# groupeLIAMG/ttcr

Measured on AMD Instinct MI355X. Metric: Mnodes/s per sweep-iteration (512^3 fp32 grid, first-order FSM), higher is better.
Workload: dtype f32

## Files before the change

include/ttcr_amd.h:

```cpp
#ifndef TTCR_AMD_H
#define TTCR_AMD_H

#include <stddef.h>
#include <stdint.h>

#ifdef __cplusplus
extern "C" {
#endif

typedef struct ttcr_fsm_grid ttcr_fsm_grid;

enum { TTCR_F32 = 0, TTCR_F64 = 1 };

enum {
    TTCR_OK = 0,
    TTCR_ERR_VALUE = 1,
    TTCR_ERR_RUNTIME = 2,
    TTCR_ERR_DEVICE = 3,
    TTCR_ERR_UNSUPPORTED = 4
};

int ttcr_fsm_device_count(void);

const char* ttcr_fsm_last_error(void);

int ttcr_fsm3d_create(ttcr_fsm_grid** out, int dtype, int cell_slowness, uint32_t ncx, uint32_t ncy,
                      uint32_t ncz, double dx, double xmin, double ymin, double zmin, double eps,
                      int maxit, int weno, int n_slots, int translate_origin, int device);

int ttcr_fsm2d_create(ttcr_fsm_grid** out, int dtype, int cell_slowness, uint32_t ncx, uint32_t ncz,
                      double dx, double dz, double xmin, double zmin, double eps, int maxit, int weno,
                      int rotated_template, int n_slots, int device);

int ttcr_fsm3d_create_multi(ttcr_fsm_grid** out, int dtype, int cell_slowness, uint32_t ncx, uint32_t ncy,
                            uint32_t ncz, double dx, double xmin, double ymin, double zmin, double eps,
                            int maxit, int weno, int n_slots, int translate_origin, const int* devices, int n_devices);
int ttcr_fsm2d_create_multi(ttcr_fsm_grid** out, int dtype, int cell_slowness, uint32_t ncx, uint32_t ncz,
                            double dx, double dz, double xmin, double zmin, double eps, int maxit, int weno,
                            int rotated_template, int n_slots, const int* devices, int n_devices);
int ttcr_fsm_n_devices(const ttcr_fsm_grid* g);

void ttcr_fsm_destroy(ttcr_fsm_grid* g);

int ttcr_fsm_set_slowness(ttcr_fsm_grid* g, const void* s, size_t n);
int ttcr_fsm_set_slowness_device(ttcr_fsm_grid* g, const void* d_s, size_t n);
int ttcr_fsm_set_slowness_c_order(ttcr_fsm_grid* g, const void* s, size_t n);

int ttcr_fsm_get_slowness(ttcr_fsm_grid* g, void* out, size_t n);

int ttcr_fsm_raytrace(ttcr_fsm_grid* g, int slot, int n_tx, const void* tx, const void* t0, int n_rx,
                      const void* rx, void* tt_out);

int ttcr_fsm_raytrace_multi(ttcr_fsm_grid* g, int n_src, const int* tx_off, const void* tx,
                            const void* t0, const int* rx_off, const void* rx, void* tt_out);

int ttcr_fsm_get_tt(ttcr_fsm_grid* g, int slot, void* out, size_t n);
int ttcr_fsm_get_tt_device(ttcr_fsm_grid* g, int slot, void** d_ptr);
int ttcr_fsm_get_tt_device_view(ttcr_fsm_grid* g, int slot, void** d_ptr, size_t* stride);

int ttcr_fsm_interp(ttcr_fsm_grid* g, int slot, int n_pts, const void* pts, void* tt_out);

int ttcr_fsm_compute_slowness(ttcr_fsm_grid* g, int n_pts, const void* pts, int translated, void* out);

int ttcr_fsm_get_niter(ttcr_fsm_grid* g, int slot, int* niter, int* niterw);
int ttcr_fsm_get_changes(ttcr_fsm_grid* g, int slot, double* first_order, int n_first, double* weno, int n_weno);
int ttcr_fsm_get_reference_changes(ttcr_fsm_grid* g, int slot, double* first_order, int n_first, double* weno, int n_weno);

int ttcr_fsm_n_slots(const ttcr_fsm_grid* g);
size_t ttcr_fsm_n_nodes(const ttcr_fsm_grid* g);
size_t ttcr_fsm_n_cells(const ttcr_fsm_grid* g);

int ttcr_fsm_set_option(ttcr_fsm_grid* g, const char* key, double value);

int ttcr_fsm_rays_size(const ttcr_fsm_grid* g, size_t* n_rays, size_t* n_points);
int ttcr_fsm_get_rays(const ttcr_fsm_grid* g, long long* offsets, void* pts);

int ttcr_fsm_raytrace_rays(ttcr_fsm_grid* g, int slot, int n_tx, const void* tx, const void* t0, int n_rx,
                           const void* rx, void* tt_out);
int ttcr_fsm_slot_rays_size(const ttcr_fsm_grid* g, int slot, size_t* n_rays, size_t* n_points);
int ttcr_fsm_get_slot_rays(const ttcr_fsm_grid* g, int slot, long long* offsets, void* pts);

int ttcr_fsm_raytrace_m(ttcr_fsm_grid* g, int slot, int n_tx, const void* tx, const void* t0, int n_rx,
                        const void* rx, void* tt_out);
int ttcr_fsm_raytrace_rm(ttcr_fsm_grid* g, int slot, int n_tx, const void* tx, const void* t0, int n_rx,
                         const void* rx, void* tt_out);
int ttcr_fsm_slot_m_size(const ttcr_fsm_grid* g, int slot, size_t* n_rows, size_t* nnz);
int ttcr_fsm_get_slot_m(const ttcr_fsm_grid* g, int slot, long long* row_off, long long* j, void* v);
int ttcr_fsm_raytrace_multi_m(ttcr_fsm_grid* g, int n_src, const int* tx_off, const void* tx, const void* t0, const int* rx_off,
                              const void* rx, void* tt_out, int with_rays);
int ttcr_fsm_multi_m_size(const ttcr_fsm_grid* g, size_t* n_rows, size_t* nnz);
int ttcr_fsm_get_multi_m(const ttcr_fsm_grid* g, long long* row_off, long long* j, void* v);

typedef struct ttcr_fsm_tape ttcr_fsm_tape;
int ttcr_fsm_raytrace_multi_tape(ttcr_fsm_grid* g, int n_src, const int* tx_off, const void* tx, const void* t0, const int* rx_off,
                                 const void* rx, void* tt_out, ttcr_fsm_tape** tape);
int ttcr_fsm_tape_size(const ttcr_fsm_tape* t, size_t* n_rows, size_t* n_cols, size_t* nnz);
int ttcr_fsm_tape_bytes(const ttcr_fsm_tape* t, size_t* bytes);
int ttcr_fsm_tape_device(const ttcr_fsm_tape* t, int* device);
int ttcr_fsm_tape_get_csr(const ttcr_fsm_tape* t, long long* row_off, long long* j, void* v);
int ttcr_fsm_tape_vjp(const ttcr_fsm_tape* t, const void* w, int w_on_device, void* grad, int grad_on_device);
int ttcr_fsm_tape_free(ttcr_fsm_tape* t);

typedef struct ttcr_fsm_adjoint ttcr_fsm_adjoint;
int ttcr_fsm_raytrace_multi_adjoint(ttcr_fsm_grid* g, int n_src, const int* tx_off, const void* tx, const void* t0, const int* rx_off,
                                    const void* rx, void* tt_out, ttcr_fsm_adjoint** tape);
int ttcr_fsm_raytrace_multi_adjoint_cells(ttcr_fsm_grid* g, int n_src, const int* tx_off, const void* tx, const void* t0, const int* rx_off,
                                          const void* rx, void* tt_out, ttcr_fsm_adjoint** tape);
int ttcr_fsm_adjoint_model(const ttcr_fsm_adjoint* t, int* cells, size_t* n_params, size_t* n_nodes);
int ttcr_fsm_adjoint_size(const ttcr_fsm_adjoint* t, size_t* n_events, size_t* n_rows, size_t* n_nodes);
int ttcr_fsm_adjoint_bytes(const ttcr_fsm_adjoint* t, size_t* bytes);
int ttcr_fsm_adjoint_device(const ttcr_fsm_adjoint* t, int* device);
int ttcr_fsm_adjoint_get_field(const ttcr_fsm_adjoint* t, size_t event, void* out);
int ttcr_fsm_adjoint_vjp(const ttcr_fsm_adjoint* t, const void* w, int w_on_device, const void* field_cot, int fc_on_device, void* grad,
                         int grad_on_device, int schedule, int* passes);
int ttcr_fsm_adjoint_jvp(const ttcr_fsm_adjoint* t, const void* ds, int ds_on_device, void* dtt, int dtt_on_device, void* dfields,
                         int df_on_device, int schedule, int* passes);
int ttcr_fsm_adjoint_gn(const ttcr_fsm_adjoint* t, const void* v, int v_on_device, const void* row_weight, int rw_on_device, void* out,
                        int out_on_device, int schedule, int* passes_jvp, int* passes_vjp);
int ttcr_fsm_adjoint_points(const ttcr_fsm_adjoint* t, size_t* n_points, int* event_of_point);
int ttcr_fsm_adjoint_jvp_source(const ttcr_fsm_adjoint* t, const void* dsrc, int dsrc_on_device, int n_cols, void* dtt, int dtt_on_device,
                                void* dfields, int df_on_device, int schedule, int* passes);
int ttcr_fsm_adjoint_vjp_source(const ttcr_fsm_adjoint* t, const void* w, int w_on_device, const void* field_cot, int fc_on_device, void* grad,
                                int grad_on_device, void* gsrc, int gsrc_on_device, int schedule, int* passes);
int ttcr_fsm_adjoint_hold(ttcr_fsm_adjoint* t, const void* w, int w_on_device, const void* field_cot, int fc_on_device, void* grad,
                          int grad_on_device, int schedule, int* passes);
int ttcr_fsm_adjoint_release(ttcr_fsm_adjoint* t);
int ttcr_fsm_adjoint_hvp(ttcr_fsm_adjoint* t, const void* v, int v_on_device, void* out, int out_on_device, int schedule, int* passes_jvp,
                         int* passes_vjp);
int ttcr_fsm_adjoint_newton(ttcr_fsm_adjoint* t, const void* v, int v_on_device, const void* row_weight, int rw_on_device, void* out,
                            int out_on_device, int schedule, int* passes_jvp, int* passes_vjp);
int ttcr_fsm_adjoint_jvp_block(const ttcr_fsm_adjoint* t, int n_cols, const void* ds, int ds_on_device, void* dtt, int dtt_on_device,
                               void* dfields, int df_on_device, int schedule, int* passes);
int ttcr_fsm_adjoint_vjp_block(const ttcr_fsm_adjoint* t, int n_cols, const void* w, int w_on_device, void* grad, int grad_on_device,
                               int schedule, int* passes);
int ttcr_fsm_adjoint_gn_block(const ttcr_fsm_adjoint* t, int n_cols, const void* v, int v_on_device, const void* row_weight,
                              int rw_cols, int rw_on_device, void* out, int out_on_device, int schedule, int* passes_jvp, int* passes_vjp);
int ttcr_fsm_adjoint_block_release(ttcr_fsm_adjoint* t);
int ttcr_fsm_adjoint_free(ttcr_fsm_adjoint* t);

int ttcr_fsm_raytrace_l(ttcr_fsm_grid* g, int slot, int n_tx, const void* tx, const void* t0, int n_rx,
                        const void* rx, void* tt_out, int with_rays);
int ttcr_fsm_slot_l_size(const ttcr_fsm_grid* g, int slot, size_t* n_rows, size_t* nnz);
int ttcr_fsm_get_slot_l(const ttcr_fsm_grid* g, int slot, long long* row_off, long long* cell, void* v);
int ttcr_fsm_raytrace_multi_l(ttcr_fsm_grid* g, int n_src, const int* tx_off, const void* tx, const void* t0, const int* rx_off,
                              const void* rx, void* tt_out, int with_rays);
int ttcr_fsm_multi_l_size(const ttcr_fsm_grid* g, size_t* n_rows, size_t* nnz);
int ttcr_fsm_get_multi_l(const ttcr_fsm_grid* g, long long* row_off, long long* cell, void* v);

typedef struct {
// ... 20 lines not shown
```

ttcr_amd/_lib.py:

```python
import ctypes as C
import os

HERE = os.path.dirname(os.path.abspath(__file__))
LIB_PATH = os.environ.get("TTCR_AMD_LIB") or os.path.join(HERE, "libttcr_amd.so")

TTCR_F32, TTCR_F64 = 0, 1
OK, ERR_VALUE, ERR_RUNTIME, ERR_DEVICE, ERR_UNSUPPORTED = 0, 1, 2, 3, 4

_P = C.c_void_p
_U32 = C.c_uint32
_D = C.c_double
_I = C.c_int


class Timing(C.Structure):
    _fields_ = [("sweep_ms", C.c_double), ("total_ms", C.c_double), ("kernel_launches", C.c_longlong),
                ("node_updates", C.c_longlong), ("evaluated_updates", C.c_longlong), ("iterations", C.c_int),
                ("n_sources", C.c_int)]


SYMBOLS = {
    "ttcr_fsm_device_count": (_I, []),
    "ttcr_fsm_last_error": (C.c_char_p, []),
    "ttcr_fsm3d_create": (_I, [C.POINTER(_P), _I, _I, _U32, _U32, _U32, _D, _D, _D, _D, _D, _I, _I, _I, _I, _I]),
    "ttcr_fsm2d_create": (_I, [C.POINTER(_P), _I, _I, _U32, _U32, _D, _D, _D, _D, _D, _I, _I, _I, _I, _I]),
    "ttcr_fsm3d_create_multi": (_I, [C.POINTER(_P), _I, _I, _U32, _U32, _U32, _D, _D, _D, _D, _D, _I, _I, _I, _I, C.POINTER(_I), _I]),
    "ttcr_fsm2d_create_multi": (_I, [C.POINTER(_P), _I, _I, _U32, _U32, _D, _D, _D, _D, _D, _I, _I, _I, _I, C.POINTER(_I), _I]),
    "ttcr_fsm_n_devices": (_I, [_P]),
    "ttcr_fsm_destroy": (None, [_P]),
    "ttcr_fsm_set_slowness": (_I, [_P, _P, C.c_size_t]),
    "ttcr_fsm_set_slowness_device": (_I, [_P, _P, C.c_size_t]),
    "ttcr_fsm_set_slowness_c_order": (_I, [_P, _P, C.c_size_t]),
    "ttcr_fsm_get_slowness": (_I, [_P, _P, C.c_size_t]),
    "ttcr_fsm_raytrace": (_I, [_P, _I, _I, _P, _P, _I, _P, _P]),
    "ttcr_fsm_raytrace_multi": (_I, [_P, _I, _P, _P, _P, _P, _P, _P]),
    "ttcr_fsm_get_tt": (_I, [_P, _I, _P, C.c_size_t]),
    "ttcr_fsm_get_tt_device": (_I, [_P, _I, C.POINTER(_P)]),
    "ttcr_fsm_get_tt_device_view": (_I, [_P, _I, C.POINTER(_P), C.POINTER(C.c_size_t)]),
    "ttcr_fsm_interp": (_I, [_P, _I, _I, _P, _P]),
    "ttcr_fsm_compute_slowness": (_I, [_P, _I, _P, _I, _P]),
    "ttcr_fsm_get_niter": (_I, [_P, _I, C.POINTER(_I), C.POINTER(_I)]),
    "ttcr_fsm_get_changes": (_I, [_P, _I, C.POINTER(_D), _I, C.POINTER(_D), _I]),
    "ttcr_fsm_get_reference_changes": (_I, [_P, _I, C.POINTER(_D), _I, C.POINTER(_D), _I]),
    "ttcr_fsm_n_slots": (_I, [_P]),
    "ttcr_fsm_n_nodes": (C.c_size_t, [_P]),
    "ttcr_fsm_n_cells": (C.c_size_t, [_P]),
    "ttcr_fsm_set_option": (_I, [_P, C.c_char_p, _D]),
    "ttcr_fsm_last_timing": (_I, [_P, C.POINTER(Timing)]),
    "ttcr_fsm_last_kernel": (_I, [_P, C.c_char_p, C.c_size_t]),
    "ttcr_fsm_build_id": (C.c_char_p, []),
    "ttcr_fsm_stopping_stats": (_I, [_P, C.POINTER(C.c_longlong), C.POINTER(C.c_longlong), C.POINTER(C.c_longlong)]),
    "ttcr_fsm_prefill_swaps": (_I, [_P, C.POINTER(C.c_longlong)]),
    "ttcr_fsm_reference_change": (_I, [_P, C.c_void_p, C.c_void_p, C.c_int, C.c_void_p]),
    "ttcr_fsm_rays_size": (_I, [_P, C.POINTER(C.c_size_t), C.POINTER(C.c_size_t)]),
    "ttcr_fsm_get_rays": (_I, [_P, _P, _P]),
    "ttcr_fsm_raytrace_rays": (_I, [_P, _I, _I, _P, _P, _I, _P, _P]),
    "ttcr_fsm_slot_rays_size": (_I, [_P, _I, C.POINTER(C.c_size_t), C.POINTER(C.c_size_t)]),
    "ttcr_fsm_get_slot_rays": (_I, [_P, _I, _P, _P]),
    "ttcr_fsm_raytrace_m": (_I, [_P, _I, _I, _P, _P, _I, _P, _P]),
    "ttcr_fsm_raytrace_rm": (_I, [_P, _I, _I, _P, _P, _I, _P, _P]),
    "ttcr_fsm_raytrace_multi_m": (_I, [_P, _I, _P, _P, _P, _P, _P, _P, _I]),
    "ttcr_fsm_multi_m_size": (_I, [_P, C.POINTER(C.c_size_t), C.POINTER(C.c_size_t)]),
    "ttcr_fsm_get_multi_m": (_I, [_P, _P, _P, _P]),
    "ttcr_fsm_raytrace_multi_tape": (_I, [_P, _I, _P, _P, _P, _P, _P, _P, C.POINTER(_P)]),
    "ttcr_fsm_tape_size": (_I, [_P, C.POINTER(C.c_size_t), C.POINTER(C.c_size_t), C.POINTER(C.c_size_t)]),
    "ttcr_fsm_tape_bytes": (_I, [_P, C.POINTER(C.c_size_t)]),
    "ttcr_fsm_tape_device": (_I, [_P, C.POINTER(_I)]),
    "ttcr_fsm_tape_get_csr": (_I, [_P, _P, _P, _P]),
    "ttcr_fsm_tape_vjp": (_I, [_P, _P, _I, _P, _I]),
    "ttcr_fsm_tape_free": (_I, [_P]),
    "ttcr_fsm_raytrace_multi_adjoint": (_I, [_P, _I, _P, _P, _P, _P, _P, _P, C.POINTER(_P)]),
    "ttcr_fsm_raytrace_multi_adjoint_cells": (_I, [_P, _I, _P, _P, _P, _P, _P, _P, C.POINTER(_P)]),
    "ttcr_fsm_adjoint_model": (_I, [_P, C.POINTER(_I), C.POINTER(C.c_size_t), C.POINTER(C.c_size_t)]),
    "ttcr_fsm_adjoint_size": (_I, [_P, C.POINTER(C.c_size_t), C.POINTER(C.c_size_t), C.POINTER(C.c_size_t)]),
    "ttcr_fsm_adjoint_bytes": (_I, [_P, C.POINTER(C.c_size_t)]),
    "ttcr_fsm_adjoint_device": (_I, [_P, C.POINTER(_I)]),
    "ttcr_fsm_adjoint_get_field": (_I, [_P, C.c_size_t, _P]),
    "ttcr_fsm_adjoint_vjp": (_I, [_P, _P, _I, _P, _I, _P, _I, _I, C.POINTER(_I)]),
    "ttcr_fsm_adjoint_jvp": (_I, [_P, _P, _I, _P, _I, _P, _I, _I, C.POINTER(_I)]),
    "ttcr_fsm_adjoint_gn": (_I, [_P, _P, _I, _P, _I, _P, _I, _I, C.POINTER(_I), C.POINTER(_I)]),
    "ttcr_fsm_adjoint_points": (_I, [_P, C.POINTER(C.c_size_t), _P]),
    "ttcr_fsm_adjoint_jvp_source": (_I, [_P, _P, _I, _I, _P, _I, _P, _I, _I, C.POINTER(_I)]),
    "ttcr_fsm_adjoint_vjp_source": (_I, [_P, _P, _I, _P, _I, _P, _I, _P, _I, _I, C.POINTER(_I)]),
    "ttcr_fsm_adjoint_hold": (_I, [_P, _P, _I, _P, _I, _P, _I, _I, C.POINTER(_I)]),
    "ttcr_fsm_adjoint_release": (_I, [_P]),
    "ttcr_fsm_adjoint_hvp": (_I, [_P, _P, _I, _P, _I, _I, C.POINTER(_I), C.POINTER(_I)]),
    "ttcr_fsm_adjoint_newton": (_I, [_P, _P, _I, _P, _I, _P, _I, _I, C.POINTER(_I), C.POINTER(_I)]),
    "ttcr_fsm_adjoint_jvp_block": (_I, [_P, _I, _P, _I, _P, _I, _P, _I, _I, C.POINTER(_I)]),
    "ttcr_fsm_adjoint_vjp_block": (_I, [_P, _I, _P, _I, _P, _I, _I, C.POINTER(_I)]),
    "ttcr_fsm_adjoint_gn_block": (_I, [_P, _I, _P, _I, _P, _I, _I, _P, _I, _I, C.POINTER(_I), C.POINTER(_I)]),
    "ttcr_fsm_adjoint_block_release": (_I, [_P]),
    "ttcr_fsm_adjoint_free": (_I, [_P]),
    "ttcr_fsm_raytrace_multi_l": (_I, [_P, _I, _P, _P, _P, _P, _P, _P, _I]),
    "ttcr_fsm_multi_l_size": (_I, [_P, C.POINTER(C.c_size_t), C.POINTER(C.c_size_t)]),
    "ttcr_fsm_get_multi_l": (_I, [_P, _P, _P, _P]),
    "ttcr_fsm_slot_m_size": (_I, [_P, _I, C.POINTER(C.c_size_t), C.POINTER(C.c_size_t)]),
    "ttcr_fsm_get_slot_m": (_I, [_P, _I, _P, _P, _P]),
    "ttcr_fsm_raytrace_l": (_I, [_P, _I, _I, _P, _P, _I, _P, _P, _I]),
    "ttcr_fsm_slot_l_size": (_I, [_P, _I, C.POINTER(C.c_size_t), C.POINTER(C.c_size_t)]),
    "ttcr_fsm_get_slot_l": (_I, [_P, _I, _P, _P, _P]),
}

_lib = None


def load():
    global _lib
    if _lib is None:
        if not os.path.exists(LIB_PATH):
            raise ImportError(
                f"{LIB_PATH} is missing: build the HIP extension first (python -m ttcr_amd.build). "
                "ttcr_amd has no CPU fallback.")
        lib = C.CDLL(LIB_PATH)
        for name, (res, args) in SYMBOLS.items():
            fn = getattr(lib, name)
            fn.restype = res
            fn.argtypes = args
        if not os.environ.get("TTCR_AMD_LIB"):
            from . import build as _b

            have, want = lib.ttcr_fsm_build_id().decode(), _b.source_hash()
            if have != want:
                raise ImportError(f"{LIB_PATH} was built from other sources (build id {have}, the sources here hash to {want}): "
                                  "rebuild it (python -m ttcr_amd.build)")
        _lib = lib
    return _lib
# ... 30 lines not shown
```

ttcr_amd/csrc/fsm_capi.hip:

```cpp
#include <hip/hip_runtime.h>

#include <algorithm>
#include <atomic>
#include <chrono>
#include <condition_variable>
#include <cmath>
#include <cstdio>
#include <cstdlib>
#include <cstring>
#include <limits>
#include <map>
#include <memory>
#include <mutex>
#include <sstream>
#include <stdexcept>
#include <string>
#include <thread>
#include <vector>

#include "../../include/ttcr_amd.h"
#include "fsm_kernels.h"
#include "fsm_fast_api.h"
#include "fsm_tape_api.h"
#include "fsm_adjoint_api.h"
// ... 60 lines not shown
    virtual ~GridBase() {}
    virtual void set_slowness(const void* s, size_t n, bool on_device, bool c_order = false) = 0;
    virtual void get_slowness(void* out, size_t n) = 0;
    virtual void raytrace_multi(int n_src, const int* tx_off, const void* tx, const void* t0, const int* rx_off,
                                const void* rx, void* tt_out, int forced_slot, const int* explicit_slots = nullptr,
                                bool force_rays = false) = 0;
    virtual void raytrace_rays(int slot, int n_tx, const void* tx, const void* t0, int n_rx, const void* rx, void* tt_out) = 0;
    virtual void slot_rays_size(int slot, size_t* n_rays, size_t* n_points) const = 0;
    virtual void get_slot_rays(int slot, long long* offsets, void* pts) const = 0;
    virtual void raytrace_m(int slot, int n_tx, const void* tx, const void* t0, int n_rx, const void* rx, void* tt_out, bool both) = 0;
    virtual void slot_m_size(int slot, size_t* n_rows, size_t* nnz) const = 0;
    virtual void get_slot_m(int slot, long long* row_off, long long* j, void* v) const = 0;
    virtual void raytrace_multi_m(int n_src, const int* tx_off, const void* tx, const void* t0, const int* rx_off, const void* rx,
                                  void* tt_out, bool both) = 0;
    virtual void multi_m_size(size_t* n_rows, size_t* nnz) const = 0;
    virtual void get_multi_m(long long* row_off, long long* j, void* v) const = 0;
    virtual void raytrace_multi_tape(int n_src, const int* tx_off, const void* tx, const void* t0, const int* rx_off, const void* rx,
                                     void* tt_out, TapeRows& out) = 0;
    virtual void raytrace_multi_adjoint(int n_src, const int* tx_off, const void* tx, const void* t0, const int* rx_off, const void* rx,
                                        void* tt_out, AdjSink& sink) = 0;
    virtual void adjoint_geometry(int* nn3, double* spacing, bool wrt_cells) const = 0;
    AdjSink* adj_sink = nullptr;
    std::vector<int> adj_src, adj_row;
    virtual void raytrace_l(int slot, int n_tx, const void* tx, const void* t0, int n_rx, const void* rx, void* tt_out, bool with_rays) = 0;
    virtual void slot_l_size(int slot, size_t* n_rows, size_t* nnz) const = 0;
    virtual void get_slot_l(int slot, long long* row_off, long long* cell, void* v) const = 0;
    virtual void raytrace_multi_l(int n_src, const int* tx_off, const void* tx, const void* t0, const int* rx_off, const void* rx,
                                  void* tt_out, bool with_rays) = 0;
    virtual void multi_l_size(size_t* n_rows, size_t* nnz) const = 0;
    virtual void get_multi_l(long long* row_off, long long* cell, void* v) const = 0;
    virtual void validate_points(int n_tx, const void* tx, int n_rx, const void* rx) = 0;
    struct Request {
        int slot, n_tx, n_rx;
        const void *tx, *t0, *rx;
        void* tt;
        int status = TTCR_OK;
        std::string err;
        bool done = false;
    };
    std::mutex q_mu;
    std::condition_variable q_cv;
    std::vector<Request*> queue;
    bool leader_active = false;
    bool had_company = false;
    std::atomic<int> combine_window_us{200};
    size_t elem_size = 4;
    virtual void get_tt(int slot, void* out, size_t n) = 0;
    virtual void* tt_device(int slot) = 0;
    virtual void* tt_device_view(int slot, size_t* stride) = 0;
    std::mutex mu;
    virtual void interp(int slot, int n, const void* pts, void* out) = 0;
    virtual void compute_slowness(int n, const void* pts, bool translated, void* out) = 0;
    virtual void rays_size(size_t* n_rays, size_t* n_points) const = 0;
    virtual void get_rays(long long* offsets, void* pts) const = 0;
    int dim = 3, dtype = 0, n_slots = 1, device = 0;
    size_t n_nodes = 0, n_cells = 0;
    std::vector<int> niter, niterw;
    std::vector<int> phys;
    int P(int slot) const { return phys.empty() ? slot : phys[slot]; }
    int stopping_shortcuts = 3;
    int stopping_rule = 1;
    long long reference_sums = 0, reference_sums_missed = 0;
    long long refsum_rounds = 0;
    virtual void stopping_stats(long long* sums, long long* missed, long long* rounds) const {
        if (sums) *sums = reference_sums;
        if (missed) *missed = reference_sums_missed;
        if (rounds) *rounds = refsum_rounds;
    }
    virtual void reference_change_host(const void* times, const void* field, bool parallel, void* out) = 0;
    int pair_by_distance = 1;
    virtual void set_pair_layout(int) {}
    virtual long long prefill_swap_count() const { return 0; }
    int lone_chunk = 16;
    int arith = 0;
    int prefill = -1;
    std::vector<std::vector<double>> change_hist, change_histw;
    std::vector<std::vector<double>> ref_hist, ref_histw;
    virtual void get_reference_changes(int slot, double* first, int n_first, double* wen, int n_weno) const {
        if (slot < 0 || slot >= n_slots) throw ValueError("Thread number is larger than number of threads");
        slot = P(slot);
        for (int q = 0; q < n_first; ++q) first[q] = (!ref_hist.empty() && q < (int)ref_hist[slot].size()) ? ref_hist[slot][q] : std::nan("");
        for (int q = 0; q < n_weno; ++q) wen[q] = (!ref_histw.empty() && q < (int)ref_histw[slot].size()) ? ref_histw[slot][q] : std::nan("");
    }
    virtual void get_changes(int slot, double* first, int n_first, double* wen, int n_weno) const {
        if (slot < 0 || slot >= n_slots) throw ValueError("Thread number is larger than number of threads");
        slot = P(slot);
        for (int q = 0; q < n_first; ++q) first[q] = (!change_hist.empty() && q < (int)change_hist[slot].size()) ? change_hist[slot][q] : 0.0;
        for (int q = 0; q < n_weno; ++q) wen[q] = (!change_histw.empty() && q < (int)change_histw[slot].size()) ? change_histw[slot][q] : 0.0;
    }
    bool weno = false;
    bool sweep45_strips = false;
    bool rotated = false;
    int ttrp = 0, interp_vel = 0;
    std::atomic<int> return_rays{0};
    int fixed_iters = 0, max_batch = 0, use_graph = 1;
    int skip = -1;
    int mode = 2;
    Timing timing;
    std::string last_kernel;
    virtual std::string kernel_name() const { return last_kernel; }
    long walk_step_limit = 1000000;
    long walk_records = 0;
    long walk_room(long extent) const { return std::min<long>(walk_step_limit, walk_records > 0 ? walk_records : extent); }
    virtual void apply_option(const std::string& k, double value) {
        if (k == "fixed_iters") fixed_iters = (int)value;
        else if (k == "max_batch") max_batch = (int)value;
        else if (k == "use_graph") use_graph = (int)value;
        else if (k == "combine_window_us") combine_window_us = (int)value;
        else if (k == "mode") mode = (int)value;
        else if (k == "skip") skip = (int)value;
        else if (k == "tt_from_rp") ttrp = value != 0;
        else if (k == "interp_vel") interp_vel = value != 0;
        else if (k == "return_rays") return_rays = value != 0;
        else if (k == "pair_sources") pair_by_distance = value != 0;
        else if (k == "pair_layout") {
            if (value != -1 && value != 0 && value != 1) throw ValueError("option 'pair_layout': -1 (default), 0 or 1");
            set_pair_layout((int)value);
        }
        else if (k == "stopping_rule") stopping_rule = (int)value;
        else if (k == "stopping_shortcuts") { if (value < 0 || value > 3 || value != (double)(int)value) throw ValueError("option stopping_shortcuts: 0 ... 3"); stopping_shortcuts = (int)value; }
        else if (k == "prefill") {
            if (value != -1 && value != 0 && value != 1) throw ValueError("option 'prefill': -1 (default), 0 or 1");
            prefill = (int)value;
        } else if (k == "lone_chunk") {
            if (value != 8 && value != 16) throw ValueError("option 'lone_chunk': 8 or 16");
            lone_chunk = (int)value;
        }
        else if (k == "arith") {
            if (value != 0 && value != 1 && value != 2)
                throw ValueError("option 'arith': 0 (the reference's arithmetic), 1 (tolerance-grade fp32 where it stays within 1e-5 s RMS) or 2 (the WENO stage as well)");
            arith = (int)value;
        }
        else if (k == "walk_records") {
            if (value != 0 && !(value >= 1 && value <= (double)walk_step_limit && value == (double)(long)value))
                throw ValueError("option 'walk_records': 0 (default) or a whole number from 1 to the step limit of a walk");
            walk_records = (long)value;
        }
        else throw ValueError("unknown option '" + k + "'");
    }
    virtual void get_niter(int slot, int* it, int* itw) const {
        if (slot < 0 || slot >= n_slots) throw ValueError("Thread number is larger than number of threads");
        if (it) *it = niter[P(slot)];
        if (itw) *itw = niterw[P(slot)];
    }
};

template <typename T, int DIM> struct TileCfg;
#ifndef FSM_PJ3
#define FSM_PJ3 16
#endif
#ifndef FSM_PK3
#define FSM_PK3 16
#endif
template <> struct TileCfg<float, 3> { static constexpr int PJ = FSM_PJ3, PK = FSM_PK3, BL = 16; };
template <> struct TileCfg<double, 3> { static constexpr int PJ = 16, PK = 8, BL = 16; };
#ifndef FSM_PJ2
#define FSM_PJ2 64
#endif
#ifndef FSM_CHUNK2
#define FSM_CHUNK2 16
#endif
template <> struct TileCfg<float, 2> { static constexpr int PJ = FSM_PJ2, PK = 1, BL = 32; };
template <> struct TileCfg<double, 2> { static constexpr int PJ = FSM_PJ2, PK = 1, BL = 32; };
template <typename T, int DIM> struct ChunkCfg { static constexpr int C = DIM == 3 ? FSM_CHUNK3 : FSM_CHUNK2; };

template <typename T>
class GridT : public GridBase {
   public:
    uint32_t ncx, ncy, ncz;
    T dx, dz, xmin, ymin, zmin, xmax, ymax, zmax, ox = 0, oy = 0, oz = 0;
    T epsilon;
    int nitermax;
    bool cell, translate;
    bool have_slowness = false;

    hipStream_t stream = nullptr;
    hipEvent_t ev0 = nullptr, ev1 = nullptr;
    DevBuf<T> d_s, d_cells, d_tt, d_rx, d_out;
    DevBuf<T> d_tt_alt;
    bool alt_filled = false;
    hipStream_t fill_stream = nullptr;
    hipEvent_t ev_fill = nullptr;
    long long prefill_swaps = 0;
    long long prefill_swap_count() const override { return prefill_swaps; }
    void set_pair_layout(int v) override { pair_layout = v; }
    DevBuf<int> d_rslot;
    DevBuf<RaySrc> d_rdesc;
    int weno_ch4_min = 8;
    int weno_c16_below = 3;
    int f64_c16_below = 5;
    int pre_min = 2;
    size_t xs_lds_bytes = 40000;
    int xs_lds_below = 2;
    size_t xs_dyn_lds(int batch) const { return (dim == 3 && stage == 0 && batch < xs_lds_below) ? xs_lds_bytes : 0; }
    int time_order_below = 1 << 30;
    DevBuf<T> d_gather;
    DevBuf<T> d_rsrc, d_rt0;
    DevBuf<int> d_rstat;
    DevBuf<T> d_ssh;
    size_t ssh_stride = 0;
    DevBuf<uint32_t> d_mask;
    DevBuf<int> d_bbox, d_slots, d_lmask;
    int* h_lmask = nullptr;
    DevBuf<uint32_t> d_tiles;
    std::vector<int> tile_off, tile_cnt;
    DevBuf<double> d_change;
    DevBuf<unsigned long long> d_prof;
    size_t prof_words = 0;
    DevBuf<uint32_t> d_order;
    DevBuf<uint32_t> d_order_xs[2][2];
    DevBuf<int> d_sync;
    int n_patches = 0;
    int* h_abort = nullptr;
    DevBuf<int> d_stamp;
    DevBuf<unsigned long long> d_cmap;
    int cmap_words = 1;
    DevBuf<unsigned long long> d_sw;
    int sw_sweeps = 0;
    DevBuf<int> d_iter;
    DevBuf<unsigned long long> d_evals;
    int* h_iter = nullptr;
    unsigned launch_epoch = 1;
    bool sync_clean = true;
    size_t sync_words = 0;
    unsigned long long* h_evals = nullptr;
    int nbf = 0, nbj = 0, nbk = 0;
    size_t n_bricks = 0;
    DevBuf<InitPoint<T>> d_pts;
    double* h_change = nullptr;
    int* h_slots = nullptr;
    size_t mask_words = 0;
    SweepGeom geom;
    int n_launch = 0;
    hipGraph_t graphs[2] = {nullptr, nullptr};
    hipGraphExec_t graph_execs[2] = {nullptr, nullptr};
    int graph_batches[2] = {0, 0}, graph_modes[2] = {-1, -1};

    GridT(int dim_, bool cell_, uint32_t nx, uint32_t ny, uint32_t nz, double ddx, double ddz, double minx,
          double miny, double minz, double eps, int maxit, int nslots, bool translate_, int dev, bool weno_) {
        dim = dim_;
        weno = weno_;
        dtype = sizeof(T) == 4 ? TTCR_F32 : TTCR_F64;
        elem_size = sizeof(T);
        cell = cell_;
        translate = translate_;
        ncx = nx; ncy = ny; ncz = nz;
        dx = (T)ddx;
        dz = (T)ddz;
        xmin = (T)minx; ymin = (T)miny; zmin = (T)minz;
        xmax = xmin + (T)nx * dx;
        if (dim == 3) {
            ymax = ymin + (T)ny * dx;
            zmax = zmin + (T)nz * dx;
        } else {
            ymax = ymin;
            zmax = zmin + (T)nz * dz;
        }
        if (translate) {
            ox = xmin; oy = ymin; oz = zmin;
            xmax -= xmin; ymax -= ymin; zmax -= zmin;
            xmin = 0; ymin = 0; zmin = 0;
        }
        n_nodes = dim == 3 ? (size_t)(nx + 1) * (ny + 1) * (nz + 1) : (size_t)(nx + 1) * (nz + 1);
        n_cells = dim == 3 ? (size_t)nx * ny * nz : (size_t)nx * nz;
        if (n_nodes >= (1ull << 32)) throw ValueError("grid too large: node index must fit uint32 (reference T2)");
        epsilon = (T)eps;
        epsilon *= (T)n_nodes;
        nitermax = maxit;
        n_slots = nslots;
        niter.assign(n_slots, 0);
        niterw.assign(n_slots, 0);
        phys.resize(n_slots);
        for (int q = 0; q < n_slots; ++q) phys[q] = q;
        max_batch = n_slots;
        device = dev;
        HIP_CHECK(hipSetDevice(device));
        {
            int cus = 0;
            HIP_CHECK(hipDeviceGetAttribute(&cus, hipDeviceAttributeMultiprocessorCount, device));
            persist_wgs = 8 * std::max(cus, 1);
        }
        HIP_CHECK(hipStreamCreateWithFlags(&stream, hipStreamNonBlocking));
        HIP_CHECK(hipEventCreate(&ev0));
        HIP_CHECK(hipEventCreate(&ev1));
        d_s.reserve(n_nodes, 64);
        {
            long long pair_units_min = 6144;
            if (const char* e = std::getenv("TTCR_FSM_PAIR_UNITS")) pair_units_min = std::atoll(e);
            const long long patches = dim == 3 ? (long long)((ny + 1 + TileCfg<T, 3>::PJ - 1) / TileCfg<T, 3>::PJ) * ((nz + 1 + TileCfg<T, 3>::PK - 1) / TileCfg<T, 3>::PK) : 0;
            NS = (n_slots >= 2 && dim == 3 && !weno && (long long)n_slots * patches > pair_units_min) ? 2 : 1;
            ns_window = NS == 2 && (long long)n_slots * patches <= (5 * pair_units_min) / 2;
        }
        if (const char* e = std::getenv("TTCR_FSM_PAIR")) { NS = (std::atoi(e) != 0 && n_slots >= 2) ? 2 : 1; ns_window = false; }
        if (const char* e = std::getenv("TTCR_FSM_LAYOUT_LO")) layout_lo = std::atof(e);
        if (const char* e = std::getenv("TTCR_FSM_LAYOUT_HI")) layout_hi = std::atof(e);
        d_tt.reserve(n_nodes * (size_t)(n_slots + (n_slots & 1)), 64);
        mask_words = (n_nodes + 31) / 32;
        d_mask.reserve(mask_words * (size_t)n_slots);
        d_bbox.reserve(6 * (size_t)n_slots);
        d_slots.reserve(n_slots);
        d_lmask.reserve(n_slots);
        HIP_CHECK(hipHostMalloc((void**)&h_lmask, sizeof(int) * n_slots));
        d_change.reserve(n_slots);
        if (std::getenv("TTCR_FSM_PROF")) {
            prof_words = 8 + 4 * (size_t)(1 << 20);
            d_prof.reserve(prof_words);
            HIP_CHECK(hipMemset(d_prof.p, 0, prof_words * sizeof(unsigned long long)));
        }
        HIP_CHECK(hipHostMalloc((void**)&h_change, sizeof(double) * n_slots));
        HIP_CHECK(hipHostMalloc((void**)&h_slots, sizeof(int) * n_slots));
        HIP_CHECK(hipHostMalloc((void**)&h_abort, sizeof(int)));
        *h_abort = 0;
        HIP_CHECK(hipHostMalloc((void**)&h_iter, 2 * sizeof(int)));
        HIP_CHECK(hipHostMalloc((void**)&h_evals, sizeof(unsigned long long) * n_slots));
        HIP_CHECK(hipMemsetAsync(d_tt.p, 0, n_nodes * (size_t)(n_slots + (n_slots & 1)) * sizeof(T), stream));

        if (dim == 3) {
            using C = TileCfg<T, 3>;
            geom.NF = nx + 1; geom.NJ = ny + 1; geom.NK = nz + 1;
            geom.npj = (geom.NJ + C::PJ - 1) / C::PJ;
            geom.npk = (geom.NK + C::PK - 1) / C::PK;
            n_launch = count_launches(C::BL);
        } else {
            using C = TileCfg<T, 2>;
            geom.NF = nz + 1; geom.NJ = nx + 1; geom.NK = 1;
            geom.npj = (geom.NJ + C::PJ - 1) / C::PJ;
            geom.npk = 1;
            n_launch = count_launches(C::BL);
        }
        geom.n_nodes = (uint32_t)n_nodes;
        geom.M = (std::max(geom.NF, geom.NJ) + 1) & ~1;
        geom.MP = geom.M + FSM_XPAD;
        geom.SR = dim == 3 ? ((geom.NJ + 15) / 16) * 32 : 0;
        ssh_stride = (size_t)geom.NK * shear_plane(geom);
        if ((double)(dim == 3 ? 16 : 1) * (double)shear_plane(geom) * sizeof(T) >= 4294967296.0)
            throw ValueError("grid too large for the slowness offsets of the sweep kernel (16 planes of max(nx, ny) x ny nodes must stay below 4 GiB)");
        d_ssh.reserve(ssh_stride * (dim == 3 ? 4 : 2));
        HIP_CHECK(hipMemsetAsync(d_ssh.p, 0, ssh_stride * (dim == 3 ? 4 : 2) * sizeof(T), stream));
        if (dim == 3) build_tile_lists(TileCfg<T, 3>::PJ, TileCfg<T, 3>::PK, TileCfg<T, 3>::BL);
        else build_tile_lists(TileCfg<T, 2>::PJ, TileCfg<T, 2>::PK, TileCfg<T, 2>::BL);
        build_persistent_lists();
        nbf = (geom.NF + FSM_BRICK - 1) / FSM_BRICK;
        nbj = (geom.NJ + FSM_BRICK - 1) / FSM_BRICK;
        nbk = (geom.NK + FSM_BRICK - 1) / FSM_BRICK;
        n_bricks = (size_t)nbf * nbj * nbk;
        d_stamp.reserve(n_bricks * n_slots);
        {
            const int PJ = dim == 3 ? TileCfg<T, 3>::PJ : TileCfg<T, 2>::PJ, PK = dim == 3 ? TileCfg<T, 3>::PK : 1;
            const int max_chunks = (geom.NF + 2 * (PJ + PK)) / 4 + 4;
            cmap_words = max_chunks / 32 + 1;
            d_cmap.reserve((size_t)n_patches * n_slots * (dim == 3 ? 8 : 4) * 2 * cmap_words);
            HIP_CHECK(hipMemset(d_cmap.p, 0, (size_t)n_patches * n_slots * (dim == 3 ? 8 : 4) * 2 * cmap_words * sizeof(unsigned long long)));
            sw_sweeps = (dim == 3 ? 8 : 4) * (2 * std::min(nitermax, 256) + 2);
            d_sw.reserve((size_t)sw_sweeps * n_slots);
        }
        d_iter.reserve(2);
        d_evals.reserve(n_slots);
        if (dim == 2)
            HIP_CHECK(hipFuncSetAttribute(reinterpret_cast<const void*>(&fsm_sweep45_rows<T>),
                                          hipFuncAttributeMaxDynamicSharedMemorySize, 156 * 1024));
        if (const char* e = std::getenv("TTCR_FSM_SWEEP45")) sweep45_strips = std::string(e) == "strips";
        if (const char* e = std::getenv("TTCR_FSM_WENO_CH4_MIN")) weno_ch4_min = std::atoi(e);
        if (const char* e = std::getenv("TTCR_FSM_WENO_C16_BELOW")) weno_c16_below = std::atoi(e);
        if (const char* e = std::getenv("TTCR_FSM_F64_C16_BELOW")) f64_c16_below = std::atoi(e);
        if (const char* e = std::getenv("TTCR_FSM_TIME_ORDER_BELOW")) time_order_below = std::atoi(e);
        if (const char* e = std::getenv("TTCR_FSM_PRE_MIN")) pre_min = std::atoi(e);
        if (const char* e = std::getenv("TTCR_FSM_SKIP")) skip = std::atoi(e);
        if (const char* e = std::getenv("TTCR_FSM_SKIP_UNITS")) skip_units_min = std::atoi(e);
        if (const char* e = std::getenv("TTCR_FSM_SKIP_PROBE_UNITS")) skip_probe_min = std::atoi(e);
        if (const char* e = std::getenv("TTCR_FSM_RS_FIELDS")) rs_fields_max = (size_t)std::max(0, std::atoi(e));
        if (const char* e = std::getenv("TTCR_FSM_WGS")) persist_wgs = std::atoi(e);
        if (const char* e = std::getenv("TTCR_FSM_XS_LDS")) xs_lds_bytes = (size_t)std::atol(e);
        if (const char* e = std::getenv("TTCR_FSM_XS_LDS_BELOW")) xs_lds_below = std::atoi(e);
        if (const char* e = std::getenv("TTCR_FSM_MODE")) mode = std::atoi(e);
        if (const char* e = std::getenv("TTCR_FSM_PREFILL")) prefill = std::atoi(e);
        if (const char* e = std::getenv("TTCR_FSM_LONE_CHUNK")) lone_chunk = std::atoi(e) == 8 ? 8 : 16;
        if (const char* e = std::getenv("TTCR_FSM_ARITH")) arith = std::max(0, std::min(2, std::atoi(e)));
    }

    void build_persistent_lists() {
        std::vector<uint32_t> order;
        for (int m = 0; m <= geom.npj + geom.npk - 2; ++m)
            for (int TK = std::max(0, m - geom.npj + 1); TK <= std::min(m, geom.npk - 1); ++TK)
                order.push_back((uint32_t)(m - TK) | ((uint32_t)TK << 16));
        n_patches = (int)order.size();
        d_order.reserve(order.size());
        HIP_CHECK(hipMemcpy(d_order.p, order.data(), order.size() * sizeof(uint32_t), hipMemcpyHostToDevice));
        sync_words = 8 + (size_t)n_patches * n_slots * (dim == 3 ? 8 : 4);
        d_sync.reserve(sync_words);
        HIP_CHECK(hipMemset(d_sync.p, 0, sync_words * sizeof(int)));
        if (geom.npj >= (1 << 14) || geom.npk >= (1 << 14)) throw ValueError("grid too large for the patch index of the sweep kernel");
        for (int st = 0; st < 2; ++st)
            for (int tm = 0; tm < 2; ++tm) {
                const std::vector<uint32_t> xs = xs_order(order, tm != 0, st == 0 ? 1 : 2);
                d_order_xs[st][tm].reserve(xs.size());
                HIP_CHECK(hipMemcpy(d_order_xs[st][tm].p, xs.data(), xs.size() * sizeof(uint32_t), hipMemcpyHostToDevice));
            }
    }

    std::vector<uint32_t> xs_order(const std::vector<uint32_t>& diag_order, bool by_time, int H) const {
        const int PJ = dim == 3 ? TileCfg<T, 3>::PJ : TileCfg<T, 2>::PJ, PK = dim == 3 ? TileCfg<T, 3>::PK : 1;
        const int C = dim == 3 ? ChunkCfg<T, 3>::C : ChunkCfg<T, 2>::C;
        return xs_order_for(diag_order, by_time, H, PJ, PK, C, geom.npj, n_patches);
    }
    std::vector<uint32_t> xs_order_for(const std::vector<uint32_t>& diag_order, bool by_time, int H, int PJ, int PK, int C, int npj,
                                       int n_patches) const {
        const int ndir = dim == 3 ? 8 : 4;
        std::vector<uint32_t> out;
        out.reserve((size_t)n_patches * ndir);
        if (!by_time) {
            for (int d = 0; d < ndir; ++d)
                for (uint32_t e : diag_order) out.push_back((e & 0xffffu) | ((e >> 16) << 14) | ((uint32_t)d << 28));
            return out;
        }
        auto flags = [&](int d, int& rj, int& rk) {
            if (dim == 3) { rj = (d >> 1) & 1; rk = (d >> 2) & 1; } else { rj = (d == 1) | (d == 2); rk = 0; }
        };
        std::vector<double> ts((size_t)n_patches * ndir, 0.0), tf((size_t)n_patches * ndir, 0.0);
        const double hop_j = (PJ + C - 1.0) / C + 1.0, hop_k = (PK + C - 1.0) / C + 1.0;
        for (int d = 0; d < ndir; ++d) {
            int rj, rk, prj = 0, prk = 0;
            flags(d, rj, rk);
            if (d > 0) flags(d - 1, prj, prk);
            for (uint32_t e : diag_order) {
                const int TJ = e & 0xffffu, TK = e >> 16;
                const size_t me = (size_t)d * n_patches + (size_t)TK * npj + TJ;
                double t = 0.0;
                if (TJ > 0) t = std::max(t, ts[me - 1] + hop_j);
                if (TK > 0) t = std::max(t, ts[me - npj] + hop_k);
                const int j0 = TJ * PJ, k0 = TK * PK;
                const int jm = std::min(j0 + PJ, geom.NJ) - 1, km = std::min(k0 + PK, geom.NK) - 1;
                if (d > 0) {
                    const int ja = std::max(j0 - 2 * H, 0), jb = std::min(jm + 2 * H, geom.NJ - 1);
                    const int ka = std::max(k0 - 2 * H, 0), kb = std::min(km + 2 * H, geom.NK - 1);
                    const int ja2 = rj != prj ? geom.NJ - 1 - jb : ja, jb2 = rj != prj ? geom.NJ - 1 - ja : jb;
                    const int ka2 = rk != prk ? geom.NK - 1 - kb : ka, kb2 = rk != prk ? geom.NK - 1 - ka : kb;
                    for (int tk = ka2 / PK; tk <= kb2 / PK; ++tk)
                        for (int tj = ja2 / PJ; tj <= jb2 / PJ; ++tj) t = std::max(t, tf[(size_t)(d - 1) * n_patches + (size_t)tk * npj + tj]);
                }
                ts[me] = t;
                tf[me] = t + ((jm - j0) + (km - k0) + geom.NF + C - 1) / C + 1.0;
            }
        }
        std::vector<uint32_t> idx((size_t)n_patches * ndir);
        size_t q = 0;
        std::vector<uint32_t> ent((size_t)n_patches * ndir);
        std::vector<double> key((size_t)n_patches * ndir);
        for (int d = 0; d < ndir; ++d)
            for (uint32_t e : diag_order) {
                const int TJ = e & 0xffffu, TK = e >> 16;
                ent[q] = (uint32_t)TJ | ((uint32_t)TK << 14) | ((uint32_t)d << 28);
                key[q] = ts[(size_t)d * n_patches + (size_t)TK * npj + TJ];
                idx[q] = (uint32_t)q;
                ++q;
            }
        std::stable_sort(idx.begin(), idx.end(), [&](uint32_t a2, uint32_t b2) { return key[a2] < key[b2]; });
        for (uint32_t i2 : idx) out.push_back(ent[i2]);
        return out;
    }

    template <int DIM, int H>
    void launch_sweeps_persistent(int batch) {
        constexpr int C0 = ChunkCfg<T, DIM>::C;
        if constexpr (DIM == 3 && C0 == 8) {
            const int below = H == 2 ? weno_c16_below : sizeof(T) == 4 ? std::numeric_limits<int>::max() : f64_c16_below;
            if (NS == 1 && mode == 2 && (lone_chunk == 16 || fast_now<H>()) && batch < below) {
                launch_sweeps_persistent_ns<DIM, H, 1, 16, true>(batch);
                return;
            }
        }
        if (H == 2 && DIM == 3 && NS == 2 && batch >= weno_ch4_min && C0 == 8) {
            if (NS == 2) launch_sweeps_persistent_ns<DIM, H, 2, (H == 2 && DIM == 3) ? 4 : C0>(batch);
            else launch_sweeps_persistent_ns<DIM, H, 1, (H == 2 && DIM == 3) ? 4 : C0>(batch);
        } else {
            if (NS == 2) launch_sweeps_persistent_ns<DIM, H, 2, C0>(batch); else launch_sweeps_persistent_ns<DIM, H, 1, C0>(batch);
        }
    }

    template <int DIM, int H, int NSV, int CH, bool XS_ONLY = false>
    void launch_sweeps_persistent_ns(int batch) {
        using C = TileCfg<T, DIM>;
        PersistArgs<T> pa;
        SweepArgs<T>& a = pa.s;
        constexpr bool NO_PRE = CH == 16 && H == 1 && DIM == 3;
        const size_t dyn_lds = NO_PRE ? 0 : xs_dyn_lds(batch);
        a.tt = d_tt.p;
        a.ts = NS;
        a.lmask = d_lmask.p;
        a.frozen = d_mask.p;
        a.bbox = d_bbox.p;
        a.change = d_change.p;
        a.slots = d_slots.p;
        a.tiles = nullptr;
        a.g = geom;
        a.prof = d_prof.p;
        a.mask_words = (uint32_t)mask_words;
        a.dx = dx;
        a.dz = dz;
        a.w = 0;
        a.variant = DIM == 3 ? 0 : (dx == dz ? 1 : 2);
        pa.order = d_order.p;
        pa.sync = d_sync.p;
        pa.n_patches = n_patches;
        pa.batch = batch;
        pa.timeout_ticks = 300000000ull;
        pa.stamp = d_stamp.p;
        pa.iter_ptr = d_iter.p;
        pa.evals = d_evals.p;
        pa.nbf = nbf; pa.nbj = nbj; pa.nbk = nbk;
        pa.ndir = DIM == 3 ? 8 : 4;
        pa.skip = skip_now(batch) ? (std::getenv("TTCR_FSM_SKIP_ALL_DIRTY") ? 2 : 1) : 0;
        pa.cmap = d_cmap.p;
        pa.cw = cmap_words;
        pa.sw = std::getenv("TTCR_FSM_NO_SW") ? nullptr : d_sw.p;
        pa.n_sw_groups = n_groups();
        pa.n_sw_sweeps = sw_sweeps;

        const size_t wg_cap = (fsm_looped(DIM == 3, H) && persist_wgs > 0) ? (size_t)persist_wgs : ~(size_t)0;
        const dim3 block(C::PJ * C::PK), grid((unsigned)std::min<size_t>((size_t)n_patches * batch, wg_cap));
        const int ndir = DIM == 3 ? 8 : 4;
        {
            const bool pre_ = mode == 2 && !NO_PRE && (DIM == 2 || batch >= pre_min || dyn_lds > 0);
            char nm[160];
            std::snprintf(nm, sizeof nm, "fsm_sweep_persistent<%s,%d,%d,%d,%s,%s,%d,%d,%s,%s>", sizeof(T) == 4 ? "float" : "double", C::PJ, C::PK, CH,
                          DIM == 3 ? "true" : "false", skip_now(batch) ? "true" : "false", H, NSV, mode == 2 ? "true" : "false", pre_ ? "true" : "false");
            last_kernel = nm;
        }
        if (mode == 2) {
            pa.ssh = d_ssh.p;
            pa.ssh_stride = ssh_stride;
            pa.dir = 0;
            a.rf = a.rj = a.rk = a.rev = 0;
            a.s_sheared = nullptr;
            pa.timeout_ticks = 1000000000ull;
            const dim3 gridx((unsigned)std::min<size_t>((size_t)n_patches * batch * ndir, wg_cap));
            pa.order = d_order_xs[H == 2 ? 1 : 0][batch < time_order_below ? 1 : 0].p;
            const bool pre = DIM == 2 || batch >= pre_min || dyn_lds > 0;
            if constexpr (std::is_same<T, float>::value) {
                if (fast_now<H>() && (H == 1 || NSV == 1)) {
                    const FastCfg fc{H, DIM, NSV, CH, skip_now(batch), NO_PRE ? false : pre};
                    last_kernel.insert(last_kernel.size() - 1, ",1");
                    const hipError_t e = fsm_fast_launch(pa, fc, gridx.x, dyn_lds, stream);
                    if (e == hipErrorInvalidValue) throw std::logic_error("arith = 1: no such kernel (" + last_kernel + ")");
                    HIP_CHECK(e);
                    return;
                }
            }
            if constexpr (NO_PRE) {
                (void)pre;
                if (skip_now(batch))
                    fsm_sweep_persistent<T, C::PJ, C::PK, CH, DIM == 3, true, H, NSV, true><<<gridx, block, dyn_lds, stream>>>(pa);
                else
                    fsm_sweep_persistent<T, C::PJ, C::PK, CH, DIM == 3, false, H, NSV, true><<<gridx, block, dyn_lds, stream>>>(pa);
            } else {
                if (skip_now(batch) && pre)
                    fsm_sweep_persistent<T, C::PJ, C::PK, CH, DIM == 3, true, H, NSV, true, true><<<gridx, block, dyn_lds, stream>>>(pa);
                else if (skip_now(batch))
                    fsm_sweep_persistent<T, C::PJ, C::PK, CH, DIM == 3, true, H, NSV, true><<<gridx, block, dyn_lds, stream>>>(pa);
                else if (pre)
                    fsm_sweep_persistent<T, C::PJ, C::PK, CH, DIM == 3, false, H, NSV, true, true><<<gridx, block, dyn_lds, stream>>>(pa);
                else
                    fsm_sweep_persistent<T, C::PJ, C::PK, CH, DIM == 3, false, H, NSV, true><<<gridx, block, dyn_lds, stream>>>(pa);
            }
            HIP_CHECK(hipGetLastError());
            return;
        }
        if (fast_now<H>() && H == 1) throw ValueError("option 'arith' = 1 needs whole-iteration launches (option 'mode' = 2)");
        if constexpr (XS_ONLY) throw std::logic_error("launch_sweeps_persistent_ns: whole-iteration launches only");
        else {
        pa.ssh = nullptr;
        pa.ssh_stride = 0;
        static const int RX2[4] = {0, 1, 1, 0}, RZ2[4] = {0, 0, 1, 1};
        for (int d = 0; d < ndir; ++d) {
            int fam;
            if (DIM == 3) {
                a.rf = d & 1; a.rj = (d >> 1) & 1; a.rk = (d >> 2) & 1;
                a.rev = a.rk;
                fam = (a.rf ^ a.rk) | ((a.rj ^ a.rk) << 1);
            } else {
                a.rj = RX2[d]; a.rf = RZ2[d]; a.rk = 0;
                a.rev = a.rj;
                fam = a.rf ^ a.rj;
            }
            a.s_sheared = d_ssh.p + (size_t)fam * ssh_stride;
            pa.dir = d;
            if (skip_now(batch))
                fsm_sweep_persistent<T, C::PJ, C::PK, CH, DIM == 3, true, H, NSV, false><<<grid, block, 0, stream>>>(pa);
            else
                fsm_sweep_persistent<T, C::PJ, C::PK, CH, DIM == 3, false, H, NSV, false><<<grid, block, 0, stream>>>(pa);
        }
        HIP_CHECK(hipGetLastError());
        }
    }

    void build_tile_lists(int PJ, int PK, int BL) {
        std::vector<uint32_t> all;
        tile_off.assign(n_launch, 0);
        tile_cnt.assign(n_launch, 0);
        for (int w = 0; w < n_launch; ++w) {
// ... 320 lines not shown
        a.n_nodes = n_nodes;
        a.mask_words = (uint32_t)mask_words;
        a.dx = dx;
        const int blocks = a.by_group ? batch * NS : batch;
        const size_t smem = 4 * ((size_t)a.nnz + 2) * sizeof(T);
        if (smem <= 156 * 1024 && !sweep45_strips) {
            const int threads = (int)std::min<size_t>(1024, (((size_t)a.nnz + 63) / 64) * 64);
            fsm_sweep45_rows<T><<<blocks, threads, smem, stream>>>(a);
        } else {
            constexpr int NTMAX = sizeof(T) == 4 ? 1024 : 512;
            if (a.nnx + 2 <= 256) fsm_sweep45<T, 256><<<blocks, 256, 0, stream>>>(a);
            else fsm_sweep45<T, NTMAX><<<blocks, NTMAX, 0, stream>>>(a);
        }
        HIP_CHECK(hipGetLastError());
    }

    void issue_sweeps(int batch) {
        issue_sweeps_axis(batch);
        if (dim == 2 && rotated && !weno && dx == dz) launch_sweep45(batch);
    }

    void issue_sweeps_axis(int batch) {
        if (stage == 1) {
            if (dim == 3) launch_sweeps_persistent<3, 2>(batch); else launch_sweeps_persistent<2, 2>(batch);
        } else if (mode >= 1) {
            if (dim == 3) launch_sweeps_persistent<3, 1>(batch); else launch_sweeps_persistent<2, 1>(batch);
        } else {
            if (dim == 3) launch_sweeps<3>(batch); else launch_sweeps<2>(batch);
        }
    }

    void run_iteration(int batch) {
        const int ndir = dim == 3 ? 8 : 4;
        if (use_graph >= 2 || (use_graph == 1 && !persistent_now())) {
            hipGraph_t& graph = graphs[stage];
            hipGraphExec_t& graph_exec = graph_execs[stage];
            const int key = mode * 2 + (skip_now(batch) ? 1 : 0);
            if (!graph_exec || graph_batches[stage] != batch || graph_modes[stage] != key) {
                if (graph_exec) { (void)hipGraphExecDestroy(graph_exec); graph_exec = nullptr; }
                if (graph) { (void)hipGraphDestroy(graph); graph = nullptr; }
                HIP_CHECK(hipStreamBeginCapture(stream, hipStreamCaptureModeThreadLocal));
                try {
                    issue_sweeps(batch);
                } catch (...) {
                    hipGraph_t junk = nullptr;
                    (void)hipStreamEndCapture(stream, &junk);
                    if (junk) (void)hipGraphDestroy(junk);
                    throw;
                }
                HIP_CHECK(hipStreamEndCapture(stream, &graph));
                HIP_CHECK(hipGraphInstantiate(&graph_exec, graph, nullptr, nullptr, 0));
                graph_batches[stage] = batch;
                graph_modes[stage] = key;
            }
            HIP_CHECK(hipGraphLaunch(graph_exec, stream));
        } else {
            issue_sweeps(batch);
        }
        timing.launches += mode == 2 ? 1 : persistent_now() ? (long long)ndir : (long long)ndir * n_launch;
    }

    std::map<int, DevBuf<T>> snap;
    std::vector<int> snap_iter;
    std::vector<double> prev_change;
    std::vector<double> prev2_change;
    bool snap_always = false;
    std::vector<int> snap_T;
    bool stamps_ok = false;
    int iter_T = 0;
    bool stamps_live_for(int entries) const { return (stopping_shortcuts & 1) && dim == 3 && !weno && persistent_now() && skip_now(entries) && n_nodes * (size_t)NS < ((size_t)1 << 31); }
    void terms_pass(int gi, T* x0, T* x1, unsigned* c0, unsigned* c1, int since_T) {
        RefTermsArgs<T> ta;
        ta.cur = d_tt.p + (size_t)gi * n_nodes * NS;
        ta.old = snap[gi].p;
        ta.x[0] = x0; ta.x[1] = x1;
        ta.cnt[0] = c0; ta.cnt[1] = c1;
        ta.n_nodes = (uint32_t)n_nodes;
        ta.ns = NS;
        constexpr int V = 16 / (int)sizeof(T);
        const size_t n_el = n_nodes * (size_t)NS;
        const bool vec = n_el % V == 0 && ((uintptr_t)ta.cur | (uintptr_t)ta.old) % 16 == 0;
        const int nodes_per_vec = vec ? std::max(1, V / NS) : 1;
        const bool bricks = since_T >= 0 && geom.NF % nodes_per_vec == 0;
        ta.stamp = bricks ? d_stamp.p + (size_t)gi * n_bricks : nullptr;
        ta.thr = (dim == 3 ? 8 : 4) * since_T + 1;
        ta.NF = geom.NF; ta.NJ = geom.NJ; ta.nbf = nbf; ta.nbj = nbj;
        const unsigned nblk = (unsigned)((n_nodes + FSM_REFSUM_CB - 1) / FSM_REFSUM_CB);
        const unsigned blocks = std::min(nblk, 8192u);
        if (vec) fsm_refsum_terms<T, V><<<blocks, 256, 0, stream>>>(ta);
        else fsm_refsum_terms<T, 1><<<blocks, 256, 0, stream>>>(ta);
        HIP_CHECK(hipGetLastError());
    }
    DevBuf<size_t> d_ref_off;
    DevBuf<T> d_ref_out;
    double window_lo() const { return sizeof(T) == 4 ? 0.5 : 1.0 - 1e-6; }
    double window_hi() const { return sizeof(T) == 4 ? 16.0 : 1.0 + 1e-6; }
    void snapshots_before_iteration(const std::vector<int>& active, int it_next) {
        if (!stopping_rule || fixed_iters > 0) return;
        if ((int)snap_iter.size() != n_groups()) snap_iter.assign(n_groups(), 0);
        const bool cheap = n_nodes * (size_t)NS <= ((size_t)1 << 24);
        std::vector<char> done(n_groups(), 0);
        for (int s2 : active) {
            const int gi = s2 / NS;
            if (done[gi]) continue;
            bool may = prev_change[s2] < 1e3 * window_hi() * (double)epsilon;
            if (may && (int)prev2_change.size() == n_slots && std::isfinite(prev2_change[s2]) && prev2_change[s2] > 0) {
                const double r = std::min(1.0, prev_change[s2] / prev2_change[s2]);
                may = prev_change[s2] * r / 8.0 <= window_hi() * (double)epsilon;
            }
            if (!(cheap || (stage == 1 && it_next == 1) || may || snap_always)) continue;
            if (it_next == 1 && stage == 0) continue;
            done[gi] = 1;
            if (snap_iter[gi] == it_next) continue;
            DevBuf<T>& b = snap[gi];
            b.reserve(n_nodes * (size_t)NS);
            if ((int)snap_T.size() != n_groups()) snap_T.assign(n_groups(), -1);
            if (stamps_ok && snap_T[gi] >= 0 && n_nodes * (size_t)NS < ((size_t)1 << 32)) terms_pass(gi, nullptr, nullptr, nullptr, nullptr, snap_T[gi]);
            else HIP_CHECK(hipMemcpyAsync(b.p, d_tt.p + (size_t)gi * n_nodes * NS, n_nodes * (size_t)NS * sizeof(T), hipMemcpyDeviceToDevice, stream));
            snap_iter[gi] = it_next;
            snap_T[gi] = iter_T;
        }
    }
    DevBuf<RefSumState> d_rs_state;
    DevBuf<RefSum4<T>> d_rs_tiles;
    DevBuf<T> d_rc_a, d_rc_b;
    size_t rs_fields_max = 16;
    DevBuf<T> d_rs_x, d_rs_xc;
    DevBuf<unsigned> d_rs_cnt;
    DevBuf<unsigned long long> d_rs_off, d_rs_n, d_rs_n2;
    void reference_change_host(const void* times, const void* field, bool parallel, void* out) override {
        HIP_CHECK(hipSetDevice(device));
        d_rc_a.reserve(n_nodes);
        d_rc_b.reserve(n_nodes);
        HIP_CHECK(hipMemcpyAsync(d_rc_a.p, field, n_nodes * sizeof(T), hipMemcpyHostToDevice, stream));
        HIP_CHECK(hipMemcpyAsync(d_rc_b.p, times, n_nodes * sizeof(T), hipMemcpyHostToDevice, stream));
        *(T*)out = reference_change(d_rc_a.p, d_rc_b.p, 1, !parallel);
    }
    T reference_change(const T* cur, const T* old, int stride, bool one_chain) {
        std::vector<const T*> c{cur}, o{old};
        return reference_changes(c, o, stride, one_chain, std::numeric_limits<T>::infinity())[0];
    }
    DevBuf<const T*> d_rs_ptrs;
    DevBuf<unsigned> d_rs_arrived;
    std::vector<T> reference_changes(const std::vector<const T*>& cur, const std::vector<const T*>& old, int stride, bool one_chain, T stop_at,
                                     const unsigned long long* d_n = nullptr, const std::vector<unsigned long long>* h_n_known = nullptr) {
        const size_t nf = cur.size();
        std::vector<T> out(nf, (T)0);
        if (one_chain) {
            d_ref_off.reserve(1);
            d_ref_out.reserve(1);
            for (size_t f = 0; f < nf; ++f) {
                RefChangeArgs<T> ra;
                ra.cur = cur[f];
                ra.old = old[f];
                const size_t zero = 0;
                HIP_CHECK(hipMemcpyAsync(d_ref_off.p, &zero, sizeof(size_t), hipMemcpyHostToDevice, stream));
                ra.off = d_ref_off.p;
                ra.out = d_ref_out.p;
                ra.n_nodes = n_nodes;
                ra.stride = stride;
                fsm_reference_change<T><<<1, 256, 0, stream>>>(ra);
                HIP_CHECK(hipGetLastError());
                HIP_CHECK(hipMemcpyAsync(&out[f], d_ref_out.p, sizeof(T), hipMemcpyDeviceToHost, stream));
                HIP_CHECK(hipStreamSynchronize(stream));
            }
            return out;
        }
// ... 124 lines not shown
                    curs[a - a0] = d_rs_xc.p + (a - a0) * pitch;
                    const int gi = active[ask[a]] / NS;
                    if (a > a0 && active[ask[a - 1]] / NS == gi) continue;
                    T* xp[2] = {nullptr, nullptr};
                    unsigned* cp[2] = {nullptr, nullptr};
                    for (size_t b = a; b < a1 && active[ask[b]] / NS == gi; ++b) {
                        xp[active[ask[b]] % NS] = d_rs_x.p + (b - a0) * pitch;
                        cp[active[ask[b]] % NS] = d_rs_cnt.p + (b - a0) * (size_t)nblk;
                    }
                    const bool bricks = stamps_ok && (int)snap_T.size() == n_groups() && snap_T[gi] == iter_T;
                    terms_pass(gi, xp[0], xp[1], cp[0], cp[1], bricks ? iter_T : -1);
                    snap_iter[gi] = it + 1;
                    if ((int)snap_T.size() != n_groups()) snap_T.assign(n_groups(), -1);
                    snap_T[gi] = iter_T + 1;
                }
                const dim3 cgrid(std::min(nblk, 4096u), (unsigned)nf);
                fsm_refsum_scan<0><<<(unsigned)nf, 1024, 0, stream>>>(d_rs_cnt.p, d_rs_off.p, nblk, d_rs_n.p);
                HIP_CHECK(hipGetLastError());
                std::vector<unsigned long long> h_m(nf);
                HIP_CHECK(hipMemcpyAsync(h_m.data(), d_rs_n.p, nf * sizeof(unsigned long long), hipMemcpyDeviceToHost, stream));
                HIP_CHECK(hipStreamSynchronize(stream));
                std::vector<size_t> need;
                for (size_t f = 0; f < nf; ++f) {
                    const double u = 0.5 * (double)std::numeric_limits<T>::epsilon(), mu = (double)h_m[f] * u;
                    const double c = h_change[active[ask[a0 + f]]], e = (double)epsilon;
                    if (host_prof) std::fprintf(stderr, "[host]   ask: slot %d iteration %d  fp64 change / (eps N) %.4f  non-zero terms %llu (M u = %.4f)\n", active[ask[a0 + f]], it, c / e, h_m[f], mu);
                    if (h_m[f] == 0ull) { res[a0 + f] = (T)0; res_known[a0 + f] = 1; continue; }
                    if ((stopping_shortcuts & 2) && stage == 0 && mu < 0.25) {
                        const double g = mu / (1.0 - mu), m = 2.0 * (double)(geom.NF + geom.NJ + geom.NK + 64) * u + 1e-6;
                        if (c * (1.0 - m) * (1.0 - g) >= e) { res_go[a0 + f] = 1; continue; }
                        if (c * (1.0 + m) * (1.0 + g) < e) { res_go[a0 + f] = 0; continue; }
                    }
                    need.push_back(f);
                }
                if (!need.empty()) {
                    fsm_refsum_compact<T><<<cgrid, 256, 0, stream>>>(d_rs_x.p, d_rs_xc.p, pitch, n_nodes, d_rs_cnt.p, d_rs_off.p, nblk);
                    HIP_CHECK(hipGetLastError());
                    std::vector<const T*> c2(need.size()), o2(need.size(), nullptr);
                    std::vector<unsigned long long> m2(need.size());
                    for (size_t q = 0; q < need.size(); ++q) { c2[q] = curs[need[q]]; m2[q] = h_m[need[q]]; }
                    d_rs_n2.reserve(std::max<size_t>(need.size(), 64));
                    HIP_CHECK(hipMemcpyAsync(d_rs_n2.p, m2.data(), need.size() * sizeof(unsigned long long), hipMemcpyHostToDevice, stream));
                    const std::vector<T> r = reference_changes(c2, o2, 1, false, epsilon, d_rs_n2.p, &m2);
                    for (size_t q = 0; q < need.size(); ++q) { res[a0 + need[q]] = r[q]; res_known[a0 + need[q]] = 1; }
                }
                a0 = a1;
            }
        }
        for (size_t a = 0; a < ask.size(); ++a) {
            go[ask[a]] = res_known[a] ? res[a] >= epsilon : res_go[a] != 0;
            if (res_known[a]) ref_change_last[active[ask[a]]] = (double)res[a];
            ++reference_sums;
        }
        return go;
    }
    std::vector<double> ref_change_last;

    bool host_prof = std::getenv("TTCR_FSM_HOST_PROF") != nullptr;
    std::chrono::steady_clock::time_point hp_t = std::chrono::steady_clock::now();
    void hp_mark(const char* what) {
        if (!host_prof) return;
        const auto now = std::chrono::steady_clock::now();
        std::fprintf(stderr, "[host] %-28s %8.3f ms\n", what, std::chrono::duration<double, std::milli>(now - hp_t).count());
        hp_t = now;
    }
    void solve_batch(const std::vector<int>& slot_ids, const std::vector<int>& src_ids, const int* tx_off,
                     const T* tx, const T* t0) {
        const int nb = (int)slot_ids.size();
        hp_mark("(before solve_batch)");
        const int nc = ncoord();
        const long long node_updates_before = timing.node_updates;
        size_t tot_pts = 0;
        for (int b = 0; b < nb; ++b) tot_pts += tx_off[src_ids[b] + 1] - tx_off[src_ids[b]];
        std::vector<InitPoint<T>> pts;
        pts.reserve(tot_pts);
        std::vector<size_t> first(nb);
        for (int b = 0; b < nb; ++b) {
            first[b] = pts.size();
            for (int n = tx_off[src_ids[b]]; n < tx_off[src_ids[b] + 1]; ++n) pts.push_back(locate(tx + (size_t)nc * n, t0[n]));
        }
        d_pts.reserve(std::max<size_t>(tot_pts, 1));
        HIP_CHECK(hipMemcpyAsync(d_pts.p, pts.data(), pts.size() * sizeof(InitPoint<T>), hipMemcpyHostToDevice, stream));
        for (int b = 0; b < nb; ++b)
            HIP_CHECK(hipMemsetAsync(d_stamp.p + (size_t)(slot_ids[b] / NS) * n_bricks, 0xFF, n_bricks * sizeof(int), stream));
        std::vector<char> group_filled(n_groups(), 0);
        const bool all_slots = nb == n_slots && prefill_on();
        if (all_slots && alt_filled) {
            HIP_CHECK(hipStreamWaitEvent(stream, ev_fill, 0));
            std::swap(d_tt.p, d_tt_alt.p);
            std::swap(d_tt.n, d_tt_alt.n);
            std::swap(d_tt.guard, d_tt_alt.guard);
            alt_filled = false;
            ++prefill_swaps;
            graph_batches[0] = graph_batches[1] = -1;
            std::fill(group_filled.begin(), group_filled.end(), 1);
        }
        if (NS > 1) {
            std::vector<int> cnt(n_groups(), 0);
            for (int b = 0; b < nb; ++b) cnt[slot_ids[b] / NS] += 1;
            for (int gi = 0; gi < n_groups(); ++gi) {
                if (cnt[gi] != NS || group_filled[gi]) continue;
                const size_t n_el = n_nodes * (size_t)NS;
                const int blocks = (int)std::min<size_t>((n_el + 255) / 256, 16384);
                fsm_fill<T><<<blocks, 256, 0, stream>>>(d_tt.p + (size_t)gi * n_el, n_el, real_traits<T>::max(), 1);
                group_filled[gi] = 1;
            }
        }
        for (int b = 0; b < nb; ++b) {
            const int slot = slot_ids[b];
            T* tt = tt_ptr(slot);
            const int blocks = (int)std::min<size_t>((n_nodes + 255) / 256, 8192);
            if (!group_filled[slot / NS]) fsm_fill<T><<<blocks, 256, 0, stream>>>(tt, n_nodes, real_traits<T>::max(), NS);
            HIP_CHECK(hipMemsetAsync(d_mask.p + (size_t)slot * mask_words, 0, mask_words * sizeof(uint32_t), stream));
            InitArgs<T> ia;
            ia.tt = tt;
            ia.ts = NS;
            ia.slowness = d_s.p;
            ia.frozen = d_mask.p + (size_t)slot * mask_words;
            ia.bbox = d_bbox.p + 6 * (size_t)slot;
            ia.pts = d_pts.p + first[b];
            ia.n_pts = tx_off[src_ids[b] + 1] - tx_off[src_ids[b]];
            ia.npts = weno ? 2 : 1;
            ia.nnx = ncx + 1;
            ia.nny = dim == 3 ? ncy + 1 : 1;
            ia.nnz = ncz + 1;
            ia.dx = dx; ia.dz = dz; ia.xmin = xmin; ia.ymin = ymin; ia.zmin = zmin;
            ia.dim = dim;
            ia.stamp = d_stamp.p + (size_t)(slot / NS) * n_bricks;
            ia.nbf = nbf; ia.nbj = nbj; ia.nbk = nbk;
            fsm_init_source<T><<<1, 128, 0, stream>>>(ia);
            niter[slot] = 0;
            niterw[slot] = 0;
            if (change_hist.empty()) { change_hist.resize(n_slots); change_histw.resize(n_slots); }
            if (ref_hist.empty()) { ref_hist.resize(n_slots); ref_histw.resize(n_slots); }
            change_hist[slot].clear();
            change_histw[slot].clear();
            ref_hist[slot].clear();
            ref_histw[slot].clear();
        }
        HIP_CHECK(hipGetLastError());
        hp_mark("reinit + initFSM issued");
        HIP_CHECK(hipStreamSynchronize(stream));
        hp_mark("reinit + initFSM done");

        const int maxit = fixed_iters > 0 ? fixed_iters : nitermax;
        const int ndir = dim == 3 ? 8 : 4;
        if (!sync_clean || launch_epoch > 0xfffff000u) {
            HIP_CHECK(hipMemsetAsync(d_sync.p, 0, sync_words * sizeof(int), stream));
            HIP_CHECK(hipMemsetAsync(d_cmap.p, 0, (size_t)n_patches * n_slots * ndir * 2 * cmap_words * sizeof(unsigned long long), stream));
            HIP_CHECK(hipStreamSynchronize(stream));
            launch_epoch = 1;
        }
        sync_clean = false;
        snap_always = false;
        if (persistent_now() || weno) HIP_CHECK(hipMemsetAsync(d_sync.p + 8, 0, (sync_words - 8) * sizeof(int), stream));
        if (persistent_now() || weno) HIP_CHECK(hipMemsetAsync(d_sync.p + 4, 0, sizeof(int), stream));
        HIP_CHECK(hipMemsetAsync(d_evals.p, 0, sizeof(unsigned long long) * n_slots, stream));
        HIP_CHECK(hipMemsetAsync(d_sw.p, 0, sizeof(unsigned long long) * (size_t)sw_sweeps * n_groups(), stream));
        HIP_CHECK(hipEventRecord(ev0, stream));
        int it_total = 0;
        for (stage = 0; stage < (weno ? 2 : 1); ++stage) {
            std::vector<int> active(slot_ids);
            int it = 0;
            prev_change.assign(n_slots, std::numeric_limits<double>::infinity());
            prev2_change.assign(n_slots, std::numeric_limits<double>::infinity());
            snap_iter.assign(n_groups(), 0);
            snap_T.assign(n_groups(), -1);
            stamps_ok = false;
            if ((int)ref_change_last.size() != n_slots) ref_change_last.assign(n_slots, std::nan(""));
            std::vector<int> groups;
            for (int s2 : slot_ids)
                if (groups.empty() || groups.back() != s2 / NS) groups.push_back(s2 / NS);
            while (!active.empty() && it < maxit) {
                int n_entries;
                if (persistent_now()) {
                    n_entries = (int)groups.size();
                    for (int b = 0; b < n_entries; ++b) {
                        int m2 = 0;
                        for (int s2 : active)
                            if (s2 / NS == groups[b]) m2 |= 1 << (s2 % NS);
                        h_slots[b] = m2 ? groups[b] : -1;
                        h_lmask[b] = m2;
                    }
                } else {
                    n_entries = nb;
                    for (int b = 0; b < nb; ++b) { h_slots[b] = b < (int)active.size() ? active[b] : -1; h_lmask[b] = 1; }
                }
                HIP_CHECK(hipMemcpyAsync(d_slots.p, h_slots, sizeof(int) * n_entries, hipMemcpyHostToDevice, stream));
                HIP_CHECK(hipMemcpyAsync(d_lmask.p, h_lmask, sizeof(int) * n_entries, hipMemcpyHostToDevice, stream));
                HIP_CHECK(hipMemsetAsync(d_change.p, 0, sizeof(double) * n_slots, stream));
                iter_T = it_total;
                snapshots_before_iteration(active, it + 1);
                if (host_prof) { HIP_CHECK(hipStreamSynchronize(stream)); hp_mark("snapshots"); }
                stamps_ok = (it == 0 ? true : stamps_ok) && stamps_live_for(n_entries);
                h_iter[0] = it_total;
                h_iter[1] = (int)launch_epoch;
                launch_epoch += (persistent_now() && mode == 2) ? 1u : (unsigned)ndir;
                HIP_CHECK(hipMemcpyAsync(d_iter.p, h_iter, 2 * sizeof(int), hipMemcpyHostToDevice, stream));
                run_iteration(n_entries);
                HIP_CHECK(hipMemcpyAsync(h_change, d_change.p, sizeof(double) * n_slots, hipMemcpyDeviceToHost, stream));
                if (persistent_now()) HIP_CHECK(hipMemcpyAsync(h_abort, d_sync.p + 4, sizeof(int), hipMemcpyDeviceToHost, stream));
                HIP_CHECK(hipStreamSynchronize(stream));
                hp_mark("sweep-iteration");
                if (persistent_now() && *h_abort) {
                    HIP_CHECK(hipMemsetAsync(d_sync.p + 4, 0, sizeof(int), stream));
                    stage = 0;
                    throw DeviceError("persistent sweep kernel: a patch timed out waiting for its upwind neighbour");
                }
                ++it;
                ++it_total;
                std::vector<int> next;
                if (fixed_iters > 0) ref_change_last.assign(n_slots, std::nan(""));
                const std::vector<char> go = fixed_iters > 0 ? std::vector<char>(active.size(), 1) : decide_go_on(active, it);
                hp_mark("stopping rule");
                for (size_t q = 0; q < active.size(); ++q) {
                    const int s2 = active[q];
                    (stage == 0 ? niter : niterw)[s2] = it;
                    (stage == 0 ? change_hist : change_histw)[s2].push_back(h_change[s2]);
                    (stage == 0 ? ref_hist : ref_histw)[s2].push_back((int)ref_change_last.size() == n_slots ? ref_change_last[s2] : std::nan(""));
                    timing.node_updates += (long long)n_nodes * ndir;
                    prev2_change[s2] = prev_change[s2];
                    prev_change[s2] = h_change[s2];
                    if (go[q]) next.push_back(s2);
                }
                active.swap(next);
            }
            timing.iterations = std::max(timing.iterations, it_total);
            if (stage == 0 && weno) {
                HIP_CHECK(hipMemsetAsync(d_sw.p, 0, sizeof(unsigned long long) * (size_t)sw_sweeps * n_groups(), stream));
                for (int s2 : slot_ids)
                    HIP_CHECK(hipMemsetD32Async((hipDeviceptr_t)(d_stamp.p + (size_t)(s2 / NS) * n_bricks), it_total * (dim == 3 ? 8 : 4),
                                                n_bricks, stream));
            }
        }
        if (std::getenv("TTCR_FSM_DEBUG_SW")) {
            std::vector<unsigned long long> h((size_t)std::min(sw_sweeps, 40) * n_groups());
            HIP_CHECK(hipMemcpy(h.data(), d_sw.p, h.size() * sizeof(unsigned long long), hipMemcpyDeviceToHost));
            for (size_t q = 0; q < h.size(); ++q) std::fprintf(stderr, "%s%u/%u", q % n_groups() == 0 ? "\n[sw] " : " ", (unsigned)h[q], (unsigned)(h[q] >> 32));
            std::fprintf(stderr, "\n");
        }
        const bool was_persistent = mode >= 1 || weno;
        stage = 0;
        sync_clean = true;
        HIP_CHECK(hipEventRecord(ev1, stream));
        if (all_slots) {
            const size_t n_el = n_nodes * (size_t)(n_slots + (n_slots & 1));
            if (!fill_stream) {
                int lo = 0, hi = 0;
                HIP_CHECK(hipDeviceGetStreamPriorityRange(&lo, &hi));
                HIP_CHECK(hipStreamCreateWithPriority(&fill_stream, hipStreamNonBlocking, lo));
                HIP_CHECK(hipEventCreateWithFlags(&ev_fill, hipEventDisableTiming));
            }
            bool have_alt = true;
            try {
                d_tt_alt.reserve(n_el, 64);
            } catch (const DeviceError&) {
                (void)hipGetLastError();
                have_alt = false;
                prefill = 0;
            }
            if (have_alt) {
            HIP_CHECK(hipStreamWaitEvent(fill_stream, ev1, 0));
            const int blocks = (int)std::min<size_t>((n_el + 255) / 256, 16384);
            fsm_fill<T><<<blocks, 256, 0, fill_stream>>>(d_tt_alt.p, n_el, real_traits<T>::max(), 1);
            HIP_CHECK(hipEventRecord(ev_fill, fill_stream));
            alt_filled = true;
            }
        }
        HIP_CHECK(hipEventSynchronize(ev1));
        if (d_prof.p) {
            unsigned long long h[8];
            HIP_CHECK(hipMemcpy(h, d_prof.p, sizeof(h), hipMemcpyDeviceToHost));
            if (const char* tp = std::getenv("TTCR_FSM_PROF_TRACE")) {
                std::vector<unsigned long long> tr(prof_words);
                HIP_CHECK(hipMemcpy(tr.data(), d_prof.p, prof_words * sizeof(unsigned long long), hipMemcpyDeviceToHost));
                if (FILE* f = std::fopen(tp, "wb")) { std::fwrite(tr.data() + 8, sizeof(unsigned long long), prof_words - 8, f); std::fclose(f); }
            }
            HIP_CHECK(hipMemset(d_prof.p, 0, sizeof(h)));
            if (mode >= 1) {
                const double nb_ = (double)std::max<unsigned long long>(h[7], 1), nu_ = (double)std::max<unsigned long long>(h[6], 1);
                std::fprintf(stderr, "[ttcr_amd prof] units %llu chunks %llu  per unit (us): start %.2f total %.2f | per chunk (us): top %.3f  wait %.3f  stage %.3f  march %.3f  writeback %.3f\n",
                             h[6], h[7], h[5] * 0.01 / nu_, (h[0] + h[1] + h[2] + h[3] + h[4] + h[5]) * 0.01 / nu_, h[0] * 0.01 / nb_,
                             h[1] * 0.01 / nb_, h[2] * 0.01 / nb_, h[3] * 0.01 / nb_, h[4] * 0.01 / nb_);
            } else {
                const double nb_ = (double)std::max<unsigned long long>(h[4], 1);
                std::fprintf(stderr, "[ttcr_amd prof] tiles %llu  per tile (us): setup %.2f  stage %.2f  march %.2f  writeback %.2f\n",
                             h[4], h[0] * 0.01 / nb_, h[1] * 0.01 / nb_, h[2] * 0.01 / nb_, h[3] * 0.01 / nb_);
            }
        }
        hp_mark("after the iterations");
        float ms = 0;
        HIP_CHECK(hipEventElapsedTime(&ms, ev0, ev1));
        timing.sweep_ms += ms;
        const long long evaluated_before = timing.evaluated_updates;
        if (was_persistent) {
            HIP_CHECK(hipMemcpy(h_evals, d_evals.p, sizeof(unsigned long long) * n_slots, hipMemcpyDeviceToHost));
            for (int s2 : slot_ids) timing.evaluated_updates += (long long)h_evals[s2];
        } else {
            timing.evaluated_updates += timing.node_updates - node_updates_before;
        }
        const bool skipped_now = skip_now(n_groups());
        if (nb == n_slots && timing.node_updates > node_updates_before && skipped_now)
            last_eval_frac = (double)(timing.evaluated_updates - evaluated_before) / (double)(timing.node_updates - node_updates_before);
        if (skip < 0 && !weno && in_probe_window((nb + NS - 1) / NS) && timing.node_updates > node_updates_before) {
            if (skipped_now) {
                probe_skip = (double)(timing.evaluated_updates - evaluated_before) / (double)(timing.node_updates - node_updates_before) < 0.6;
                probe_off_calls = 0;
            } else if (++probe_off_calls >= 8) {
                probe_skip = true;
                probe_off_calls = 0;
            }
        }
    }

    void interp(int slot, int n, const void* pts, void* out) override {
        HIP_CHECK(hipSetDevice(device));
        check_slot(slot);
        if (n <= 0) return;
        const int nc = ncoord();
        std::vector<T> p((const T*)pts, (const T*)pts + (size_t)nc * n);
        if (translate)
            for (int m = 0; m < n; ++m) { p[3 * m] -= ox; p[3 * m + 1] -= oy; p[3 * m + 2] -= oz; }
        check_pts(p.data(), n);
        interp_grid_coords(P(slot), n, p.data(), (T*)out);
    }

    void compute_slowness(int n, const void* pts, bool translated, void* out) override {
        HIP_CHECK(hipSetDevice(device));
        if (!have_slowness) throw std::runtime_error("Error: slowness has not been assigned.");
        if (n <= 0) return;
        const int nc = ncoord();
        std::vector<T> p((const T*)pts, (const T*)pts + (size_t)nc * n);
        if (translate && !translated)
            for (int m = 0; m < n; ++m) { p[3 * m] -= ox; p[3 * m + 1] -= oy; p[3 * m + 2] -= oz; }
        check_pts(p.data(), n);
        d_rx.reserve((size_t)nc * n);
        d_out.reserve(n);
        HIP_CHECK(hipMemcpyAsync(d_rx.p, p.data(), sizeof(T) * nc * n, hipMemcpyHostToDevice, stream));
        const int blocks = (n + 63) / 64;
        if (dim == 3) {
            RayGeom<T> rg;
            rg.nnx = ncx + 1; rg.nny = ncy + 1; rg.nnz = ncz + 1;
            rg.dx = dx; rg.xmin = xmin; rg.ymin = ymin; rg.zmin = zmin; rg.xmax = xmax; rg.ymax = ymax; rg.zmax = zmax;
            rg.interp_vel = interp_vel;
            fsm_compute_slowness3d<T><<<blocks, 64, 0, stream>>>(rg, d_s.p, d_rx.p, n, d_out.p);
        } else {
            RayGeom2<T> rg2;
            rg2.nnx = ncx + 1; rg2.nnz = ncz + 1;
            rg2.dx = dx; rg2.dz = dz; rg2.xmin = xmin; rg2.zmin = zmin; rg2.xmax = xmax; rg2.zmax = zmax;
            fsm_compute_slowness2d<T><<<blocks, 64, 0, stream>>>(rg2, d_s.p, d_rx.p, n, d_out.p);
        }
        HIP_CHECK(hipGetLastError());
        HIP_CHECK(hipMemcpyAsync(out, d_out.p, sizeof(T) * n, hipMemcpyDeviceToHost, stream));
        HIP_CHECK(hipStreamSynchronize(stream));
    }

    void interp_grid_coords(int slot, int n, const T* p, T* out) {
        if (n <= 0) return;
        const int nc = ncoord();
        d_rx.reserve((size_t)nc * n);
        d_out.reserve(n);
        HIP_CHECK(hipMemcpyAsync(d_rx.p, p, sizeof(T) * nc * n, hipMemcpyHostToDevice, stream));
        const T* tt = tt_ptr(slot);
        const int blocks = (n + 127) / 128;
        if (dim == 3)
            fsm_interp3d<T><<<blocks, 128, 0, stream>>>(tt, NS, d_rx.p, d_out.p, n, (int)ncx + 1, (int)ncy + 1, (int)ncz + 1, dx, xmin, ymin, zmin);
        else
            fsm_interp2d<T><<<blocks, 128, 0, stream>>>(tt, NS, d_rx.p, d_out.p, n, (int)ncx + 1, (int)ncz + 1, dx, dz, xmin, zmin);
        HIP_CHECK(hipGetLastError());
        HIP_CHECK(hipMemcpyAsync(out, d_out.p, sizeof(T) * n, hipMemcpyDeviceToHost, stream));
        HIP_CHECK(hipStreamSynchronize(stream));
    }

    void interp_batch(const std::vector<int>& sl, const std::vector<int>& sr, const int* rx_off, const T* rx, T* tt_out) {
        const int nc = ncoord();
        size_t n = 0;
        for (int s2 : sr) n += (size_t)(rx_off[s2 + 1] - rx_off[s2]);
        if (n == 0) return;
        std::vector<T> p(nc * n), o(n);
        std::vector<int> so(n);
        size_t k = 0;
        for (size_t b = 0; b < sl.size(); ++b) {
            const int m = rx_off[sr[b] + 1] - rx_off[sr[b]];
            std::memcpy(p.data() + nc * k, rx + (size_t)nc * rx_off[sr[b]], sizeof(T) * nc * m);
// ... 893 lines not shown
                } else {
                    raypath_batch_rays(sl, sr, tx_off, tx.data(), t0, rx_off, rx.data(), tt_out, src_ray_len, src_ray_pts);
                }
            }
        }
        if (return_rays) {
            size_t tot = 0;
            for (int n = 0; n < n_src; ++n) tot += src_ray_pts[n].size();
            rays_pts.reserve(tot);
            for (int n = 0; n < n_src; ++n) {
                for (long long len : src_ray_len[n]) rays_off.push_back(rays_off.back() + len);
                rays_pts.insert(rays_pts.end(), src_ray_pts[n].begin(), src_ray_pts[n].end());
                std::vector<T>().swap(src_ray_pts[n]);
            }
        }
        timing.total_ms = std::chrono::duration<double, std::milli>(std::chrono::steady_clock::now() - wall0).count();
    }
};

class MultiGrid : public GridBase {
   public:
    std::vector<std::unique_ptr<GridBase>> rep;
    int spd = 1;
    std::vector<long long> rays_off{0};
    std::vector<char> rays_pts;
    size_t pt_bytes = 12;

    template <typename Make>
    MultiGrid(int n_slots_, const std::vector<int>& devs, Make&& make) {
        n_slots = n_slots_;
        const int nd = std::min<int>((int)devs.size(), n_slots);
        spd = (n_slots + nd - 1) / nd;
        for (int r = 0; r * spd < n_slots; ++r) rep.emplace_back(make(std::min(spd, n_slots - r * spd), devs[r]));
        const GridBase& g0 = *rep[0];
        dim = g0.dim; dtype = g0.dtype; device = g0.device; n_nodes = g0.n_nodes; n_cells = g0.n_cells;
        elem_size = g0.elem_size; weno = g0.weno;
        pt_bytes = elem_size * (dim == 3 ? 3 : 2);
        niter.assign(n_slots, 0);
        niterw.assign(n_slots, 0);
        for (size_t a = 0; a < rep.size(); ++a)
            for (size_t b = 0; b < rep.size(); ++b)
                if (rep[a]->device != rep[b]->device) {
                    (void)hipSetDevice(rep[a]->device);
                    (void)hipDeviceEnablePeerAccess(rep[b]->device, 0);
                    (void)hipGetLastError();
                }
    }
    GridBase& of(int slot, int& local) const {
        if (slot < 0 || slot >= n_slots) throw ValueError("Thread number is larger than number of threads");
        local = slot % spd;
        return *rep[slot / spd];
    }
    void apply_option(const std::string& k, double value) override {
        GridBase::apply_option(k, value);
        for (auto& r : rep) r->apply_option(k, value);
    }
    void set_slowness(const void* s, size_t n, bool on_device, bool c_order = false) override {
        for (auto& r : rep) r->set_slowness(s, n, on_device, c_order);
    }
    void get_slowness(void* out, size_t n) override { rep[0]->get_slowness(out, n); }
    void validate_points(int n_tx, const void* tx, int n_rx, const void* rx) override { rep[0]->validate_points(n_tx, tx, n_rx, rx); }
    void get_tt(int slot, void* out, size_t n) override { int l; GridBase& g = of(slot, l); g.get_tt(l, out, n); }
    void* tt_device(int slot) override { int l; GridBase& g = of(slot, l); return g.tt_device(l); }
    void* tt_device_view(int slot, size_t* stride) override { int l; GridBase& g = of(slot, l); return g.tt_device_view(l, stride); }
    void interp(int slot, int n, const void* pts, void* out) override { int l; GridBase& g = of(slot, l); g.interp(l, n, pts, out); }
    void compute_slowness(int n, const void* pts, bool translated, void* out) override { rep[0]->compute_slowness(n, pts, translated, out); }
    void get_niter(int slot, int* it, int* itw) const override { int l; GridBase& g = of(slot, l); g.get_niter(l, it, itw); }
    std::string kernel_name() const override { return rep[0]->kernel_name(); }
    long long prefill_swap_count() const override { long long a = 0; for (const auto& r : rep) a += r->prefill_swap_count(); return a; }
    void stopping_stats(long long* sums, long long* missed, long long* rounds) const override {
        long long a = 0, b = 0, c = 0;
        for (const auto& r : rep) { long long x = 0, y = 0, z = 0; r->stopping_stats(&x, &y, &z); a += x; b += y; c += z; }
        if (sums) *sums = a;
        if (missed) *missed = b;
        if (rounds) *rounds = c;
    }
    void reference_change_host(const void* times, const void* field, bool parallel, void* out) override { rep[0]->reference_change_host(times, field, parallel, out); }
    void get_changes(int slot, double* first, int n_first, double* wen, int n_weno) const override {
        int l; GridBase& g = of(slot, l); g.get_changes(l, first, n_first, wen, n_weno);
    }
    void get_reference_changes(int slot, double* first, int n_first, double* wen, int n_weno) const override {
        int l; GridBase& g = of(slot, l); g.get_reference_changes(l, first, n_first, wen, n_weno);
    }
    void rays_size(size_t* n_rays, size_t* n_points) const override { *n_rays = rays_off.size() - 1; *n_points = (size_t)rays_off.back(); }
    void get_rays(long long* offsets, void* pts) const override {
        std::memcpy(offsets, rays_off.data(), rays_off.size() * sizeof(long long));
        if (!rays_pts.empty()) std::memcpy(pts, rays_pts.data(), rays_pts.size());
    }
    void raytrace_rays(int slot, int n_tx, const void* tx, const void* t0, int n_rx, const void* rx, void* tt_out) override {
        int l; GridBase& g = of(slot, l);
        g.raytrace_rays(l, n_tx, tx, t0, n_rx, rx, tt_out);
        timing = g.timing;
    }
    void raytrace_m(int slot, int n_tx, const void* tx, const void* t0, int n_rx, const void* rx, void* tt_out, bool both) override {
        int l; GridBase& g = of(slot, l);
        g.raytrace_m(l, n_tx, tx, t0, n_rx, rx, tt_out, both);
        timing = g.timing;
    }
    void slot_m_size(int slot, size_t* n_rows, size_t* nnz) const override { int l; GridBase& g = of(slot, l); g.slot_m_size(l, n_rows, nnz); }
    std::vector<long long> mm_off{0}, mm_idx;
    std::vector<char> mm_val;
    template <typename Call, typename Size, typename Get>
    void sharded_matrix_call(int n_src, const int* tx_off, const void* tx_v, const void* t0_v, const int* rx_off, const void* rx_v, void* tt_out_v,
                             Call&& call, Size&& size_of, Get&& get_of) {
        const auto wall0 = std::chrono::steady_clock::now();
        timing = Timing();
        timing.n_sources = n_src;
        mm_off.assign(1, 0); mm_idx.clear(); mm_val.clear();
        rays_off.assign(1, 0); rays_pts.clear();
        if (n_src <= 0) return;
        const char* tx = (const char*)tx_v; const char* t0 = (const char*)t0_v; const char* rx = (const char*)rx_v;
        char* tt_out = (char*)tt_out_v;
        const int nd = (int)rep.size();
        std::vector<int> first(nd + 1, 0);
        {
            long long before = 0;
            for (int d = 0; d < nd; ++d) {
                first[d] = (int)((long long)n_src * before / n_slots);
                before += rep[d]->n_slots;
            }
            first[nd] = n_src;
        }
        struct Part { std::vector<long long> off, idx, roff; std::vector<char> val, rpts; Timing t; };
        std::vector<Part> part(nd);
        std::vector<std::exception_ptr> errs(nd);
        auto work = [&](int d) {
            try {
                const int s0 = first[d], m = first[d + 1] - first[d];
                if (m <= 0) return;
                GridBase& g = *rep[d];
                std::vector<int> to(m + 1), ro(m + 1);
                for (int q = 0; q <= m; ++q) { to[q] = tx_off[s0 + q] - tx_off[s0]; ro[q] = rx_off[s0 + q] - rx_off[s0]; }
                std::vector<char> stt(elem_size * (size_t)std::max(ro[m], 1));
                call(g, m, to.data(), tx + pt_bytes * tx_off[s0], t0 + elem_size * tx_off[s0], ro.data(), rx + pt_bytes * rx_off[s0], stt.data());
                std::memcpy(tt_out + elem_size * rx_off[s0], stt.data(), elem_size * (size_t)ro[m]);
                Part& p = part[d];
                p.t = g.timing;
                size_t nr = 0, nnz = 0;
                size_of(g, &nr, &nnz);
                p.off.assign(nr + 1, 0); p.idx.resize(nnz); p.val.resize(nnz * elem_size);
                if (nr > 0) get_of(g, p.off.data(), p.idx.data(), p.val.data());
                size_t rr = 0, rp = 0;
                g.rays_size(&rr, &rp);
                p.roff.assign(rr + 1, 0); p.rpts.resize(rp * pt_bytes);
                if (rr > 0) g.get_rays(p.roff.data(), p.rpts.data());
            } catch (...) { errs[d] = std::current_exception(); }
        };
        std::vector<std::thread> th;
        for (int d = 1; d < nd; ++d) th.emplace_back(work, d);
        work(0);
        for (auto& t : th) t.join();
        for (auto& e : errs)
            if (e) std::rethrow_exception(e);
        for (int d = 0; d < nd; ++d) {
            const Part& p = part[d];
            if (p.off.empty()) continue;
            const long long base = mm_off.back();
            for (size_t r = 1; r < p.off.size(); ++r) mm_off.push_back(base + p.off[r]);
            mm_idx.insert(mm_idx.end(), p.idx.begin(), p.idx.end());
            mm_val.insert(mm_val.end(), p.val.begin(), p.val.end());
            const long long rbase = rays_off.back();
            for (size_t r = 1; r < p.roff.size(); ++r) rays_off.push_back(rbase + p.roff[r]);
            rays_pts.insert(rays_pts.end(), p.rpts.begin(), p.rpts.end());
            timing.sweep_ms = std::max(timing.sweep_ms, p.t.sweep_ms);
            timing.launches += p.t.launches;
            timing.node_updates += p.t.node_updates;
// ... 1317 lines not shown
        if (!n_rows || !nnz) throw ValueError("null output pointer");
        g->impl->multi_l_size(n_rows, nnz);
    });
}
int ttcr_fsm_get_multi_l(const ttcr_fsm_grid* g, long long* row_off, long long* cell, void* v) {
    return guarded_on(g, [&] { g->impl->get_multi_l(row_off, cell, v); });
}
int ttcr_fsm_multi_m_size(const ttcr_fsm_grid* g, size_t* n_rows, size_t* nnz) {
    return guarded_on(g, [&] {
        if (!n_rows || !nnz) throw ValueError("null output pointer");
        g->impl->multi_m_size(n_rows, nnz);
    });
}
int ttcr_fsm_get_multi_m(const ttcr_fsm_grid* g, long long* row_off, long long* j, void* v) {
    return guarded_on(g, [&] { g->impl->get_multi_m(row_off, j, v); });
}
int ttcr_fsm_slot_m_size(const ttcr_fsm_grid* g, int slot, size_t* n_rows, size_t* nnz) {
    return guarded_on(g, [&] {
        if (!n_rows || !nnz) throw ValueError("null output pointer");
        g->impl->slot_m_size(slot, n_rows, nnz);
    });
}
int ttcr_fsm_get_slot_m(const ttcr_fsm_grid* g, int slot, long long* row_off, long long* j, void* v) {
    return guarded_on(g, [&] { g->impl->get_slot_m(slot, row_off, j, v); });
}
int ttcr_fsm_raytrace_l(ttcr_fsm_grid* g, int slot, int n_tx, const void* tx, const void* t0, int n_rx, const void* rx,
                        void* tt_out, int with_rays) {
    return guarded_on(g, [&] { g->impl->raytrace_l(slot, n_tx, tx, t0, n_rx, rx, tt_out, with_rays != 0); });
}
int ttcr_fsm_slot_l_size(const ttcr_fsm_grid* g, int slot, size_t* n_rows, size_t* nnz) {
    return guarded_on(g, [&] {
        if (!n_rows || !nnz) throw ValueError("null output pointer");
        g->impl->slot_l_size(slot, n_rows, nnz);
    });
}
int ttcr_fsm_get_slot_l(const ttcr_fsm_grid* g, int slot, long long* row_off, long long* cell, void* v) {
    return guarded_on(g, [&] { g->impl->get_slot_l(slot, row_off, cell, v); });
}
int ttcr_fsm_slot_rays_size(const ttcr_fsm_grid* g, int slot, size_t* n_rays, size_t* n_points) {
    return guarded_on(g, [&] {
        if (!n_rays || !n_points) throw ValueError("null output pointer");
        g->impl->slot_rays_size(slot, n_rays, n_points);
    });
}
int ttcr_fsm_get_slot_rays(const ttcr_fsm_grid* g, int slot, long long* offsets, void* pts) {
    return guarded_on(g, [&] { g->impl->get_slot_rays(slot, offsets, pts); });
}

int ttcr_fsm_raytrace_multi(ttcr_fsm_grid* g, int n_src, const int* tx_off, const void* tx, const void* t0,
                            const int* rx_off, const void* rx, void* tt_out) {
    return guarded_on(g, [&] { g->impl->raytrace_multi(n_src, tx_off, tx, t0, rx_off, rx, tt_out, -1); });
}

int ttcr_fsm_get_tt(ttcr_fsm_grid* g, int slot, void* out, size_t n) {
    return guarded_on(g, [&] { g->impl->get_tt(slot, out, n); });
}
int ttcr_fsm_get_tt_device(ttcr_fsm_grid* g, int slot, void** d_ptr) {
    return guarded_on(g, [&] {
        if (!d_ptr) throw ValueError("null output pointer");
        *d_ptr = g->impl->tt_device(slot);
    });
}
int ttcr_fsm_get_tt_device_view(ttcr_fsm_grid* g, int slot, void** d_ptr, size_t* stride) {
    return guarded_on(g, [&] {
        if (!d_ptr || !stride) throw ValueError("null output pointer");
        *d_ptr = g->impl->tt_device_view(slot, stride);
    });
}
int ttcr_fsm_interp(ttcr_fsm_grid* g, int slot, int n_pts, const void* pts, void* tt_out) {
    return guarded_on(g, [&] { g->impl->interp(slot, n_pts, pts, tt_out); });
}
int ttcr_fsm_compute_slowness(ttcr_fsm_grid* g, int n_pts, const void* pts, int translated, void* out) {
    return guarded_on(g, [&] { g->impl->compute_slowness(n_pts, pts, translated != 0, out); });
}
int ttcr_fsm_get_niter(ttcr_fsm_grid* g, int slot, int* niter, int* niterw) {
    return guarded_on(g, [&] { g->impl->get_niter(slot, niter, niterw); });
}
int ttcr_fsm_get_changes(ttcr_fsm_grid* g, int slot, double* first_order, int n_first, double* weno, int n_weno) {
    return guarded_on(g, [&] {
        if ((n_first > 0 && !first_order) || (n_weno > 0 && !weno) || n_first < 0 || n_weno < 0) throw ValueError("bad output buffers");
        g->impl->get_changes(slot, first_order, n_first, weno, n_weno);
    });
}
int ttcr_fsm_get_reference_changes(ttcr_fsm_grid* g, int slot, double* first_order, int n_first, double* weno, int n_weno) {
    return guarded_on(g, [&] {
        if ((n_first > 0 && !first_order) || (n_weno > 0 && !weno) || n_first < 0 || n_weno < 0) throw ValueError("bad output buffers");
        g->impl->get_reference_changes(slot, first_order, n_first, weno, n_weno);
    });
}
int ttcr_fsm_n_slots(const ttcr_fsm_grid* g) { return g->impl->n_slots; }
size_t ttcr_fsm_n_nodes(const ttcr_fsm_grid* g) { return g->impl->n_nodes; }
size_t ttcr_fsm_n_cells(const ttcr_fsm_grid* g) { return g->impl->n_cells; }

int ttcr_fsm_set_option(ttcr_fsm_grid* g, const char* key, double value) {
    return guarded_on(g, [&] { g->impl->apply_option(std::string(key ? key : ""), value); });
}

int ttcr_fsm_rays_size(const ttcr_fsm_grid* g, size_t* n_rays, size_t* n_points) {
    return guarded_on(g, [&] { g->impl->rays_size(n_rays, n_points); });
}
int ttcr_fsm_get_rays(const ttcr_fsm_grid* g, long long* offsets, void* pts) {
    return guarded_on(g, [&] { g->impl->get_rays(offsets, pts); });
}

int ttcr_fsm_last_timing(const ttcr_fsm_grid* g, ttcr_fsm_timing* out) {
    return guarded_on(g, [&] {
        const Timing& t = g->impl->timing;
        out->sweep_ms = t.sweep_ms;
        out->total_ms = t.total_ms;
        out->kernel_launches = t.launches;
        out->node_updates = t.node_updates;
        out->evaluated_updates = t.evaluated_updates;
        out->iterations = t.iterations;
        out->n_sources = t.n_sources;
    });
}

int ttcr_fsm_stopping_stats(const ttcr_fsm_grid* g, long long* reference_sums, long long* reference_sums_missed, long long* rounds) {
    return guarded_on(g, [&] { g->impl->stopping_stats(reference_sums, reference_sums_missed, rounds); });
}
int ttcr_fsm_prefill_swaps(const ttcr_fsm_grid* g, long long* swaps) {
    return guarded_on(g, [&] { if (swaps) *swaps = g->impl->prefill_swap_count(); });
}
int ttcr_fsm_reference_change(ttcr_fsm_grid* g, const void* times, const void* field, int parallel, void* out) {
    return guarded_on(g, [&] {
        if (!times || !field || !out) throw ValueError("ttcr_fsm_reference_change: null argument");
        g->impl->reference_change_host(times, field, parallel != 0, out);
    });
}

int ttcr_fsm_last_kernel(const ttcr_fsm_grid* g, char* buf, size_t n) {
    return guarded_on(g, [&] {
        if (!buf || n == 0) throw ValueError("ttcr_fsm_last_kernel: no buffer");
        const std::string k = g->impl->kernel_name();
        std::snprintf(buf, n, "%s", k.c_str());
    });
}

#ifndef TTCR_BUILD_ID
#define TTCR_BUILD_ID "unknown"
#endif
const char* ttcr_fsm_build_id(void) { return TTCR_BUILD_ID; }

}
```

ttcr_amd/csrc/fsm_kernels.h:

```cpp
#pragma once
#include <hip/hip_runtime.h>
#include <stdint.h>
#include <type_traits>

namespace ttcr_amd {

constexpr int FSM_BRICK = 16;

template <typename T> struct real_traits;
template <> struct real_traits<float> {
    static __host__ __device__ constexpr float max() { return 3.402823466e+38f; }
    static __device__ __forceinline__ float inf() { return __builtin_huge_valf(); }
};
template <> struct real_traits<double> {
    static __host__ __device__ constexpr double max() { return 1.7976931348623157e+308; }
    static __device__ __forceinline__ double inf() { return __builtin_huge_val(); }
};

__device__ __forceinline__ uint32_t idx_u32(double v) { return v < 0 ? 0u : (v >= 4294967295.0 ? 4294967295u : (uint32_t)v); }

__device__ __forceinline__ float rmin(float a, float b) { return a < b ? a : b; }
__device__ __forceinline__ double rmin(double a, double b) { return a < b ? a : b; }
__device__ __forceinline__ float rmax(float a, float b) { return a < b ? b : a; }
__device__ __forceinline__ double rmax(double a, double b) { return a < b ? b : a; }

__device__ __forceinline__ bool wave_any(bool p) { return __builtin_amdgcn_ballot_w64(p) != 0ull; }
__device__ __forceinline__ unsigned long long lanes_gt(float a, float b) { return __builtin_amdgcn_fcmpf(a, b, 2); }
__device__ __forceinline__ unsigned long long lanes_gt(double a, double b) { return __builtin_amdgcn_fcmp(a, b, 2); }

__device__ __forceinline__ double sqrt_disc(double x) {
    double y = __builtin_amdgcn_rsq(x);
    double g = x * y;
    double h = 0.5 * y;
    double e = __builtin_fma(-h, g, 0.5);
    g = __builtin_fma(g, e, g);
    h = __builtin_fma(h, e, h);
    double d = __builtin_fma(-g, g, x);
    g = __builtin_fma(d, h, g);
    d = __builtin_fma(-g, g, x);
    g = __builtin_fma(d, h, g);
    return x == 0.0 ? x : g;
}
__device__ __forceinline__ double sqrt_disc_pos(double x) {
    double y = __builtin_amdgcn_rsq(x);
    double g = x * y;
    double h = 0.5 * y;
    double e = __builtin_fma(-h, g, 0.5);
    g = __builtin_fma(g, e, g);
    h = __builtin_fma(h, e, h);
    double d = __builtin_fma(-g, g, x);
    g = __builtin_fma(d, h, g);
    d = __builtin_fma(-g, g, x);
    return __builtin_fma(d, h, g);
}

__device__ __forceinline__ float update3(float ax, float ay, float az, float s, float dx, unsigned long long live_lanes) {
    const float a1 = __builtin_fminf(__builtin_fminf(ax, ay), az);
    const float a3 = __builtin_fmaxf(__builtin_fmaxf(ax, ay), az);
    const float a2 = __builtin_amdgcn_fmed3f(ax, ay, az);
    const float fh = s * dx;
    const float t1 = a1 + fh;
    float t = t1;
    const unsigned long long beyond1d = lanes_gt(t1, a2) & live_lanes;
    if (beyond1d != 0ull) {
        const double d1 = a1, d2 = a2, d3 = a3, dfh = fh;
        double r = -d1 * d1;
        r = __builtin_fma(d1, d2, r);
        r = __builtin_fma(-d2, d2, r);
        r = __builtin_fma(d1, d3, r);
        r = __builtin_fma(d2, d3, r);
        r = __builtin_fma(-d3, d3, r);
        r = __builtin_fma(r, 2.0, (3.0 * dfh) * dfh);
        const float s12 = a1 + a2;
        const float s123 = s12 + a3;
        const float t3 = (float)((1. / 3.) * ((double)s123 + sqrt_disc_pos(r)));
        const float u = a3 - a1, v = a3 - a2;
        const float slack = fh * fh - (u * u + v * v);
        const float thr = 4e-6f * fh * (__builtin_fabsf(a1) + __builtin_fabsf(a3) + fh);
        if ((beyond1d & ~lanes_gt(slack, thr)) != 0ull) {
            const float df = a1 - a2;
            const float df2 = df * df;
            const double disc2 = __builtin_fma(dfh * dfh, 2.0, -(double)df2);
            const float t2 = (float)(0.5 * ((double)s12 + sqrt_disc_pos(disc2)));
            t = t1 > a2 ? (t2 > a3 ? t3 : t2) : t1;
        } else {
            t = t1 > a2 ? t3 : t1;
        }
    }
    return t;
}
// ... 268 lines not shown
    const int kn = rk ? NK - 1 - kp : kp;
    const uint32_t colbase = ((uint32_t)kn * NJ + jn) * NF;
    const T dx = a.dx, dz = a.dz;
    const int variant = a.variant;
    T dec = 0;
    bool changed = false;

    __syncthreads();
    FSM_PROF_MARK(1)

    T own[NQ];
#pragma unroll
    for (int q = 0; q < NQ; ++q) own[q] = Tt[row * RS + q];

#pragma unroll
    for (int q = 1; q <= BL; ++q) {
        bool active = (q >= qa) & (q <= qb);
        if (near_src && active) {
            const int ip = L0 - 1 + q - jp - kp;
            const uint32_t n = colbase + (rf ? NF - 1 - ip : ip);
            active = !((Fz[n >> 5] >> (n & 31)) & 1u);
        }
        const T c = own[q];
        const T af = vmin(own[q - 1], own[q + 1]);
        const T aj = vmin(Tt[(row - 1) * RS + q - 1], Tt[(row + 1) * RS + q + 1]);
        const T s = sv[q - 1];
        T t;
        if (IS3D) {
            const T ak = vmin(Tt[(row - RJ) * RS + q - 1], Tt[(row + RJ) * RS + q + 1]);
            t = update3(ak, aj, af, s, dx, __builtin_amdgcn_ballot_w64(active));
        } else {
            t = variant == 1 ? update2(aj, af, s, dx) : update2_xz(aj, af, s, dx, dz);
        }
        const bool acc = active & (t < c);
        const T nv = acc ? t : c;
        dec += acc ? c - t : (T)0;
        changed |= acc;
        own[q] = nv;
        Tt[row * RS + q] = nv;
        __syncthreads();
    }

    FSM_PROF_MARK(2)
    if (FSM_ENABLE_PROF && a.prof && tid == 0) atomicAdd(a.prof + 4, 1ull);
    if (__syncthreads_or(changed)) {
        for (int f = tid; f < NT * BL; f += NT) {
            const int c = f / BL, q = f - c * BL;
            const int cj = c % PJ, ck = c / PJ;
            const int jq = j0 + cj, kq = k0 + ck;
            const int ip = L0 + q - jq - kq;
            if (jq < NJ && kq < NK && ip >= 0 && ip < NF) {
                const int i = rf ? NF - 1 - ip : ip;
                const int j = rj ? NJ - 1 - jq : jq;
                const int k = rk ? NK - 1 - kq : kq;
                const int r2 = IS3D ? (ck + 1) * RJ + cj + 1 : cj + 1;
                Tg[(size_t)(((uint32_t)k * NJ + j) * NF + i) * ts] = Tt[r2 * RS + q + 1];
            }
        }
        double accd = (double)dec;
#pragma unroll
        for (int off = 32; off > 0; off >>= 1) accd += __shfl_down(accd, off, 64);
        if ((tid & 63) == 0 && accd != 0.0) atomicAdd(a.change + slot, accd);
        FSM_PROF_MARK(3)
    }
}

template <typename T>
struct PersistArgs {
    SweepArgs<T> s;
    const uint32_t* order;
    int* sync;
    int n_patches, batch;
    unsigned long long timeout_ticks;
    int* stamp;
    const int* iter_ptr;
    unsigned long long* evals;
    int nbf, nbj, nbk;
    int dir, ndir;
    int skip;
    unsigned long long* cmap;
    int cw;
    unsigned long long* sw;
    int n_sw_groups, n_sw_sweeps;
    const T* ssh;
    size_t ssh_stride;
};



__device__ __forceinline__ float ld_sc1(const float* p) {
    return __uint_as_float(__hip_atomic_load((const unsigned int*)p, __ATOMIC_RELAXED, __HIP_MEMORY_SCOPE_AGENT));
}
__device__ __forceinline__ double ld_sc1(const double* p) {
    return __longlong_as_double(__hip_atomic_load((const long long*)p, __ATOMIC_RELAXED, __HIP_MEMORY_SCOPE_AGENT));
}
__device__ __forceinline__ void st_sc1(float* p, float v) {
    __hip_atomic_store((unsigned int*)p, __float_as_uint(v), __ATOMIC_RELAXED, __HIP_MEMORY_SCOPE_AGENT);
}
__device__ __forceinline__ void st_sc1(double* p, double v) {
    __hip_atomic_store((long long*)p, __double_as_longlong(v), __ATOMIC_RELAXED, __HIP_MEMORY_SCOPE_AGENT);
}

__device__ __forceinline__ double div_h2(double x, double h2, double r2) {
    const double q0 = x * r2;
    return __builtin_fma(__builtin_fma(-q0, h2, x), r2, q0);
}

__device__ __forceinline__ float weno_fwd(float v1, float v2, float v3, float v4, float h, double r2) {
    const float eps = 1.1920928955078125e-07f;
    const float num = (float)(((double)v4 - 2.0 * (double)v3) + (double)v2);
    const float den = (float)(((double)v3 - 2.0 * (double)v2) + (double)v1);
    const float r = (eps + num * num) / (eps + den * den);
    const float w = (float)(1.0 / (1.0 + (2.0 * (double)r) * (double)r));
    const float d31 = v3 - v1;
    const double h2 = 2.0 * (double)h;
    const double ap = div_h2((1.0 - (double)w) * (double)d31, h2, r2) +
                      div_h2((double)w * ((-(double)v4 + 4.0 * (double)v3) - 3.0 * (double)v2), h2, r2);
    return v2 + h * (float)ap;
}
__device__ __forceinline__ float weno_bwd(float v0, float v1, float v2, float v3, float h, double r2) {
    const float eps = 1.1920928955078125e-07f;
    const float num = (float)(((double)v2 - 2.0 * (double)v1) + (double)v0);
    const float den = (float)(((double)v3 - 2.0 * (double)v2) + (double)v1);
    const float r = (eps + num * num) / (eps + den * den);
    const float w = (float)(1.0 / (1.0 + (2.0 * (double)r) * (double)r));
    const float d31 = v3 - v1;
    const double h2 = 2.0 * (double)h;
    const double am = div_h2((1.0 - (double)w) * (double)d31, h2, r2) +
                      div_h2((double)w * ((3.0 * (double)v2 - 4.0 * (double)v1) + (double)v0), h2, r2);
    return v2 - h * (float)am;
}
__device__ __forceinline__ double weno_fwd(double v1, double v2, double v3, double v4, double h, double) {
    const double eps = 2.220446049250313e-16;
    const double num = (v4 - 2.0 * v3 + v2);
    const double den = (v3 - 2.0 * v2 + v1);
    const double r = (eps + num * num) / (eps + den * den);
    const double w = 1.0 / (1.0 + 2.0 * r * r);
    const double ap = (1.0 - w) * (v3 - v1) / (2.0 * h) + w * (-v4 + 4.0 * v3 - 3.0 * v2) / (2.0 * h);
    return v2 + h * ap;
}
__device__ __forceinline__ double weno_bwd(double v0, double v1, double v2, double v3, double h, double) {
    const double eps = 2.220446049250313e-16;
    const double num = (v2 - 2.0 * v1 + v0);
    const double den = (v3 - 2.0 * v2 + v1);
    const double r = (eps + num * num) / (eps + den * den);
    const double w = 1.0 / (1.0 + 2.0 * r * r);
    const double am = (1.0 - w) * (v3 - v1) / (2.0 * h) + w * (3.0 * v2 - 4.0 * v1 + v0) / (2.0 * h);
    return v2 - h * am;
}

template <typename T>
__device__ __forceinline__ T weno_axis(T m2, T m1, T c, T p1, T p2, int idx, int n, T h, double r2) {
    const bool c0 = idx == 0;
    const bool c1 = !c0 && idx == 1;
    const bool cn = !c0 && !c1 && idx == n;
    const bool cm = !c0 && !c1 && !cn && idx == n - 1;
    const T F = weno_fwd(m1, c, p1, p2, h, r2);
    const T B = weno_bwd(m2, m1, c, p1, h, r2);
    T a = cm ? B : F;
    const T t = c1 ? m1 : (cm ? p1 : B);
    a = a < t ? a : t;
    return c0 ? p1 : (cn ? m1 : a);
}

#ifndef FSM_WENO_PLAIN
#define FSM_WENO_PLAIN 0
// ... 205 lines not shown
}

template <typename T, int NS> struct Pack;
template <typename T> struct Pack<T, 1> { T v[1]; };
template <typename T> struct alignas(2 * sizeof(T)) Pack<T, 2> { T v[2]; };

template <typename T, int NS>
__device__ __forceinline__ Pack<T, NS> pack_fill(T x) {
    Pack<T, NS> p;
#pragma unroll
    for (int l = 0; l < NS; ++l) p.v[l] = x;
    return p;
}
__device__ __forceinline__ Pack<float, 1> ld_sc1(const Pack<float, 1>* p) { Pack<float, 1> r; r.v[0] = ld_sc1(&p->v[0]); return r; }
__device__ __forceinline__ Pack<double, 1> ld_sc1(const Pack<double, 1>* p) { Pack<double, 1> r; r.v[0] = ld_sc1(&p->v[0]); return r; }
__device__ __forceinline__ Pack<float, 2> ld_sc1(const Pack<float, 2>* p) {
    const unsigned long long u = __hip_atomic_load((const unsigned long long*)p, __ATOMIC_RELAXED, __HIP_MEMORY_SCOPE_AGENT);
    Pack<float, 2> r;
    r.v[0] = __uint_as_float((unsigned)u);
    r.v[1] = __uint_as_float((unsigned)(u >> 32));
    return r;
}
__device__ __forceinline__ Pack<double, 2> ld_sc1(const Pack<double, 2>* p) {
    Pack<double, 2> r;
    r.v[0] = ld_sc1(&p->v[0]);
    r.v[1] = ld_sc1(&p->v[1]);
    return r;
}
__device__ __forceinline__ void st_sc1(Pack<float, 1>* p, Pack<float, 1> x) { st_sc1(&p->v[0], x.v[0]); }
__device__ __forceinline__ void st_sc1(Pack<double, 1>* p, Pack<double, 1> x) { st_sc1(&p->v[0], x.v[0]); }
__device__ __forceinline__ void st_sc1(Pack<float, 2>* p, Pack<float, 2> x) {
    const unsigned long long u = (unsigned long long)__float_as_uint(x.v[0]) | ((unsigned long long)__float_as_uint(x.v[1]) << 32);
    __hip_atomic_store((unsigned long long*)p, u, __ATOMIC_RELAXED, __HIP_MEMORY_SCOPE_AGENT);
}
__device__ __forceinline__ void st_sc1(Pack<double, 2>* p, Pack<double, 2> x) {
    st_sc1(&p->v[0], x.v[0]);
    st_sc1(&p->v[1], x.v[1]);
}

__host__ __device__ constexpr bool fsm_looped(bool is3d, int h) { return is3d && h == 1; }

__device__ __forceinline__ int kmaxp_of(int k0, int NK, int PK) { return (k0 + PK < NK ? k0 + PK : NK) - 1; }
template <typename T, int PJ, int PK, int C, bool IS3D, bool SKIP, int H, int NS, bool XS, bool PRE, int AR = 0>
__device__ __forceinline__ bool fsm_sweep_unit(const PersistArgs<T>& pa) {
    static_assert(AR == 0 || std::is_same<T, float>::value, "tolerance-grade arithmetic: fp32 kernels");
    constexpr bool LOOPED = fsm_looped(IS3D, H);
    using P = Pack<T, NS>;
    constexpr int NT = PJ * PK;
    constexpr int RJ = PJ + 2 * H;
    constexpr int NROWS = IS3D ? RJ * (PK + 2 * H) : RJ;
    constexpr int NQ = C + 2 * H;
    constexpr int RS = NQ | 1;
    constexpr int NUP = IS3D ? H * (PJ + PK) : H;
    constexpr int NDH = IS3D ? H * (PJ + PK) : H;
    constexpr int RPI = NT / C;
    constexpr int NOWN = C;
    constexpr int NHI = (NDH + RPI - 1) / RPI;
    constexpr int NUPI = (NUP + RPI - 1) / RPI;
    static_assert(NT % C == 0 && (IS3D || PK == 1) && C <= FSM_BRICK && (H == 1 || H == 2), "tile shape");
    static_assert(C - 1 <= FSM_XPAD, "the rows of a chunk are read from the sheared copies without a wrap");
    static_assert(!(SKIP && FSM_EARLY_PUB > 0), "FSM_EARLY_PUB is a tuning option of the kernels without exact skipping");
    const SweepArgs<T>& a = pa.s;
    const unsigned epoch = (unsigned)pa.iter_ptr[1] + (XS ? 0u : (unsigned)pa.dir);
    const int e2 = (int)(epoch % 3u) + 1;
    auto dec_prog = [&](int raw_) -> int { return (int)((unsigned)raw_ >> 30) == e2 ? (raw_ & 0x3fffffff) : 0; };
    auto ld_raw = [&](const int* p_) -> int { return __hip_atomic_load(p_, __ATOMIC_RELAXED, __HIP_MEMORY_SCOPE_AGENT); };
    auto ld_prog = [&](const int* p_) -> int { return dec_prog(ld_raw(p_)); };
    auto st_prog = [&](int* p_, int v_) {
        __hip_atomic_store(p_, (int)(((unsigned)e2 << 30) | (unsigned)v_), __ATOMIC_RELAXED, __HIP_MEMORY_SCOPE_AGENT);
    };
    auto ld_cmap = [&](const unsigned long long* p_) -> unsigned {
        const unsigned long long v_ = __hip_atomic_load(p_, __ATOMIC_RELAXED, __HIP_MEMORY_SCOPE_AGENT);
        return (unsigned)(v_ >> 32) == epoch ? (unsigned)v_ : 0u;
    };
    auto st_cmap = [&](unsigned long long* p_, unsigned v_) {
        __hip_atomic_store(p_, ((unsigned long long)epoch << 32) | v_, __ATOMIC_RELAXED, __HIP_MEMORY_SCOPE_AGENT);
    };

    __shared__ P Tt[NROWS * RS];
    __shared__ int s_ticket, s_abort;
    __shared__ int s_anychg;
    constexpr int SLABW = SKIP ? FSM_SLAB_WORDS : 1;
    __shared__ unsigned s_stamped[SKIP ? 9 : 1][SLABW];
    __shared__ unsigned s_slab[SLABW];
    __shared__ int s_next, s_act;
    __shared__ int s_cwi[2], s_cwl[2];
    __shared__ unsigned s_cwv[2];
    __shared__ int s_mywi;
    __shared__ unsigned s_mywv[2];
    enum { U_THR, U_RSJLO, U_RSKLO, U_RSNJ, U_RSNK, U_LCF, U_UPLCF0, U_UPLCF1, U_HIST, U_EVER, U_UCHG, U_PENDV, U_LCHG, U_N };
    __shared__ int s_u[U_N];

    int tid = threadIdx.x;
    if constexpr (LOOPED) asm volatile("" : "+v"(tid));
    unsigned long long prof_t = (FSM_ENABLE_PROF && a.prof) ? wall_clock64() : 0ull;
    unsigned long long pacc[6] = {0, 0, 0, 0, 0, 0};
    unsigned pchunks = 0;
    unsigned long long twait = 0;
    constexpr int FSM_TRACE_UNITS = FSM_ENABLE_PROF == 2 ? (1 << 20) : 65536;
    const unsigned long long trace_t0 = prof_t;
    unsigned long long* prec = nullptr;
    __shared__ unsigned long long s_pacc[FSM_ENABLE_PROF == 2 ? 8 : 1];
    if constexpr (FSM_ENABLE_PROF == 2) {
        if (tid == 0) {
            for (int q = 0; q < 6; ++q) s_pacc[q] = 0;
            s_pacc[6] = prof_t;
        }
    }
#define FSM_PMARK(slot_)                                                          \
    if constexpr (FSM_ENABLE_PROF == 2) {                                         \
        if (a.prof && tid == 0) {                                                 \
            const unsigned long long now_ = wall_clock64();                       \
            s_pacc[slot_] += now_ - s_pacc[6];                                    \
            s_pacc[6] = now_;                                                     \
        }                                                                         \
    }                                                                             \
    if (FSM_ENABLE_PROF == 1 && a.prof && tid == 0) {                             \
        const unsigned long long now_ = wall_clock64();                           \
        pacc[slot_] += now_ - prof_t;                                             \
        prof_t = now_;                                                            \
         \
        if ((slot_) < 5 && prec && pchunks < 80u) prec[pchunks * 5u + (slot_)] = now_; \
    }
    const int NF = a.g.NF, NJ = a.g.NJ, NK = a.g.NK;
    const int npj = a.g.npj;
    auto prev_sweep_counter = [&](int d, int TJ_, int TK_, int z_, int lane) -> const int* {
        const int pd = d - 1;
        int crj, crk, prj, prk;
        if (IS3D) { crj = (d >> 1) & 1; crk = (d >> 2) & 1; prj = (pd >> 1) & 1; prk = (pd >> 2) & 1; }
        else { crj = (d == 1) | (d == 2); crk = 0; prj = (pd == 1) | (pd == 2); prk = 0; }
        const int j0_ = TJ_ * PJ, k0_ = TK_ * PK;
        const int jm_ = (j0_ + PJ < NJ ? j0_ + PJ : NJ) - 1, km_ = (k0_ + PK < NK ? k0_ + PK : NK) - 1;
        int ja = j0_ - 2 * H, jb = jm_ + 2 * H, ka = k0_ - 2 * H, kb = km_ + 2 * H;
        ja = ja < 0 ? 0 : ja; jb = jb > NJ - 1 ? NJ - 1 : jb;
        ka = ka < 0 ? 0 : ka; kb = kb > NK - 1 ? NK - 1 : kb;
        const int ja2 = (crj != prj) ? NJ - 1 - jb : ja, jb2 = (crj != prj) ? NJ - 1 - ja : jb;
        const int ka2 = (crk != prk) ? NK - 1 - kb : ka, kb2 = (crk != prk) ? NK - 1 - ka : kb;
        const int tja = ja2 / PJ, ntj = jb2 / PJ - tja + 1;
        const int tka = IS3D ? ka2 / PK : 0, ntk = IS3D ? kb2 / PK - tka + 1 : 1;
        const int ia = lane & 3, ib = lane >> 2;
        if (ia >= ntj || ib >= ntk) return nullptr;
        return pa.sync + 8 + ((size_t)pd * pa.batch + z_) * pa.n_patches + ((tka + ib) * npj + tja + ia);
    };
    if constexpr (LOOPED) __syncthreads();
    if (tid == 0) {
        const int t_ = atomicAdd(pa.sync + (epoch & 3u), 1);
        if (t_ == 0) __hip_atomic_store(pa.sync + ((epoch + 2u) & 3u), 0, __ATOMIC_RELAXED, __HIP_MEMORY_SCOPE_AGENT);
        s_ticket = t_;
    }
    if (LOOPED && tid == 1) s_abort = __hip_atomic_load(pa.sync + 4, __ATOMIC_RELAXED, __HIP_MEMORY_SCOPE_AGENT);
    __syncthreads();
    if (LOOPED && s_abort) return false;
    const int ticket = __builtin_amdgcn_readfirstlane(s_ticket);
    const int oidx = ticket / pa.batch, z = ticket - oidx * pa.batch;
    if (oidx >= (XS ? pa.n_patches * pa.ndir : pa.n_patches)) return false;
    if (FSM_ENABLE_PROF == 1 && a.prof && ticket < 8192) prec = a.prof + 8 + 4 * 65536 + (size_t)ticket * 400;
    const uint32_t tile = pa.order[oidx];
    const int dir = XS ? (int)(tile >> 28) : pa.dir;
    const int TJ = XS ? (int)(tile & 0x3fffu) : (int)(tile & 0xffffu), TK = XS ? (int)((tile >> 14) & 0x3fffu) : (int)(tile >> 16);
    int* prog = pa.sync + 8 + ((size_t)(XS ? dir : 0) * pa.batch + z) * pa.n_patches;
    int* my_prog = prog + (TK * npj + TJ);
    int rf, rj, rk, rev;
    const T* __restrict__ Sg;
    if (XS) {
        int fam;
        if (IS3D) {
            rf = dir & 1; rj = (dir >> 1) & 1; rk = (dir >> 2) & 1;
            rev = rk;
            fam = (rf ^ rk) | ((rj ^ rk) << 1);
        } else {
            rj = (dir == 1) | (dir == 2); rf = dir >> 1; rk = 0;
            rev = rj;
            fam = rf ^ rj;
// ... 221 lines not shown
                    if (q & 1) rowp += SRB;
                }
            } else {
#pragma unroll
                for (int q = 0; q < C; ++q) {
                    if (!(q & 1)) { sv[q] = ld_row(1); rowp += SRB; } else sv[q] = ld_row(0);
                }
            }
        } else {
#pragma unroll
            for (int q = 0; q < C; ++q) {
                sv[q] = ld_row(0);
                rowp += SRB;
            }
        }
        x = rev ? x - C : x + C;
        if (x < 0 || x >= M) { x %= M; x = x < 0 ? x + M : x; }
        xs_next = x;
        xs_level = L + C;
        const int sL = sf * L;
#pragma unroll
        for (int it = 0; it < NOWN + NHI; ++it) {
            P v = PFILL;
            if ((unsigned)(L + ipb[it]) < (unsigned)NF) v = XS ? ld_sc1(Tg + (abase[it] + sL)) : Tg[abase[it] + sL];
            tv[it] = v;
        }
    };

    unsigned long long nevals = 0;

    T dec[NS];
#pragma unroll
    for (int l = 0; l < NS; ++l) dec[l] = 0;
    P carry[2 * H];
#pragma unroll
    for (int q = 0; q < 2 * H; ++q) carry[q] = PFILL;
    bool have_prev = false;
    int pref_for = -(1 << 30);
    int pending = 0;
    int n_done = 0;
    int pre_j = -1, pre_k = -1;
    int smp_j = 0, smp_k = 0;
    P uvn[NUPI];
    int uvn_for = -(1 << 30);
    int near_lo[NS], near_hi[NS];
    {
        const int jlo = rj ? NJ - 1 - jmaxp : j0, jhi = rj ? NJ - 1 - j0 : jmaxp;
        const int klo = rk ? NK - 1 - kmaxp : k0, khi = rk ? NK - 1 - k0 : kmaxp;
#pragma unroll
        for (int l = 0; l < NS; ++l) {
            const int* b6 = bb + 6 * l;
            const int b0 = rf ? NF - 1 - b6[1] : b6[0], b1 = rf ? NF - 1 - b6[0] : b6[1];
            const bool jk = !(jhi < b6[2] || jlo > b6[3] || khi < b6[4] || klo > b6[5]) && b0 <= NF - 1 && b1 >= 0;
            near_lo[l] = jk ? b0 - (C - 1) + j0 + k0 : 1;
            near_hi[l] = jk ? b1 + jmaxp + kmaxp : 0;
        }
    }
    if (!FSM_EXP_NOWAIT && XS && dir > 0 && !chase) {
        if (tid < 16) {
            const int* pp = prev_sweep_counter(dir, TJ, TK, z, tid);
            if (pp) {
                const unsigned long long t0 = wall_clock64();
                int spins = 0;
                while (ld_prog(pp) < (SKIP ? FSM_FIN : 0x3fffffff)) {
                    if ((++spins & 63) == 0) {
                        if (__hip_atomic_load(pa.sync + 4, __ATOMIC_RELAXED, __HIP_MEMORY_SCOPE_AGENT)) break;
                        if (wall_clock64() - t0 > pa.timeout_ticks) {
                            __hip_atomic_store(pa.sync + 4, 1, __ATOMIC_RELAXED, __HIP_MEMORY_SCOPE_AGENT);
                            break;
                        }
                    }
                    __builtin_amdgcn_s_sleep(8);
                }
            }
        }
        __syncthreads();
    }
    if (CHASE_OK && chase) chase_wait(Lc - C, -1, false);
    if (!SKIP) { issue_static(Lc); pref_for = Lc; }
    if constexpr (SKIP) {
        const int nsw = (pa.nbf + 31) >> 5;
        for (int w = tid; w < nsw; w += NT) s_slab[w] = 0u;
        for (int w = tid; w < 9 * SLABW; w += NT) s_stamped[w / SLABW][w % SLABW] = 0u;
        if (tid == 0) {
            s_cwi[0] = -1; s_cwi[1] = -1; s_mywi = -1;
            const int ja = j0 - H < 0 ? 0 : j0 - H, jb = jmaxp + H > NJ - 1 ? NJ - 1 : jmaxp + H;
            const int ka = k0 - H < 0 ? 0 : k0 - H, kb = kmaxp + H > NK - 1 ? NK - 1 : kmaxp + H;
            const int jlo = (rj ? NJ - 1 - jb : ja) / FSM_BRICK, jhi = (rj ? NJ - 1 - ja : jb) / FSM_BRICK;
            const int klo = (rk ? NK - 1 - kb : ka) / FSM_BRICK, khi = (rk ? NK - 1 - ka : kb) / FSM_BRICK;
            s_u[U_RSJLO] = jlo; s_u[U_RSNJ] = jhi - jlo + 1;
            s_u[U_RSKLO] = klo; s_u[U_RSNK] = khi - klo + 1;
            const int sg = pa.ndir * pa.iter_ptr[0] + dir + 1;
            s_u[U_THR] = pa.skip == 2 ? -(1 << 30) : (sg - 1 > 0 ? sg - 1 : 0);
            s_u[U_LCF] = Lc;
            const int lsj = Ls - PJ, lsk = Ls - PK, mu = TJ + TK - 1;
            s_u[U_UPLCF0] = lsj - (((lsj - mu) % C + C) % C);
            s_u[U_UPLCF1] = lsk - (((lsk - mu) % C + C) % C);
            s_u[U_HIST] = 0; s_u[U_EVER] = 0; s_u[U_UCHG] = 0; s_u[U_PENDV] = 0; s_u[U_LCHG] = 0;
        }
        __syncthreads();
        {
            const int jlo = s_u[U_RSJLO], nj = s_u[U_RSNJ], klo = s_u[U_RSKLO], nk = s_u[U_RSNK], thr = s_u[U_THR];
            const int* __restrict__ stamp = pa.stamp + (size_t)grp * pa.nbf * pa.nbj * pa.nbk;
            const int total = pa.nbf * nj * nk;
            for (int b = tid; b < total; b += NT) {
                const int bf = b % pa.nbf, jk = b / pa.nbf;
                const int bj = jlo + jk % nj, bk = klo + jk / nj;
                const int v = __hip_atomic_load(stamp + ((size_t)bk * pa.nbj + bj) * pa.nbf + bf, __ATOMIC_RELAXED, __HIP_MEMORY_SCOPE_AGENT);
                if (v >= thr) atomicOr(&s_slab[bf >> 5], 1u << (bf & 31));
            }
        }
        __syncthreads();
    }
    FSM_PMARK(5)
    const unsigned long long trace_t1 = (FSM_ENABLE_PROF && a.prof) ? wall_clock64() : 0ull;
    auto cmap_of = [&](int pidx, int e) -> unsigned long long* {
        return pa.cmap + ((((size_t)(XS ? dir : 0) * pa.batch + z) * pa.n_patches + (size_t)pidx) * 2 + e) * pa.cw;
    };
    auto slab_any = [&](int flo, int fhi) -> bool {
        const int b0 = flo / FSM_BRICK, b1 = fhi / FSM_BRICK;
        for (int w = b0 >> 5; w <= (b1 >> 5); ++w) {
            const int lo = w == (b0 >> 5) ? (b0 & 31) : 0, hi = w == (b1 >> 5) ? (b1 & 31) : 31;
            const unsigned msk = (hi == 31 ? 0xffffffffu : ((2u << hi) - 1u)) & ~((1u << lo) - 1u);
            if (s_slab[w] & msk) return true;
        }
        return false;
    };
    auto chunk_frange = [&](int L, int ext, int& flo, int& fhi) {
        int ia = L - ext - jmaxp - kmaxp, ib = L + C - 1 + ext - j0 - k0;
        ia = ia < 0 ? 0 : ia;
        ib = ib > NF - 1 ? NF - 1 : ib;
        flo = rf ? NF - 1 - ib : ia;
        fhi = rf ? NF - 1 - ia : ib;
    };
    auto up_dirty = [&](int v, int need, int e) -> bool {
        if (v >= FSM_FIN && !((v >> e) & 1)) return false;
        for (int p2 = 0; p2 < H; ++p2) {
            const int nd = need - p2 * C;
            const int ulcf = s_u[U_UPLCF0 + e];
            const int ciu = (nd - C - ulcf) / C;
            if (nd - C - ulcf < 0) continue;
            int bit;
            const int d = v >= FSM_FIN ? 4 : ((v >> 8) - nd) / C;
            if (d < 4) {
                bit = (v >> (2 * d + e)) & 1;
            } else {
                const int w = ciu >> 5;
                if (w >= pa.cw) continue;
                if (s_cwi[e] != w || s_cwl[e] < nd) {
                    s_cwl[e] = v >= FSM_FIN ? 0x7fffffff : (v >> 8);
                    const unsigned long long* um = cmap_of(e == 0 ? TK * npj + TJ - 1 : (TK - 1) * npj + TJ, e);
                    s_cwv[e] = ld_cmap(um + w);
                    s_cwi[e] = w;
                }
                bit = (s_cwv[e] >> (ciu & 31)) & 1u;
            }
            if (bit) return true;
        }
        return false;
    };
    auto poll_until = [&](const int* ptr, int want, bool& ok) -> int {
        unsigned long long t0 = 0;
        int spins = 0;
        for (;;) {
            const int v = ld_prog(ptr);
            if (v >= want) {
                if (FSM_ENABLE_PROF == 2 && spins) twait += wall_clock64() - t0;
                return v;
            }
            if (spins == 0) t0 = wall_clock64();
            if ((++spins & 63) == 0) {
                if (__hip_atomic_load(pa.sync + 4, __ATOMIC_RELAXED, __HIP_MEMORY_SCOPE_AGENT)) { ok = false; return v; }
                if (wall_clock64() - t0 > pa.timeout_ticks) {
                    __hip_atomic_store(pa.sync + 4, 1, __ATOMIC_RELAXED, __HIP_MEMORY_SCOPE_AGENT);
                    ok = false;
                    return v;
                }
            }
            __builtin_amdgcn_s_sleep(FSM_POLL_SLEEP);
        }
    };
    for (; Lc <= Le; Lc += C) {
        if constexpr (PRE) {
            pre_j = dec_prog(smp_j);
            pre_k = dec_prog(smp_k);
        }
        if constexpr (SKIP) {
            FSM_PMARK(0)
            if (tid == 0) {
                int L = Lc, act = 1, h = s_u[U_HIST];
                const int lcf = s_u[U_LCF];
                const bool follow = s_u[U_LCHG] != 0 && L <= Le;
                s_u[U_LCHG] = 0;
// ... 152 lines not shown
        }
        if (PRE && (tid & 63) == 0 && Lc + C <= Le) {
            if (up_j) smp_j = ld_raw(up_j);
            if (up_k) smp_k = ld_raw(up_k);
        }
        if (PRE && CHASE_OK && chase_ptr && Lc + C <= Le)
            smp_j = ld_raw(chase_ptr);

        bool near_src[NS];
#pragma unroll
        for (int l = 0; l < NS; ++l) near_src[l] = L0 >= near_lo[l] && L0 <= near_hi[l];

        P own[NQ];
#pragma unroll
        for (int q = 0; q < 2 * H; ++q) own[q] = carry[q];
#pragma unroll
        for (int q = 2 * H; q < NQ; ++q) own[q] = Tt[row * RS + q];
        T sc[C];
#pragma unroll
        for (int q = 0; q < C; ++q) sc[q] = rev ? sv[C - 1 - q] : sv[q];
        FSM_PMARK(2)

        if (Lc + C <= Le) { issue_static(Lc + C); pref_for = Lc + C; }

        constexpr bool WAVE2D = !IS3D && NT == 64 && H == 1;
        P hup[WAVE2D ? C : 1], hdn[WAVE2D ? C : 1];
        if (WAVE2D) {
#pragma unroll
            for (int ee = 0; ee < C; ++ee) {
                hup[ee] = Tt[(H - 1) * RS + ee + H - 1];
                hdn[ee] = Tt[(PJ + H) * RS + ee + H + 1];
            }
        }
        bool changed = false;
        constexpr bool DUP = H == 1 && !IS3D;
        if constexpr (!DUP) {
#define FSM_SIMPLE false
#define FSM_VAR 0
#include "fsm_march_levels.inc"
#undef FSM_SIMPLE
#undef FSM_VAR
        } else {
            bool near_any = false;
#pragma unroll
            for (int l = 0; l < NS; ++l) near_any |= near_src[l];
            const bool full_wave = !near_any && __builtin_amdgcn_ballot_w64(ea == 0 && eb == C - 1) == ~0ull;
            if (!full_wave) {
#define FSM_SIMPLE false
#define FSM_VAR 0
#include "fsm_march_levels.inc"
#undef FSM_SIMPLE
#undef FSM_VAR
            } else if (variant == 1) {
#define FSM_SIMPLE true
#define FSM_VAR 1
#include "fsm_march_levels.inc"
#undef FSM_SIMPLE
#undef FSM_VAR
            } else {
#define FSM_SIMPLE true
#define FSM_VAR 2
#include "fsm_march_levels.inc"
#undef FSM_SIMPLE
#undef FSM_VAR
            }
        }
#pragma unroll
        for (int q = 0; q < 2 * H; ++q) carry[q] = own[C + q];
        FSM_PMARK(3)
        if (FSM_ENABLE_PROF) ++pchunks;

        if constexpr (SKIP) {
            const bool ej = changed && jp + H > jmaxp, ek = IS3D && changed && kp + H > kmaxp;
            const int f = (wave_any(changed) ? 1 : 0) | (wave_any(ej) ? 2 : 0) | (wave_any(ek) ? 4 : 0);
            if (f && (tid & 63) == 0) atomicOr(&s_anychg, f);
            if (!(FSM_SKIP_ABL & 2) && changed) {
                const int ip0 = L0 - jp - kp;
                const int ia = ip0 + ea, ib = ip0 + eb;
                const int ba = (rf ? NF - 1 - ib : ia) / FSM_BRICK, bb2 = (rf ? NF - 1 - ia : ib) / FSM_BRICK;
                const int my_bj = (rj ? NJ - 1 - jp : jp) / FSM_BRICK - s_u[U_RSJLO], my_bk = (rk ? NK - 1 - kp : kp) / FSM_BRICK - s_u[U_RSKLO];
                const int jk = my_bk * s_u[U_RSNJ] + my_bj;
                atomicOr(&s_stamped[jk][ba >> 5], 1u << (ba & 31));
                if (bb2 != ba) atomicOr(&s_stamped[jk][bb2 >> 5], 1u << (bb2 & 31));
            }
        } else {
            if (wave_any(changed) && (tid & 63) == 0) s_anychg = 1;
        }
        __syncthreads();
        const int chg_flags = SKIP ? __builtin_amdgcn_readfirstlane(s_anychg) : s_anychg;
        const bool any_changed = chg_flags != 0;
        if (any_changed) {
#pragma unroll
            for (int it = 0; it < NOWN; ++it) {
                const int ipm = L0 + ipb[it] - H;
                if ((unsigned)ipm < (unsigned)NF) {
                    const int rid = rsub + RPI * it;
                    const int cj = rid % PJ, ck = rid / PJ;
                    P* dst = Tg + (abase[it] + sf * (L0 - H));
                    const P v = Tt[lrow[it] - H];
                    if (XS || cj >= PJ - H || (IS3D && ck >= PK - H)) st_sc1(dst, v); else *dst = v;
                }
            }
        }
        if constexpr (SKIP) {
            if (!(FSM_SKIP_ABL & 4) && tid == 0) {
                if (any_changed) {
                    int flo, fhi;
                    chunk_frange(L0, 0, flo, fhi);
                    for (int b = flo / FSM_BRICK; b <= fhi / FSM_BRICK; ++b) s_slab[b >> 5] |= 1u << (b & 31);
                    const int ci = (L0 - s_u[U_LCF]) / C, w = ci >> 5;
                    if ((chg_flags & 6) && w < pa.cw) {
                        if (s_mywi != w) { s_mywi = w; s_mywv[0] = 0u; s_mywv[1] = 0u; }
                        for (int e2 = 0; e2 < 2; ++e2)
                            if (chg_flags & (2 << e2)) {
                                s_mywv[e2] |= 1u << (ci & 31);
                                st_cmap(cmap_of(TK * npj + TJ, e2) + w, s_mywv[e2]);
                            }
                    }
                    s_u[U_UCHG] = 1;
                    s_u[U_LCHG] = 1;
                }
                const int h2 = ((s_u[U_HIST] << 2) | (chg_flags >> 1)) & 0xff, ev2 = s_u[U_EVER] | (chg_flags >> 1);
                s_u[U_HIST] = h2;
                s_u[U_EVER] = ev2;
                s_u[U_PENDV] = Lc + C > Le ? (FSM_FIN | ev2) : (((Lc + C) << 8) | h2);
            }
        }
        if constexpr (SKIP) pending = 1;
        else pending = Lc + C > Le ? 0x3fffffff : Lc + C;
        if (FSM_EARLY_PUB > 0 && n_done < FSM_EARLY_PUB) {
            asm volatile("s_waitcnt vmcnt(0)" ::: "memory");
            __syncthreads();
            if (tid == 0) st_prog(my_prog, SKIP ? s_u[U_PENDV] : pending);
            pending = 0;
        }
        ++n_done;
        FSM_PMARK(4)
    }
    if constexpr (SKIP) {
        __syncthreads();
        if (s_u[U_UCHG]) {
            const int nsw = (pa.nbf + 31) >> 5;
            const int rs_jlo = s_u[U_RSJLO], rs_nj = s_u[U_RSNJ], rs_klo = s_u[U_RSKLO], njk = rs_nj * s_u[U_RSNK];
            int* __restrict__ stamp = pa.stamp + (size_t)grp * pa.nbf * pa.nbj * pa.nbk;
            const int sigma = pa.ndir * pa.iter_ptr[0] + dir + 1;
            for (int q = tid; q < njk * nsw * 32; q += NT) {
                const int jk = q / (nsw * 32), bf = q % (nsw * 32);
                if (bf < pa.nbf && ((s_stamped[jk][bf >> 5] >> (bf & 31)) & 1u))
                    atomicMax(stamp + ((size_t)(rs_klo + jk / rs_nj) * pa.nbj + rs_jlo + jk % rs_nj) * pa.nbf + bf, sigma);
            }
            pending = 1;
        }
    }
    if (pending) {
        asm volatile("s_waitcnt vmcnt(0)" ::: "memory");
        __syncthreads();
        if (tid == 0) st_prog(my_prog, SKIP ? s_u[U_PENDV] : pending);
    }
    if constexpr (SKIP) {
        const int sigma0 = pa.ndir * pa.iter_ptr[0] + dir;
        if (tid == 0 && pa.sw && sigma0 < pa.n_sw_sweeps)
            atomicAdd(pa.sw + (size_t)sigma0 * pa.n_sw_groups + grp, 1ull | (s_u[U_UCHG] ? (1ull << 32) : 0ull));
    }

    if (FSM_ENABLE_PROF && a.prof && tid == 0) {
        if constexpr (FSM_ENABLE_PROF == 2) {
            for (int q = 0; q < 6; ++q) atomicAdd(a.prof + q, s_pacc[q]);
            atomicAdd(a.prof + 6, 1ull);
            atomicAdd(a.prof + 7, (unsigned long long)pchunks);
        }
        if (FSM_ENABLE_PROF == 1) {
#pragma unroll
            for (int q = 0; q < 6; ++q) atomicAdd(a.prof + q, pacc[q]);
            atomicAdd(a.prof + 6, 1ull);
            atomicAdd(a.prof + 7, (unsigned long long)pchunks);
        }
        if (ticket < FSM_TRACE_UNITS) {
            unsigned long long* tr = a.prof + 8 + 4 * (size_t)ticket;
            tr[0] = trace_t0; tr[1] = FSM_ENABLE_PROF == 2 ? ((trace_t1 - trace_t0) & 0xffffffffull) | (twait << 32) : trace_t1; tr[2] = wall_clock64();
            tr[3] = (unsigned long long)TJ | ((unsigned long long)TK << 16) | ((unsigned long long)dir << 32) | ((unsigned long long)z << 40) |
                    ((unsigned long long)pchunks << 48);
        }
    }
#undef FSM_PMARK
#pragma unroll
    for (int off = 32; off > 0; off >>= 1) nevals += __shfl_down(nevals, off, 64);
#pragma unroll
    for (int l = 0; l < NS; ++l) {
        double accd = (double)dec[l];
#pragma unroll
        for (int off = 32; off > 0; off >>= 1) accd += __shfl_down(accd, off, 64);
        if ((tid & 63) == 0 && accd != 0.0) atomicAdd(a.change + grp * NS + l, accd);
        if ((tid & 63) == 0 && nevals && ((lm >> l) & 1)) atomicAdd(pa.evals + grp * NS + l, nevals);
    }
    return true;
}

template <typename T, int PJ, int PK, int C, bool IS3D, bool SKIP, int H, int NS, bool XS, bool PRE = false, int AR = 0>
#ifndef FSM_WENO_MINW
#define FSM_WENO_MINW FSM_MINW
#endif
__global__ __launch_bounds__(PJ* PK, (SKIP && IS3D && H == 1 && NS == 2 && sizeof(T) == 4) ? 3
                                     : (IS3D && H == 2 && NS == 1 && sizeof(T) == 4) ? FSM_WENO_MINW : FSM_MINW) void fsm_sweep_persistent(const PersistArgs<T> pa) {
    if constexpr (fsm_looped(IS3D, H)) {
        (void)pa;
        for (;;) {
            auto kp = __builtin_amdgcn_kernarg_segment_ptr();
            asm volatile("" : "+s"(kp));
            if (!fsm_sweep_unit<T, PJ, PK, C, IS3D, SKIP, H, NS, XS, PRE, AR>(*(const PersistArgs<T>*)kp)) break;
        }
    } else {
        fsm_sweep_unit<T, PJ, PK, C, IS3D, SKIP, H, NS, XS, PRE, AR>(pa);
    }
}

template <typename T>
struct Sweep45Args {
    T* tt;
    const T* s;
    const uint32_t* frozen;
    double* change;
    const int* slots;
    const int* lmask;
    int ts, by_group;
    int nnx, nnz;
    size_t n_nodes;
    uint32_t mask_words;
    T dx;
};

template <typename T, int NT>
__global__ __launch_bounds__(NT) void fsm_sweep45(const Sweep45Args<T> a) {
    constexpr int W = 16, C = 8;
    __shared__ T ring[NT * W];
    int slot;
    if (a.by_group) {
        const int z = blockIdx.x / a.ts, l = blockIdx.x % a.ts;
        const int grp = a.slots[z];
        if (grp < 0 || !((a.lmask[z] >> l) & 1)) return;
        slot = grp * a.ts + l;
    } else {
        slot = a.slots[blockIdx.x];
        if (slot < 0) return;
    }
    T* __restrict__ Tg = a.tt + ((size_t)(slot / a.ts) * a.n_nodes * a.ts + slot % a.ts);
    const uint32_t* __restrict__ Fz = a.frozen + (size_t)slot * a.mask_words;
    const int nnx = a.nnx, nnz = a.nnz, ts = a.ts;
    const T TMAX = real_traits<T>::max();
    const int r = threadIdx.x;
    constexpr int S = NT - 2;
    T dec = 0;
    for (int dir = 0; dir < 4; ++dir) {
        const int ri = (dir == 1) | (dir == 2), rj = dir >> 1;
        for (int x0 = 0; x0 < nnx; x0 += S) {
            const int ncol = nnx - x0 < S ? nnx - x0 : S;
            const int nlev = 2 * (ncol - 1) + nnz;
            const int xp = x0 + r - 1;
            const bool col_in = xp >= 0 && xp < nnx && r <= ncol + 1;
            const bool own = r >= 1 && r <= ncol;
            const int i = ri ? nnx - 1 - xp : xp;
            const uint32_t rowbase = (uint32_t)(col_in ? i : 0) * nnz;
            auto load_levels = [&](int lo, T* v) {
#pragma unroll
                for (int e = 0; e < C; ++e) {
                    const int zp = lo + e - 2 * (r - 1);
                    const bool ok = col_in && zp >= 0 && zp < nnz;
                    const uint32_t n = rowbase + (rj ? nnz - 1 - zp : zp);
                    v[e] = ok ? ld_sc1(Tg + (size_t)n * ts) : TMAX;
                }
// ... 785 lines not shown
    uint32_t* frozen;
    int* bbox;
    const InitPoint<T>* pts;
    int n_pts, npts;
    int nnx, nny, nnz;
    T dx, dz, xmin, ymin, zmin;
    int dim;
    int* stamp;
    int nbf, nbj, nbk;
};

template <typename T>
__device__ __forceinline__ T node_coord(T cmin, uint32_t n, T d) { return cmin + (T)n * d; }

template <typename T>
__global__ void fsm_init_source(const InitArgs<T> a) {
    const int tid = threadIdx.x;
    int lo[3] = {1 << 30, 1 << 30, 1 << 30}, hi[3] = {-1, -1, -1};
    for (int n = 0; n < a.n_pts; ++n) {
        const InitPoint<T> p = a.pts[n];
        const int npts = a.npts;
        const int b0 = p.on_node ? -npts : -(npts - 1);
        const int w = npts - b0 + 1;
        const int nbox = a.dim == 3 ? w * w * w : w * w;
        if (p.on_node && tid == 0) {
            const size_t nn = a.dim == 3 ? ((size_t)p.k * a.nny + p.j) * a.nnx + p.i : (size_t)p.i * a.nnz + p.k;
            a.tt[nn * a.ts] = p.t0;
            atomicOr(&a.frozen[nn >> 5], 1u << (nn & 31));
        }
        __syncthreads();
        for (int b = tid; b < nbox; b += blockDim.x) {
            if (a.dim == 3) {
                const int ii = p.i + b0 + b % w, jj = p.j + b0 + (b / w) % w, kk = p.k + b0 + b / (w * w);
                if (ii < 0 || ii >= a.nnx || jj < 0 || jj >= a.nny || kk < 0 || kk >= a.nnz) continue;
                if (ii == p.i && jj == p.j && kk == p.k) continue;
                const size_t m = ((size_t)kk * a.nny + jj) * a.nnx + ii;
                const T x = node_coord(a.xmin, ii, a.dx), y = node_coord(a.ymin, jj, a.dx), z = node_coord(a.zmin, kk, a.dx);
                const T d2 = (x - p.x) * (x - p.x) + (y - p.y) * (y - p.y) + (z - p.z) * (z - p.z);
                const T d = (T)__builtin_sqrt((double)d2);
                a.tt[m * a.ts] = p.t0 + d * a.slowness[m];
                atomicOr(&a.frozen[m >> 5], 1u << (m & 31));
            } else {
                const int ii = p.i + b0 + b / w, kk = p.k + b0 + b % w;
                if (ii < 0 || ii >= a.nnx || kk < 0 || kk >= a.nnz) continue;
                if (p.on_node && ii == p.i && kk == p.k) continue;
                const size_t m = (size_t)ii * a.nnz + kk;
                const T x = node_coord(a.xmin, ii, a.dx), z = node_coord(a.zmin, kk, a.dz);
                const T d2 = (x - p.x) * (x - p.x) + (z - p.z) * (z - p.z);
                const T d = (T)__builtin_sqrt((double)d2);
                T tt;
                if (p.on_node) {
                    const size_t nn = (size_t)p.i * a.nnz + p.k;
                    const T ssum = a.slowness[m] + a.slowness[nn];
                    tt = (T)((double)p.t0 + ((double)d * 0.5) * (double)ssum);
                } else {
                    tt = p.t0 + d * a.slowness[m];
                }
                a.tt[m * a.ts] = tt;
                atomicOr(&a.frozen[m >> 5], 1u << (m & 31));
            }
        }
        __syncthreads();
        const int ci[3] = {p.i, p.j, p.k};
        const int nn3[3] = {a.nnx, a.dim == 3 ? a.nny : 1, a.nnz};
        for (int d = 0; d < 3; ++d) {
            if (a.dim == 2 && d == 1) { lo[1] = 0; hi[1] = 0; continue; }
            int l = ci[d] + b0, h = ci[d] + npts;
            l = l < 0 ? 0 : l;
            h = h > nn3[d] - 1 ? nn3[d] - 1 : h;
            lo[d] = l < lo[d] ? l : lo[d];
            hi[d] = h > hi[d] ? h : hi[d];
        }
    }
    if (tid == 0) {
        if (a.dim == 3) {
            a.bbox[0] = lo[0]; a.bbox[1] = hi[0]; a.bbox[2] = lo[1]; a.bbox[3] = hi[1]; a.bbox[4] = lo[2]; a.bbox[5] = hi[2];
        } else {
            a.bbox[0] = lo[2]; a.bbox[1] = hi[2]; a.bbox[2] = lo[0]; a.bbox[3] = hi[0]; a.bbox[4] = 0; a.bbox[5] = 0;
        }
        if (a.stamp) {
            for (int bk = a.bbox[4] / FSM_BRICK; bk <= a.bbox[5] / FSM_BRICK; ++bk)
                for (int bj = a.bbox[2] / FSM_BRICK; bj <= a.bbox[3] / FSM_BRICK; ++bj)
                    for (int bf = a.bbox[0] / FSM_BRICK; bf <= a.bbox[1] / FSM_BRICK; ++bf)
                        a.stamp[((size_t)bk * a.nbj + bj) * a.nbf + bf] = 0;
        }
    }
}

template <typename T>
__device__ __forceinline__ T interp3d_pt(const T* __restrict__ Tn, int ts, T px, T py, T pz, int nnx, int nny, int nnz, T dx,
                                         T xmin, T ymin, T zmin) {
    const double small2 = 1.e-4 * 1.e-4;
    const T dy = dx, dz = dx;
    const uint32_t i = idx_u32(small2 + (double)((px - xmin) / dx));
    const uint32_t j = idx_u32(small2 + (double)((py - ymin) / dy));
    const uint32_t k = idx_u32(small2 + (double)((pz - zmin) / dz));
    auto ab = [](T v) { return v < 0 ? -v : v; };
    const bool onx = (double)ab(px - (xmin + (T)i * dx)) < small2;
    const bool ony = (double)ab(py - (ymin + (T)j * dy)) < small2;
    const bool onz = (double)ab(pz - (zmin + (T)k * dz)) < small2;
    auto cl = [](uint32_t v, int n) { return v < (uint32_t)n ? v : (uint32_t)n - 1u; };
#define TT(ii, jj, kk) Tn[(((size_t)cl(kk, nnz) * nny + cl(jj, nny)) * nnx + cl(ii, nnx)) * ts]
    T tt;
    if (onx && ony && onz) {
        tt = TT(i, j, k);
    } else if (onx && ony) {
        T t1 = TT(i, j, k), t2 = TT(i, j, k + 1);
        T w1 = (zmin + (T)(k + 1) * dz - pz) / dz, w2 = (pz - (zmin + (T)k * dz)) / dz;
        tt = t1 * w1 + t2 * w2;
    } else if (onx && onz) {
        T t1 = TT(i, j, k), t2 = TT(i, j + 1, k);
        T w1 = (ymin + (T)(j + 1) * dy - py) / dy, w2 = (py - (ymin + (T)j * dy)) / dy;
        tt = t1 * w1 + t2 * w2;
    } else if (ony && onz) {
        T t1 = TT(i, j, k), t2 = TT(i + 1, j, k);
        T w1 = (xmin + (T)(i + 1) * dx - px) / dx, w2 = (px - (xmin + (T)i * dx)) / dx;
        tt = t1 * w1 + t2 * w2;
    } else if (onx) {
        T t1 = TT(i, j, k), t2 = TT(i, j, k + 1), t3 = TT(i, j + 1, k), t4 = TT(i, j + 1, k + 1);
        T w1 = (zmin + (T)(k + 1) * dz - pz) / dz, w2 = (pz - (zmin + (T)k * dz)) / dz;
        t1 = t1 * w1 + t2 * w2;
        t2 = t3 * w1 + t4 * w2;
        w1 = (ymin + (T)(j + 1) * dy - py) / dy;
        w2 = (py - (ymin + (T)j * dy)) / dy;
        tt = t1 * w1 + t2 * w2;
    } else if (ony) {
        T t1 = TT(i, j, k), t2 = TT(i, j, k + 1), t3 = TT(i + 1, j, k), t4 = TT(i + 1, j, k + 1);
        T w1 = (zmin + (T)(k + 1) * dz - pz) / dz, w2 = (pz - (zmin + (T)k * dz)) / dz;
        t1 = t1 * w1 + t2 * w2;
        t2 = t3 * w1 + t4 * w2;
        w1 = (xmin + (T)(i + 1) * dx - px) / dx;
        w2 = (px - (xmin + (T)i * dx)) / dx;
        tt = t1 * w1 + t2 * w2;
    } else if (onz) {
        T t1 = TT(i, j, k), t2 = TT(i, j + 1, k), t3 = TT(i + 1, j, k), t4 = TT(i + 1, j + 1, k);
        T w1 = (ymin + (T)(j + 1) * dy - py) / dy, w2 = (py - (ymin + (T)j * dy)) / dy;
        t1 = t1 * w1 + t2 * w2;
        t2 = t3 * w1 + t4 * w2;
        w1 = (xmin + (T)(i + 1) * dx - px) / dx;
        w2 = (px - (xmin + (T)i * dx)) / dx;
        tt = t1 * w1 + t2 * w2;
    } else {
        T t1 = TT(i, j, k), t2 = TT(i, j, k + 1), t3 = TT(i, j + 1, k), t4 = TT(i, j + 1, k + 1);
        T t5 = TT(i + 1, j, k), t6 = TT(i + 1, j, k + 1), t7 = TT(i + 1, j + 1, k), t8 = TT(i + 1, j + 1, k + 1);
        T w1 = (zmin + (T)(k + 1) * dz - pz) / dz, w2 = (pz - (zmin + (T)k * dz)) / dz;
        t1 = t1 * w1 + t2 * w2;
        t2 = t3 * w1 + t4 * w2;
        t3 = t5 * w1 + t6 * w2;
        t4 = t7 * w1 + t8 * w2;
        w1 = (ymin + (T)(j + 1) * dy - py) / dy;
        w2 = (py - (ymin + (T)j * dy)) / dy;
        t1 = t1 * w1 + t2 * w2;
        t2 = t3 * w1 + t4 * w2;
        w1 = (xmin + (T)(i + 1) * dx - px) / dx;
        w2 = (px - (xmin + (T)i * dx)) / dx;
        tt = t1 * w1 + t2 * w2;
    }
#undef TT
    return tt;
}

template <typename T>
__host__ __device__ inline int interp3d_stencil(T px, T py, T pz, int nnx, int nny, int nnz, T dx, T xmin, T ymin, T zmin, long long* node,
                                                T* wt) {
    const double small2 = 1.e-4 * 1.e-4;
    const T p[3] = {px, py, pz}, cmin[3] = {xmin, ymin, zmin};
    const int ext[3] = {nnx, nny, nnz};
// ... 768 lines not shown
```

ttcr_amd/rgrid.py:

```python
import ctypes as C

import numpy as np

from . import _lib

_verbose = 0


def set_verbose(v):
    global _verbose
    _verbose = int(v)


def _ptr(a):
    return a.ctypes.data_as(C.c_void_p)


def _row_groups(a):
    key = np.ascontiguousarray(a, dtype=np.float64) + 0.0
    n = key.shape[0]
    if n == 0:
        return np.zeros(0, dtype=np.intp), np.zeros(1, dtype=np.intp), key
    ne = key[1:] != key[:-1]
    diff = ne[:, 0].copy()
    for c in range(1, key.shape[1]):
        diff |= ne[:, c]
    run0 = np.r_[0, np.nonzero(diff)[0] + 1]
    lens = np.diff(np.r_[run0, n])
    reps = key[run0]
    ro = np.lexsort(reps.T[::-1])
    reps, run0, lens = reps[ro], run0[ro], lens[ro]
    first = np.cumsum(lens) - lens
    order = np.arange(n) - np.repeat(first, lens) + np.repeat(run0, lens)
    g0 = np.r_[True, np.any(reps[1:] != reps[:-1], axis=1)]
    return order, np.r_[first[g0], n], reps[g0]


def _first_rows(a):
    order, bounds, _ = _row_groups(a)
    return np.sort(order[bounds[:-1]])


def _device_arg(device):
    if isinstance(device, (list, tuple, np.ndarray)):
        devs = tuple(int(d) for d in device)
        if not devs:
            raise ValueError("device list is empty")
        return devs if len(devs) > 1 else devs[0]
    return int(device)


class _GridBase:

    _dtype = np.float64
    _ndim = 3

    def __init__(self):
        self._h = C.c_void_p()
        self._lib = None

    def __del__(self):
        try:
            if self._lib is not None and self._h:
                self._lib.ttcr_fsm_destroy(self._h)
                self._h = C.c_void_p()
        except Exception:
            pass

    @property
    def n_threads(self):
        return self._n_threads

    @property
    def n_devices(self):
        return int(self._lib.ttcr_fsm_n_devices(self._h))

    def set_use_thread_pool(self, use_thread_pool):
        self._use_pool = bool(use_thread_pool)

    def set_traveltime_from_raypath(self, traveltime_from_raypath):
        self.set_option("tt_from_rp", 1 if traveltime_from_raypath else 0)
        self.tt_from_rp = bool(traveltime_from_raypath)

    def set_option(self, key, value):
        _lib.check(self._lib.ttcr_fsm_set_option(self._h, key.encode(), float(value)))

    def set_slowness_device(self, device_ptr, n):
        _lib.check(self._lib.ttcr_fsm_set_slowness_device(self._h, C.c_void_p(int(device_ptr)), int(n)))

    def get_niter(self, thread_no=0):
        a, b = C.c_int(), C.c_int()
        _lib.check(self._lib.ttcr_fsm_get_niter(self._h, int(thread_no), C.byref(a), C.byref(b)))
        return a.value

    def get_niterw(self, thread_no=0):
        a, b = C.c_int(), C.c_int()
        _lib.check(self._lib.ttcr_fsm_get_niter(self._h, int(thread_no), C.byref(a), C.byref(b)))
        return b.value

    def get_changes(self, thread_no=0):
        n1, n2 = self.get_niter(thread_no), self.get_niterw(thread_no)
        a, b = (C.c_double * max(n1, 1))(), (C.c_double * max(n2, 1))()
        _lib.check(self._lib.ttcr_fsm_get_changes(self._h, int(thread_no), a, n1, b, n2))
        return np.array(a[:n1]), np.array(b[:n2])

    def get_reference_changes(self, thread_no=0):
        n1, n2 = self.get_niter(thread_no), self.get_niterw(thread_no)
        a, b = (C.c_double * max(n1, 1))(), (C.c_double * max(n2, 1))()
        _lib.check(self._lib.ttcr_fsm_get_reference_changes(self._h, int(thread_no), a, n1, b, n2))
        return np.array(a[:n1]), np.array(b[:n2])

    def timing(self):
        t = _lib.Timing()
        _lib.check(self._lib.ttcr_fsm_last_timing(self._h, C.byref(t)))
        return {k: getattr(t, k) for k, _ in t._fields_}

    def stopping_stats(self):
        a, b, c = C.c_longlong(0), C.c_longlong(0), C.c_longlong(0)
        _lib.check(self._lib.ttcr_fsm_stopping_stats(self._h, C.byref(a), C.byref(b), C.byref(c)))
        return {"reference_sums": a.value, "reference_sums_missed": b.value, "rounds": c.value}

    def prefill_swaps(self):
        a = C.c_longlong(0)
        _lib.check(self._lib.ttcr_fsm_prefill_swaps(self._h, C.byref(a)))
        return a.value

    def reference_change(self, times, field, parallel=True):
        dt = self._dtype
        a = np.ascontiguousarray(times, dtype=dt).ravel()
        b = np.ascontiguousarray(field, dtype=dt).ravel()
        n = self.get_number_of_nodes()
        if a.size != n or b.size != n:
            raise ValueError('reference_change: fields of get_number_of_nodes() values expected')
        out = np.zeros(1, dtype=dt)
        _lib.check(self._lib.ttcr_fsm_reference_change(self._h, a.ctypes.data, b.ctypes.data, 1 if parallel else 0, out.ctypes.data))
        return out[0]

    def last_kernel(self):
        buf = C.create_string_buffer(256)
        _lib.check(self._lib.ttcr_fsm_last_kernel(self._h, buf, 256))
        return buf.value.decode()

    def _flat_tt(self, thread_no):
        if thread_no >= self._n_threads:
            raise ValueError('Thread number is larger than number of threads')
        n = self.get_number_of_nodes()
        out = np.empty(n, dtype=self._dtype)
        _lib.check(self._lib.ttcr_fsm_get_tt(self._h, int(thread_no), _ptr(out), n))
        return out

    def get_s0(self, hypo, slowness=None):
        nd = self._ndim
        hypo = np.asarray(hypo)
        if hypo.ndim != 2 or hypo.shape[1] != nd + 2:
            raise ValueError('hypo should be npts x %d' % (nd + 2))
        src = hypo[:, 2:2 + nd]
        evID = hypo[:, 0]
        eid = np.sort(np.unique(evID))
        if slowness is not None:
            self.set_slowness(slowness)
        first = np.array([int(np.nonzero(evID == e)[0][0]) for e in eid], dtype=np.int64)
        pts = np.ascontiguousarray(src[first, :], dtype=self._dtype)
        out = np.empty(max(len(eid), 1), dtype=self._dtype)
        _lib.check(self._lib.ttcr_fsm_compute_slowness(self._h, len(eid), _ptr(pts), 0, _ptr(out)))
        s0 = np.zeros((src.shape[0],))
        for n, e in enumerate(eid):
            s0[evID == e] = out[n]
        return s0

    def tt_device_ptr(self, thread_no=0):
        p = C.c_void_p()
        _lib.check(self._lib.ttcr_fsm_get_tt_device(self._h, int(thread_no), C.byref(p)))
        return p.value

    def tt_device_view(self, thread_no=0):
        p, st = C.c_void_p(), C.c_size_t()
        _lib.check(self._lib.ttcr_fsm_get_tt_device_view(self._h, int(thread_no), C.byref(p), C.byref(st)))
        return p.value, st.value

    def to_vtk(self, fields, filename):
        from . import io as _io

        if self._ndim == 3:
            nodes, cells = (self._x.size, self._y.size, self._z.size), (self._x.size - 1, self._y.size - 1, self._z.size - 1)
            xyz = (self._x, self._y, self._z)
        else:
            nodes, cells = (self._x.size, self._z.size), (self._x.size - 1, self._z.size - 1)
# ... 1391 lines not shown
```

Baseline: 96000.

## Add per-face brick stamp planes to sharpen skip decisions in persistent sweeps

```diff
diff --git a/include/ttcr_amd.h b/include/ttcr_amd.h
--- a/include/ttcr_amd.h
+++ b/include/ttcr_amd.h
@@ -65,6 +65,7 @@
 int ttcr_fsm_get_niter(ttcr_fsm_grid* g, int slot, int* niter, int* niterw);
 int ttcr_fsm_get_changes(ttcr_fsm_grid* g, int slot, double* first_order, int n_first, double* weno, int n_weno);
 int ttcr_fsm_get_reference_changes(ttcr_fsm_grid* g, int slot, double* first_order, int n_first, double* weno, int n_weno);
+int ttcr_fsm_get_sweep_evals(ttcr_fsm_grid* g, int slot, unsigned long long* evals, int n, int* n_sweeps);
 
 int ttcr_fsm_n_slots(const ttcr_fsm_grid* g);
 size_t ttcr_fsm_n_nodes(const ttcr_fsm_grid* g);
diff --git a/ttcr_amd/_lib.py b/ttcr_amd/_lib.py
--- a/ttcr_amd/_lib.py
+++ b/ttcr_amd/_lib.py
@@ -42,6 +42,7 @@
     "ttcr_fsm_get_niter": (_I, [_P, _I, C.POINTER(_I), C.POINTER(_I)]),
     "ttcr_fsm_get_changes": (_I, [_P, _I, C.POINTER(_D), _I, C.POINTER(_D), _I]),
     "ttcr_fsm_get_reference_changes": (_I, [_P, _I, C.POINTER(_D), _I, C.POINTER(_D), _I]),
+    "ttcr_fsm_get_sweep_evals": (_I, [_P, _I, C.POINTER(C.c_ulonglong), _I, C.POINTER(_I)]),
     "ttcr_fsm_n_slots": (_I, [_P]),
     "ttcr_fsm_n_nodes": (C.c_size_t, [_P]),
     "ttcr_fsm_n_cells": (C.c_size_t, [_P]),
diff --git a/ttcr_amd/csrc/fsm_capi.hip b/ttcr_amd/csrc/fsm_capi.hip
--- a/ttcr_amd/csrc/fsm_capi.hip
+++ b/ttcr_amd/csrc/fsm_capi.hip
@@ -166,6 +166,14 @@
         for (int q = 0; q < n_first; ++q) first[q] = (!ref_hist.empty() && q < (int)ref_hist[slot].size()) ? ref_hist[slot][q] : std::nan("");
         for (int q = 0; q < n_weno; ++q) wen[q] = (!ref_histw.empty() && q < (int)ref_histw[slot].size()) ? ref_histw[slot][q] : std::nan("");
     }
+    std::vector<std::vector<unsigned long long>> sweep_evals;
+    virtual int get_sweep_evals(int slot, unsigned long long* out, int n) const {
+        if (slot < 0 || slot >= n_slots) throw ValueError("Thread number is larger than number of threads");
+        slot = P(slot);
+        const int have = sweep_evals.empty() ? 0 : (int)sweep_evals[slot].size();
+        for (int q = 0; q < n; ++q) out[q] = q < have ? sweep_evals[slot][q] : 0ull;
+        return have;
+    }
     virtual void get_changes(int slot, double* first, int n_first, double* wen, int n_weno) const {
         if (slot < 0 || slot >= n_slots) throw ValueError("Thread number is larger than number of threads");
         slot = P(slot);
@@ -300,6 +308,7 @@
     DevBuf<unsigned long long> d_cmap;
     int cmap_words = 1;
     DevBuf<unsigned long long> d_sw;
+    DevBuf<unsigned long long> d_sw_evals;
     int sw_sweeps = 0;
     DevBuf<int> d_iter;
     DevBuf<unsigned long long> d_evals;
@@ -428,7 +437,7 @@
         nbj = (geom.NJ + FSM_BRICK - 1) / FSM_BRICK;
         nbk = (geom.NK + FSM_BRICK - 1) / FSM_BRICK;
         n_bricks = (size_t)nbf * nbj * nbk;
-        d_stamp.reserve(n_bricks * n_slots);
+        d_stamp.reserve(FSM_STAMP_PLANES * n_bricks * n_slots);
         {
             const int PJ = dim == 3 ? TileCfg<T, 3>::PJ : TileCfg<T, 2>::PJ, PK = dim == 3 ? TileCfg<T, 3>::PK : 1;
             const int max_chunks = (geom.NF + 2 * (PJ + PK)) / 4 + 4;
@@ -437,6 +446,7 @@
             HIP_CHECK(hipMemset(d_cmap.p, 0, (size_t)n_patches * n_slots * (dim == 3 ? 8 : 4) * 2 * cmap_words * sizeof(unsigned long long)));
             sw_sweeps = (dim == 3 ? 8 : 4) * (2 * std::min(nitermax, 256) + 2);
             d_sw.reserve((size_t)sw_sweeps * n_slots);
+            d_sw_evals.reserve((size_t)sw_sweeps * n_slots);
         }
         d_iter.reserve(2);
         d_evals.reserve(n_slots);
@@ -599,6 +609,7 @@
         pa.sw = std::getenv("TTCR_FSM_NO_SW") ? nullptr : d_sw.p;
         pa.n_sw_groups = n_groups();
         pa.n_sw_sweeps = sw_sweeps;
+        pa.sw_evals = d_sw_evals.p;
 
         const size_t wg_cap = (fsm_looped(DIM == 3, H) && persist_wgs > 0) ? (size_t)persist_wgs : ~(size_t)0;
         const dim3 block(C::PJ * C::PK), grid((unsigned)std::min<size_t>((size_t)n_patches * batch, wg_cap));
@@ -1085,7 +1096,7 @@
         const bool vec = n_el % V == 0 && ((uintptr_t)ta.cur | (uintptr_t)ta.old) % 16 == 0;
         const int nodes_per_vec = vec ? std::max(1, V / NS) : 1;
         const bool bricks = since_T >= 0 && geom.NF % nodes_per_vec == 0;
-        ta.stamp = bricks ? d_stamp.p + (size_t)gi * n_bricks : nullptr;
+        ta.stamp = bricks ? d_stamp.p + (size_t)gi * FSM_STAMP_PLANES * n_bricks : nullptr;
         ta.thr = (dim == 3 ? 8 : 4) * since_T + 1;
         ta.NF = geom.NF; ta.NJ = geom.NJ; ta.nbf = nbf; ta.nbj = nbj;
         const unsigned nblk = (unsigned)((n_nodes + FSM_REFSUM_CB - 1) / FSM_REFSUM_CB);
@@ -1376,7 +1387,7 @@
         d_pts.reserve(std::max<size_t>(tot_pts, 1));
         HIP_CHECK(hipMemcpyAsync(d_pts.p, pts.data(), pts.size() * sizeof(InitPoint<T>), hipMemcpyHostToDevice, stream));
         for (int b = 0; b < nb; ++b)
-            HIP_CHECK(hipMemsetAsync(d_stamp.p + (size_t)(slot_ids[b] / NS) * n_bricks, 0xFF, n_bricks * sizeof(int), stream));
+            HIP_CHECK(hipMemsetAsync(d_stamp.p + (size_t)(slot_ids[b] / NS) * FSM_STAMP_PLANES * n_bricks, 0xFF, FSM_STAMP_PLANES * n_bricks * sizeof(int), stream));
         std::vector<char> group_filled(n_groups(), 0);
         const bool all_slots = nb == n_slots && prefill_on();
         if (all_slots && alt_filled) {
@@ -1420,7 +1431,7 @@
             ia.nnz = ncz + 1;
             ia.dx = dx; ia.dz = dz; ia.xmin = xmin; ia.ymin = ymin; ia.zmin = zmin;
             ia.dim = dim;
-            ia.stamp = d_stamp.p + (size_t)(slot / NS) * n_bricks;
+            ia.stamp = d_stamp.p + (size_t)(slot / NS) * FSM_STAMP_PLANES * n_bricks;
             ia.nbf = nbf; ia.nbj = nbj; ia.nbk = nbk;
             fsm_init_source<T><<<1, 128, 0, stream>>>(ia);
             niter[slot] = 0;
@@ -1451,8 +1462,10 @@
         if (persistent_now() || weno) HIP_CHECK(hipMemsetAsync(d_sync.p + 4, 0, sizeof(int), stream));
         HIP_CHECK(hipMemsetAsync(d_evals.p, 0, sizeof(unsigned long long) * n_slots, stream));
         HIP_CHECK(hipMemsetAsync(d_sw.p, 0, sizeof(unsigned long long) * (size_t)sw_sweeps * n_groups(), stream));
+        HIP_CHECK(hipMemsetAsync(d_sw_evals.p, 0, sizeof(unsigned long long) * (size_t)sw_sweeps * n_groups(), stream));
         HIP_CHECK(hipEventRecord(ev0, stream));
         int it_total = 0;
+        int launched_entries = nb;
         for (stage = 0; stage < (weno ? 2 : 1); ++stage) {
             std::vector<int> active(slot_ids);
             int it = 0;
@@ -1465,6 +1478,7 @@
             std::vector<int> groups;
             for (int s2 : slot_ids)
                 if (groups.empty() || groups.back() != s2 / NS) groups.push_back(s2 / NS);
+            if (stage == 0) launched_entries = persistent_now() ? (int)groups.size() : nb;
             while (!active.empty() && it < maxit) {
                 int n_entries;
                 if (persistent_now()) {
@@ -1523,8 +1537,8 @@
             if (stage == 0 && weno) {
                 HIP_CHECK(hipMemsetAsync(d_sw.p, 0, sizeof(unsigned long long) * (size_t)sw_sweeps * n_groups(), stream));
                 for (int s2 : slot_ids)
-                    HIP_CHECK(hipMemsetD32Async((hipDeviceptr_t)(d_stamp.p + (size_t)(s2 / NS) * n_bricks), it_total * (dim == 3 ? 8 : 4),
-                                                n_bricks, stream));
+                    HIP_CHECK(hipMemsetD32Async((hipDeviceptr_t)(d_stamp.p + (size_t)(s2 / NS) * FSM_STAMP_PLANES * n_bricks), it_total * (dim == 3 ? 8 : 4),
+                                                FSM_STAMP_PLANES * n_bricks, stream));
             }
         }
         if (std::getenv("TTCR_FSM_DEBUG_SW")) {
@@ -1590,10 +1604,18 @@
         if (was_persistent) {
             HIP_CHECK(hipMemcpy(h_evals, d_evals.p, sizeof(unsigned long long) * n_slots, hipMemcpyDeviceToHost));
             for (int s2 : slot_ids) timing.evaluated_updates += (long long)h_evals[s2];
+            const int rows = std::min(it_total * ndir, sw_sweeps);
+            std::vector<unsigned long long> h_sw((size_t)std::max(rows, 1) * n_groups());
+            if (rows > 0) HIP_CHECK(hipMemcpy(h_sw.data(), d_sw_evals.p, sizeof(unsigned long long) * (size_t)rows * n_groups(), hipMemcpyDeviceToHost));
+            if ((int)sweep_evals.size() != n_slots) sweep_evals.assign(n_slots, {});
+            for (int s2 : slot_ids) {
+                sweep_evals[s2].resize(rows);
+                for (int q = 0; q < rows; ++q) sweep_evals[s2][q] = h_sw[(size_t)q * n_groups() + s2 / NS];
+            }
         } else {
             timing.evaluated_updates += timing.node_updates - node_updates_before;
         }
-        const bool skipped_now = skip_now(n_groups());
+        const bool skipped_now = skip_now(launched_entries);
         if (nb == n_slots && timing.node_updates > node_updates_before && skipped_now)
             last_eval_frac = (double)(timing.evaluated_updates - evaluated_before) / (double)(timing.node_updates - node_updates_before);
         if (skip < 0 && !weno && in_probe_window((nb + NS - 1) / NS) && timing.node_updates > node_updates_before) {
@@ -2653,6 +2675,9 @@
     void get_reference_changes(int slot, double* first, int n_first, double* wen, int n_weno) const override {
         int l; GridBase& g = of(slot, l); g.get_reference_changes(l, first, n_first, wen, n_weno);
     }
+    int get_sweep_evals(int slot, unsigned long long* out, int n) const override {
+        int l; GridBase& g = of(slot, l); return g.get_sweep_evals(l, out, n);
+    }
     void rays_size(size_t* n_rays, size_t* n_points) const override { *n_rays = rays_off.size() - 1; *n_points = (size_t)rays_off.back(); }
     void get_rays(long long* offsets, void* pts) const override {
         std::memcpy(offsets, rays_off.data(), rays_off.size() * sizeof(long long));
@@ -4136,6 +4161,12 @@
         g->impl->get_changes(slot, first_order, n_first, weno, n_weno);
     });
 }
+int ttcr_fsm_get_sweep_evals(ttcr_fsm_grid* g, int slot, unsigned long long* evals, int n, int* n_sweeps) {
+    return guarded_on(g, [&] {
+        const int have = g->impl->get_sweep_evals(slot, evals, n);
+        if (n_sweeps) *n_sweeps = have;
+    });
+}
 int ttcr_fsm_get_reference_changes(ttcr_fsm_grid* g, int slot, double* first_order, int n_first, double* weno, int n_weno) {
     return guarded_on(g, [&] {
         if ((n_first > 0 && !first_order) || (n_weno > 0 && !weno) || n_first < 0 || n_weno < 0) throw ValueError("bad output buffers");
diff --git a/ttcr_amd/csrc/fsm_kernels.h b/ttcr_amd/csrc/fsm_kernels.h
--- a/ttcr_amd/csrc/fsm_kernels.h
+++ b/ttcr_amd/csrc/fsm_kernels.h
@@ -6,6 +6,7 @@
 namespace ttcr_amd {
 
 constexpr int FSM_BRICK = 16;
+constexpr int FSM_STAMP_PLANES = 5;
 
 template <typename T> struct real_traits;
 template <> struct real_traits<float> {
@@ -440,6 +441,7 @@
     int cw;
     unsigned long long* sw;
     int n_sw_groups, n_sw_sweeps;
+    unsigned long long* sw_evals;
     const T* ssh;
     size_t ssh_stride;
 };
@@ -811,13 +813,21 @@
     __shared__ int s_anychg;
     constexpr int SLABW = SKIP ? FSM_SLAB_WORDS : 1;
     __shared__ unsigned s_stamped[SKIP ? 9 : 1][SLABW];
+    constexpr int NOWNB = IS3D ? 4 : 6;
+    static_assert(!SKIP || (IS3D ? (PJ <= FSM_BRICK && PK <= FSM_BRICK) : PJ <= 4 * FSM_BRICK), "own bricks of a unit");
+    __shared__ unsigned s_fstamped[SKIP ? 4 * NOWNB : 1][SLABW];
+    __shared__ int s_plane[SKIP ? 9 : 1], s_ownrow[SKIP ? NOWNB : 1];
+    __shared__ unsigned short s_tface[SKIP ? NT : 1];
     __shared__ unsigned s_slab[SLABW];
     __shared__ int s_next, s_act;
     __shared__ int s_cwi[2], s_cwl[2];
     __shared__ unsigned s_cwv[2];
     __shared__ int s_mywi;
     __shared__ unsigned s_mywv[2];
-    enum { U_THR, U_RSJLO, U_RSKLO, U_RSNJ, U_RSNK, U_LCF, U_UPLCF0, U_UPLCF1, U_HIST, U_EVER, U_UCHG, U_PENDV, U_LCHG, U_N };
+    enum { U_THR, U_RSJLO, U_RSKLO, U_RSNJ, U_RSNK, U_LCF, U_UPLCF0, U_UPLCF1, U_HIST, U_EVER, U_UCHG, U_PENDV, U_LCHG,
+           U_OJLO, U_OJN, U_OKLO, U_OKN,
+           U_NOWN,
+           U_N };
     __shared__ int s_u[U_N];
 
     int tid = threadIdx.x;
@@ -1205,6 +1215,7 @@
         const int nsw = (pa.nbf + 31) >> 5;
         for (int w = tid; w < nsw; w += NT) s_slab[w] = 0u;
         for (int w = tid; w < 9 * SLABW; w += NT) s_stamped[w / SLABW][w % SLABW] = 0u;
+        for (int w = tid; w < 4 * NOWNB * nsw; w += NT) s_fstamped[w / nsw][w % nsw] = 0u;
         if (tid == 0) {
             s_cwi[0] = -1; s_cwi[1] = -1; s_mywi = -1;
             const int ja = j0 - H < 0 ? 0 : j0 - H, jb = jmaxp + H > NJ - 1 ? NJ - 1 : jmaxp + H;
@@ -1213,6 +1224,20 @@
             const int klo = (rk ? NK - 1 - kb : ka) / FSM_BRICK, khi = (rk ? NK - 1 - ka : kb) / FSM_BRICK;
             s_u[U_RSJLO] = jlo; s_u[U_RSNJ] = jhi - jlo + 1;
             s_u[U_RSKLO] = klo; s_u[U_RSNK] = khi - klo + 1;
+            const int ojlo = (rj ? NJ - 1 - jmaxp : j0) / FSM_BRICK, ojhi = (rj ? NJ - 1 - j0 : jmaxp) / FSM_BRICK;
+            const int oklo = (rk ? NK - 1 - kmaxp : k0) / FSM_BRICK, okhi = (rk ? NK - 1 - k0 : kmaxp) / FSM_BRICK;
+            s_u[U_OJLO] = ojlo - jlo; s_u[U_OJN] = ojhi - ojlo + 1;
+            s_u[U_OKLO] = oklo - klo; s_u[U_OKN] = okhi - oklo + 1;
+            s_u[U_NOWN] = (ojhi - ojlo + 1) * (okhi - oklo + 1);
+            for (int pk = 0; pk <= khi - klo; ++pk)
+                for (int pj = 0; pj <= jhi - jlo; ++pj) {
+                    const bool inj = pj >= ojlo - jlo && pj <= ojhi - jlo, ink = pk >= oklo - klo && pk <= okhi - klo;
+                    int plane = 0;
+                    if (inj != ink) plane = ink ? (pj < ojlo - jlo ? 2 : 1) : (pk < oklo - klo ? 4 : 3);
+                    else if (H == 1 && !inj) plane = -1;
+                    s_plane[pk * (jhi - jlo + 1) + pj] = plane;
+                    if (inj && ink) s_ownrow[(pk - (oklo - klo)) * (ojhi - ojlo + 1) + pj - (ojlo - jlo)] = pk * (jhi - jlo + 1) + pj;
+                }
             const int sg = pa.ndir * pa.iter_ptr[0] + dir + 1;
             s_u[U_THR] = pa.skip == 2 ? -(1 << 30) : (sg - 1 > 0 ? sg - 1 : 0);
             s_u[U_LCF] = Lc;
@@ -1224,14 +1249,26 @@
         __syncthreads();
         {
             const int jlo = s_u[U_RSJLO], nj = s_u[U_RSNJ], klo = s_u[U_RSKLO], nk = s_u[U_RSNK], thr = s_u[U_THR];
-            const int* __restrict__ stamp = pa.stamp + (size_t)grp * pa.nbf * pa.nbj * pa.nbk;
+            const size_t nb3 = (size_t)pa.nbf * pa.nbj * pa.nbk;
+            const int* __restrict__ stamp = pa.stamp + (size_t)grp * FSM_STAMP_PLANES * nb3;
             const int total = pa.nbf * nj * nk;
             for (int b = tid; b < total; b += NT) {
                 const int bf = b % pa.nbf, jk = b / pa.nbf;
                 const int bj = jlo + jk % nj, bk = klo + jk / nj;
-                const int v = __hip_atomic_load(stamp + ((size_t)bk * pa.nbj + bj) * pa.nbf + bf, __ATOMIC_RELAXED, __HIP_MEMORY_SCOPE_AGENT);
+                const int plane = s_plane[jk];
+                if (plane < 0) continue;
+                const int v = __hip_atomic_load(stamp + plane * nb3 + ((size_t)bk * pa.nbj + bj) * pa.nbf + bf, __ATOMIC_RELAXED, __HIP_MEMORY_SCOPE_AGENT);
                 if (v >= thr) atomicOr(&s_slab[bf >> 5], 1u << (bf & 31));
             }
+            unsigned rows = 0xffffu;
+            if (col_ok) {
+                const int jnat = rj ? NJ - 1 - jp : jp, knat = rk ? NK - 1 - kp : kp;
+                const int ob = (knat / FSM_BRICK - klo - s_u[U_OKLO]) * s_u[U_OJN] + (jnat / FSM_BRICK - jlo - s_u[U_OJLO]);
+                const int jr = jnat % FSM_BRICK, kr = knat % FSM_BRICK;
+                const int fj = jr < H ? 0 : (jr >= FSM_BRICK - H ? 1 : -1), fk = !IS3D ? -1 : (kr < H ? 2 : (kr >= FSM_BRICK - H ? 3 : -1));
+                rows = (fj >= 0 ? (unsigned)(fj * NOWNB + ob) : 0xffu) | ((fk >= 0 ? (unsigned)(fk * NOWNB + ob) : 0xffu) << 8);
+            }
+            s_tface[tid] = (unsigned short)rows;
         }
         __syncthreads();
     }
@@ -1550,6 +1587,15 @@
                 const int jk = my_bk * s_u[U_RSNJ] + my_bj;
                 atomicOr(&s_stamped[jk][ba >> 5], 1u << (ba & 31));
                 if (bb2 != ba) atomicOr(&s_stamped[jk][bb2 >> 5], 1u << (bb2 & 31));
+                const unsigned rows = s_tface[tid];
+                if ((rows & 0xffu) != 0xffu) {
+                    atomicOr(&s_fstamped[rows & 0xffu][ba >> 5], 1u << (ba & 31));
+                    if (bb2 != ba) atomicOr(&s_fstamped[rows & 0xffu][bb2 >> 5], 1u << (bb2 & 31));
+                }
+                if ((rows >> 8) != 0xffu) {
+                    atomicOr(&s_fstamped[rows >> 8][ba >> 5], 1u << (ba & 31));
+                    if (bb2 != ba) atomicOr(&s_fstamped[rows >> 8][bb2 >> 5], 1u << (bb2 & 31));
+                }
             }
         } else {
             if (wave_any(changed) && (tid & 63) == 0) s_anychg = 1;
@@ -1575,7 +1621,11 @@
                 if (any_changed) {
                     int flo, fhi;
                     chunk_frange(L0, 0, flo, fhi);
-                    for (int b = flo / FSM_BRICK; b <= fhi / FSM_BRICK; ++b) s_slab[b >> 5] |= 1u << (b & 31);
+                    for (int w = (flo / FSM_BRICK) >> 5; w <= (fhi / FSM_BRICK) >> 5; ++w) {
+                        unsigned m2 = 0u;
+                        for (int q = 0; q < s_u[U_NOWN]; ++q) m2 |= s_stamped[s_ownrow[q]][w];
+                        s_slab[w] |= m2;
+                    }
                     const int ci = (L0 - s_u[U_LCF]) / C, w = ci >> 5;
                     if ((chg_flags & 6) && w < pa.cw) {
                         if (s_mywi != w) { s_mywi = w; s_mywv[0] = 0u; s_mywv[1] = 0u; }
@@ -1610,13 +1660,20 @@
         if (s_u[U_UCHG]) {
             const int nsw = (pa.nbf + 31) >> 5;
             const int rs_jlo = s_u[U_RSJLO], rs_nj = s_u[U_RSNJ], rs_klo = s_u[U_RSKLO], njk = rs_nj * s_u[U_RSNK];
-            int* __restrict__ stamp = pa.stamp + (size_t)grp * pa.nbf * pa.nbj * pa.nbk;
+            const size_t nb3 = (size_t)pa.nbf * pa.nbj * pa.nbk;
+            int* __restrict__ stamp = pa.stamp + (size_t)grp * FSM_STAMP_PLANES * nb3;
             const int sigma = pa.ndir * pa.iter_ptr[0] + dir + 1;
             for (int q = tid; q < njk * nsw * 32; q += NT) {
                 const int jk = q / (nsw * 32), bf = q % (nsw * 32);
                 if (bf < pa.nbf && ((s_stamped[jk][bf >> 5] >> (bf & 31)) & 1u))
                     atomicMax(stamp + ((size_t)(rs_klo + jk / rs_nj) * pa.nbj + rs_jlo + jk % rs_nj) * pa.nbf + bf, sigma);
             }
+            const int onj = s_u[U_OJN], nob = onj * s_u[U_OKN];
+            for (int q = tid; q < 4 * nob * nsw * 32; q += NT) {
+                const int f = q / (nob * nsw * 32), r = q % (nob * nsw * 32), ob = r / (nsw * 32), bf = r % (nsw * 32);
+                if (bf < pa.nbf && ((s_fstamped[f * NOWNB + ob][bf >> 5] >> (bf & 31)) & 1u))
+                    atomicMax(stamp + (1 + f) * nb3 + ((size_t)(rs_klo + s_u[U_OKLO] + ob / onj) * pa.nbj + rs_jlo + s_u[U_OJLO] + ob % onj) * pa.nbf + bf, sigma);
+            }
             pending = 1;
         }
     }
@@ -1653,6 +1710,10 @@
 #undef FSM_PMARK
 #pragma unroll
     for (int off = 32; off > 0; off >>= 1) nevals += __shfl_down(nevals, off, 64);
+    if constexpr (SKIP) {
+        const int sigma0 = pa.ndir * pa.iter_ptr[0] + dir;
+        if ((tid & 63) == 0 && nevals && sigma0 < pa.n_sw_sweeps) atomicAdd(pa.sw_evals + (size_t)sigma0 * pa.n_sw_groups + grp, nevals);
+    }
 #pragma unroll
     for (int l = 0; l < NS; ++l) {
         double accd = (double)dec[l];
@@ -2604,7 +2665,8 @@
             for (int bk = a.bbox[4] / FSM_BRICK; bk <= a.bbox[5] / FSM_BRICK; ++bk)
                 for (int bj = a.bbox[2] / FSM_BRICK; bj <= a.bbox[3] / FSM_BRICK; ++bj)
                     for (int bf = a.bbox[0] / FSM_BRICK; bf <= a.bbox[1] / FSM_BRICK; ++bf)
-                        a.stamp[((size_t)bk * a.nbj + bj) * a.nbf + bf] = 0;
+                        for (int pl = 0; pl < FSM_STAMP_PLANES; ++pl)
+                            a.stamp[(size_t)pl * a.nbf * a.nbj * a.nbk + ((size_t)bk * a.nbj + bj) * a.nbf + bf] = 0;
         }
     }
 }
diff --git a/ttcr_amd/rgrid.py b/ttcr_amd/rgrid.py
--- a/ttcr_amd/rgrid.py
+++ b/ttcr_amd/rgrid.py
@@ -103,6 +103,13 @@
         a, b = (C.c_double * max(n1, 1))(), (C.c_double * max(n2, 1))()
         _lib.check(self._lib.ttcr_fsm_get_changes(self._h, int(thread_no), a, n1, b, n2))
         return np.array(a[:n1]), np.array(b[:n2])
+
+    def get_sweep_evals(self, thread_no=0):
+        n = C.c_int(0)
+        _lib.check(self._lib.ttcr_fsm_get_sweep_evals(self._h, int(thread_no), None, 0, C.byref(n)))
+        a = (C.c_ulonglong * max(n.value, 1))()
+        _lib.check(self._lib.ttcr_fsm_get_sweep_evals(self._h, int(thread_no), a, n.value, None))
+        return np.array(a[:n.value], dtype=np.uint64)
 
     def get_reference_changes(self, thread_no=0):
         n1, n2 = self.get_niter(thread_no), self.get_niterw(thread_no)
```

After: 95100. About the same (-0.9%).
